# seung-lab/igneous

Measured on NVIDIA H100. Metric: Mvoxels/s on 2048x2048x1024 uint32 seg per GPU (downsample+CCL+mesh) @1/2/4/8 H100; % HBM roofline, higher is better.
Workload: dtype u32

## Files before the change

igneous_b200/csrc/common.cuh:

```cuda
#pragma once
#include <cuda_runtime.h>
#include <stdint.h>
#include <stdio.h>
#include <string>
#include <vector>

#include "../../include/igneous_b200.h"

#if defined(__CUDA_ARCH__) && (__CUDA_ARCH__ != 900)
#error "libigneous_b200 targets sm_90a (Hopper H100) only"
#endif

namespace ign {

void set_error(const char* fmt, ...);

#define IGN_CUDA(call)                                                          \
  do {                                                                          \
    cudaError_t _e = (call);                                                    \
    if (_e != cudaSuccess) {                                                    \
      ign::set_error("%s:%d: %s -> %s", __FILE__, __LINE__, #call,              \
                     cudaGetErrorString(_e));                                   \
      return IGN_ERR_CUDA;                                                      \
    }                                                                           \
  } while (0)

#define IGN_TRY(call)                 \
  do {                                \
    int _s = (call);                  \
    if (_s != IGN_OK) return _s;      \
  } while (0)

#define IGN_REQUIRE(cond, status, ...)   \
  do {                                   \
    if (!(cond)) {                       \
      ign::set_error(__VA_ARGS__);       \
      return (status);                   \
    }                                    \
  } while (0)

static inline int dtype_size(int dt) {
  switch (dt) {
    case IGN_U8: return 1;
    case IGN_U16: return 2;
    case IGN_U32: return 4;
    case IGN_U64: return 8;
    case IGN_F32: return 4;
    default: return 0;
  }
}

template <typename F>
int dispatch_label(int dtype, const char* who, F&& f) {
  switch (dtype) {
    case IGN_U8: return f(uint8_t{});
    case IGN_U16: return f(uint16_t{});
    case IGN_U32: return f(uint32_t{});
    case IGN_U64: return f(uint64_t{});
  }
  set_error("%s: unsupported label dtype %d", who, dtype);
  return IGN_ERR_UNSUPPORTED;
}

}

constexpr int IGN_TIMER_SLOTS = 64;

struct ign_ctx {
  int device;
  int sm_count;
  cudaStream_t stream;
  cudaStream_t copy_stream;
  struct ScratchBlock { char* base; size_t bytes, used; };
  std::vector<ScratchBlock> scratch;
  size_t scratch_lin;
  size_t scratch_high;
  int scratch_frames;
  char* pinned;
  size_t pinned_bytes;
  cudaEvent_t timers[IGN_TIMER_SLOTS][2];
  uint64_t launches;
  int prof_on;
  struct ProfRec { int cls; cudaEvent_t a, b; };
  ProfRec* prof;
  int prof_n, prof_cap;
  char* mesh_pool;
  size_t mesh_pool_bytes;
  int mesh_pool_busy;
  char* win;
  char* win_dev;
  size_t win_fetch_used, win_push_used;
  struct FetchRec { void* dst; size_t off, bytes; };
  FetchRec fetch[32];
  int fetch_n;
};

enum { IGN_PROF_CCL_LOCAL = 0, IGN_PROF_CCL_MERGE = 1, IGN_PROF_CCL_LABEL = 2, IGN_PROF_POOL = 3,
       IGN_PROF_MC = 4, IGN_PROF_SIMP = 5, IGN_PROF_CLASSES = 8 };

namespace ign {

int activate(ign_ctx* ctx);
class ScratchFrame {
 public:
  explicit ScratchFrame(ign_ctx* ctx);
  ~ScratchFrame();
  ScratchFrame(const ScratchFrame&) = delete;
  ScratchFrame& operator=(const ScratchFrame&) = delete;
  int take(void** p, size_t bytes);
  template <typename T>
  int take(T** p, size_t count) { return take((void**)p, count * sizeof(T)); }
  void rewind();
  bool innermost() const;

 private:
  ign_ctx* ctx_;
  std::vector<size_t> mark_;
  size_t mark_lin_;
  int depth_;
};

static inline size_t align_up(size_t v, size_t a) { return (v + a - 1) / a * a; }

struct HostBuf {
  const void* from;
  void* to;
  size_t bytes;
};

template <typename F>
int staged(ign_ctx* ctx, std::vector<HostBuf>& bufs, F&& call) {
  IGN_TRY(activate(ctx));
  ScratchFrame f(ctx);
  std::vector<void*> d(bufs.size(), nullptr);
  for (size_t i = 0; i < bufs.size(); i++) {
    if (!bufs[i].from && !bufs[i].to) continue;
    IGN_TRY(f.take(&d[i], bufs[i].bytes));
    if (bufs[i].from)
      IGN_CUDA(cudaMemcpyAsync(d[i], bufs[i].from, bufs[i].bytes, cudaMemcpyHostToDevice, ctx->stream));
  }
  IGN_TRY(call(d.data()));
  for (size_t i = 0; i < bufs.size(); i++)
    if (bufs[i].to) IGN_CUDA(cudaMemcpyAsync(bufs[i].to, d[i], bufs[i].bytes, cudaMemcpyDeviceToHost, ctx->stream));
  IGN_CUDA(cudaStreamSynchronize(ctx->stream));
  return IGN_OK;
}
template <typename F>
int staged(ign_ctx* ctx, std::vector<HostBuf>&& bufs, F&& call) {
  return staged(ctx, bufs, call);
}

int small_d2h(ign_ctx* ctx, void* host_dst, const void* dev_src, size_t bytes);
int d2h_by_kernel(ign_ctx* ctx, void* host_dst, const void* dev_src, size_t bytes);
int small_h2d(ign_ctx* ctx, void* dev_dst, const void* host_src, size_t bytes);
int small_sync(ign_ctx* ctx);

#define IGN_LAUNCH(ctx, kernel, grid, block, smem, ...)                          \
  do {                                                                           \
    kernel<<<(grid), (block), (smem), (ctx)->stream>>>(__VA_ARGS__);             \
    (ctx)->launches++;                                                           \
    IGN_CUDA(cudaGetLastError());                                                \
  } while (0)

int prof_begin(ign_ctx* ctx, int cls);
void prof_end(ign_ctx* ctx, int slot);
#define IGN_LAUNCH_PROF(ctx, cls, kernel, grid, block, smem, ...)                 \
  do {                                                                           \
    const int _slot = ign::prof_begin((ctx), (cls));                             \
    kernel<<<(grid), (block), (smem), (ctx)->stream>>>(__VA_ARGS__);             \
    (ctx)->launches++;                                                           \
    ign::prof_end((ctx), _slot);                                                 \
    IGN_CUDA(cudaGetLastError());                                                \
  } while (0)

static inline unsigned blocks_for(uint64_t n, unsigned threads) {
  return (unsigned)((n + threads - 1) / threads);
}

}

#ifdef __CUDACC__
namespace ign {

__device__ __forceinline__ uint4 ld_stream(const void* p) {
  uint4 r;
  asm volatile("ld.global.nc.L1::no_allocate.v4.u32 {%0,%1,%2,%3}, [%4];"
               : "=r"(r.x), "=r"(r.y), "=r"(r.z), "=r"(r.w)
               : "l"(p));
  return r;
}
__device__ __forceinline__ void st_stream(void* p, uint4 v) {
  asm volatile("st.global.L1::no_allocate.v4.u32 [%0], {%1,%2,%3,%4};" ::"l"(p), "r"(v.x),
               "r"(v.y), "r"(v.z), "r"(v.w)
               : "memory");
}
__device__ __forceinline__ void st_stream(void* p, uint2 v) {
  asm volatile("st.global.L1::no_allocate.v2.u32 [%0], {%1,%2};" ::"l"(p), "r"(v.x), "r"(v.y)
               : "memory");
}

__device__ __forceinline__ uint64_t mix64(uint64_t z) {
  z += 0x9E3779B97F4A7C15ull;
  z = (z ^ (z >> 30)) * 0xBF58476D1CE4E5B9ull;
  z = (z ^ (z >> 27)) * 0x94D049BB133111EBull;
  return z ^ (z >> 31);
}

}
#endif
```

igneous_b200/csrc/ctx.cu:

```cuda
#include <stdarg.h>
#include <string.h>

#include "common.cuh"

namespace ign {

static thread_local std::string g_err;

void set_error(const char* fmt, ...) {
  char buf[1024];
  va_list ap;
  va_start(ap, fmt);
  vsnprintf(buf, sizeof(buf), fmt, ap);
  va_end(ap);
  g_err = buf;
}

int activate(ign_ctx* ctx) {
  IGN_REQUIRE(ctx != nullptr, IGN_ERR_INVALID, "null ign_ctx");
  IGN_CUDA(cudaSetDevice(ctx->device));
  return IGN_OK;
}

ScratchFrame::ScratchFrame(ign_ctx* ctx) : ctx_(ctx), mark_lin_(ctx->scratch_lin), depth_(++ctx->scratch_frames) {
  for (const auto& b : ctx->scratch) mark_.push_back(b.used);
}

ScratchFrame::~ScratchFrame() {
  rewind();
  if (--ctx_->scratch_frames > 0 || ctx_->scratch.size() < 2) return;
  if (cudaStreamSynchronize(ctx_->stream) != cudaSuccess) {
    cudaGetLastError();
    return;
  }
  for (const auto& b : ctx_->scratch) cudaFree(b.base);
  ctx_->scratch.clear();
  const size_t bytes = align_up(ctx_->scratch_high, 1 << 20);
  char* base = nullptr;
  if (cudaMalloc((void**)&base, bytes) == cudaSuccess) ctx_->scratch.push_back({base, bytes, 0});
  else cudaGetLastError();
}

void ScratchFrame::rewind() {
  for (size_t b = 0; b < ctx_->scratch.size(); b++) ctx_->scratch[b].used = b < mark_.size() ? mark_[b] : 0;
  ctx_->scratch_lin = mark_lin_;
}

bool ScratchFrame::innermost() const { return ctx_->scratch_frames == depth_; }

int ScratchFrame::take(void** p, size_t bytes) {
  *p = nullptr;
  std::vector<ign_ctx::ScratchBlock>& blocks = ctx_->scratch;
  size_t b = 0, off = 0;
  for (; b < blocks.size(); b++) {
    off = align_up(blocks[b].used, 256);
    if (off + bytes <= blocks[b].bytes) break;
  }
  if (b == blocks.size()) {
    const size_t want = align_up(bytes ? bytes : 1, 1 << 20);
    char* base = nullptr;
    cudaError_t e = cudaMalloc((void**)&base, want);
    if (e != cudaSuccess) {
      cudaGetLastError();
      set_error("scratch arena: cudaMalloc(%zu) failed: %s", want, cudaGetErrorString(e));
      return IGN_ERR_NOMEM;
    }
    blocks.push_back({base, want, 0});
    off = 0;
  }
  blocks[b].used = off + bytes;
  ctx_->scratch_lin = align_up(ctx_->scratch_lin, 256) + bytes;
  if (ctx_->scratch_lin > ctx_->scratch_high) ctx_->scratch_high = ctx_->scratch_lin;
  *p = blocks[b].base + off;
  return IGN_OK;
}

template <typename T>
__global__ void __launch_bounds__(256)
    k_copy_box(const T* __restrict__ src, uint64_t sx, uint64_t sy, uint64_t x0, uint64_t y0,
               uint64_t z0, uint64_t bx, uint64_t by, uint64_t total, T* __restrict__ dst) {
  const uint64_t i = blockIdx.x * (uint64_t)blockDim.x + threadIdx.x;
  if (i >= total) return;
  const uint64_t x = i % bx, r = i / bx, y = r % by, z = r / by;
  dst[i] = src[((z0 + z) * sy + (y0 + y)) * sx + (x0 + x)];
}

enum : size_t { WIN_FETCH_BYTES = 256 << 10, WIN_PUSH_BYTES = 768 << 10 };

__global__ void __launch_bounds__(256) k_copy_small(void* __restrict__ dst, const void* __restrict__ src,
                                                    uint32_t n_words, uint32_t tail_bytes) {
  const uint32_t i = blockIdx.x * blockDim.x + threadIdx.x;
  if (i < n_words) ((uint32_t*)dst)[i] = ((const uint32_t*)src)[i];
  if (i < tail_bytes) ((uint8_t*)dst)[4ull * n_words + i] = ((const uint8_t*)src)[4ull * n_words + i];
}

static int copy_small_launch(ign_ctx* ctx, void* dst, const void* src, size_t bytes);

__global__ void __launch_bounds__(256) k_copy_to_host(uint4* __restrict__ dst, const uint4* __restrict__ src, uint64_t n16) {
  for (uint64_t i = blockIdx.x * (uint64_t)blockDim.x + threadIdx.x; i < n16; i += (uint64_t)gridDim.x * blockDim.x)
    dst[i] = src[i];
}

int d2h_by_kernel(ign_ctx* ctx, void* host_dst, const void* dev_src, size_t bytes) {
  cudaPointerAttributes at;
  const bool pinned = cudaPointerGetAttributes(&at, host_dst) == cudaSuccess && at.type == cudaMemoryTypeHost &&
                      at.devicePointer != nullptr;
  cudaGetLastError();
  if (!pinned || ((uintptr_t)at.devicePointer % 16) != 0 || ((uintptr_t)dev_src % 16) != 0) {
    IGN_CUDA(cudaMemcpyAsync(host_dst, dev_src, bytes, cudaMemcpyDeviceToHost, ctx->stream));
    return IGN_OK;
  }
  const uint64_t n16 = bytes / 16;
  if (n16) {
    const unsigned grid = (unsigned)(blocks_for(n16, 256) < (uint64_t)ctx->sm_count * 2 ? blocks_for(n16, 256) : (uint64_t)ctx->sm_count * 2);
    IGN_LAUNCH(ctx, k_copy_to_host, grid, 256, 0, (uint4*)at.devicePointer, (const uint4*)dev_src, n16);
  }
  if (bytes % 16)
    IGN_TRY(copy_small_launch(ctx, (char*)at.devicePointer + 16 * n16, (const char*)dev_src + 16 * n16, bytes % 16));
  return IGN_OK;
}

static int copy_small_launch(ign_ctx* ctx, void* dst, const void* src, size_t bytes) {
  const bool words = ((uintptr_t)dst % 4 == 0) && ((uintptr_t)src % 4 == 0);
  const uint32_t nw = words ? (uint32_t)(bytes / 4) : 0;
  const uint32_t tail = (uint32_t)(bytes - 4ull * nw);
  const uint32_t work = nw > tail ? nw : tail;
  IGN_LAUNCH(ctx, k_copy_small, blocks_for(work, 256), 256, 0, dst, src, nw, tail);
  return IGN_OK;
}

int small_d2h(ign_ctx* ctx, void* host_dst, const void* dev_src, size_t bytes) {
  if (bytes == 0) return IGN_OK;
  const size_t off = align_up(ctx->win_fetch_used, 16);
  if (!ctx->win || ctx->fetch_n == 32 || off + bytes > WIN_FETCH_BYTES) {
    IGN_CUDA(cudaMemcpyAsync(host_dst, dev_src, bytes, cudaMemcpyDeviceToHost, ctx->stream));
    return IGN_OK;
  }
  IGN_TRY(copy_small_launch(ctx, ctx->win_dev + off, dev_src, bytes));
  ctx->fetch[ctx->fetch_n++] = {host_dst, off, bytes};
  ctx->win_fetch_used = off + bytes;
  return IGN_OK;
}

int small_sync(ign_ctx* ctx) {
  cudaError_t e = cudaStreamSynchronize(ctx->stream);
  if (e == cudaSuccess)
    for (int i = 0; i < ctx->fetch_n; i++)
      memcpy(ctx->fetch[i].dst, ctx->win + ctx->fetch[i].off, ctx->fetch[i].bytes);
  ctx->fetch_n = 0;
  ctx->win_fetch_used = 0;
  ctx->win_push_used = 0;
  IGN_CUDA(e);
  return IGN_OK;
}

int small_h2d(ign_ctx* ctx, void* dev_dst, const void* host_src, size_t bytes) {
  if (bytes == 0) return IGN_OK;
  if (!ctx->win || bytes > WIN_PUSH_BYTES) {
    IGN_CUDA(cudaMemcpyAsync(dev_dst, host_src, bytes, cudaMemcpyHostToDevice, ctx->stream));
    return IGN_OK;
  }
  size_t off = align_up(ctx->win_push_used, 16);
  if (off + bytes > WIN_PUSH_BYTES) {
    IGN_CUDA(cudaStreamSynchronize(ctx->stream));
    off = 0;
  }
  char* stage = ctx->win + WIN_FETCH_BYTES + off;
  memcpy(stage, host_src, bytes);
  ctx->win_push_used = off + bytes;
  return copy_small_launch(ctx, dev_dst, ctx->win_dev + WIN_FETCH_BYTES + off, bytes);
}

int prof_begin(ign_ctx* ctx, int cls) {
  if (!ctx->prof_on) return -1;
  if (ctx->prof_n == ctx->prof_cap) {
    const int ncap = ctx->prof_cap ? ctx->prof_cap * 2 : 256;
    ign_ctx::ProfRec* np = (ign_ctx::ProfRec*)realloc(ctx->prof, sizeof(ign_ctx::ProfRec) * ncap);
    if (!np) return -1;
    for (int i = ctx->prof_cap; i < ncap; i++) {
      cudaEventCreate(&np[i].a);
      cudaEventCreate(&np[i].b);
    }
    ctx->prof = np;
    ctx->prof_cap = ncap;
  }
  const int slot = ctx->prof_n++;
  ctx->prof[slot].cls = cls;
  cudaEventRecord(ctx->prof[slot].a, ctx->stream);
  return slot;
}

void prof_end(ign_ctx* ctx, int slot) {
  if (slot >= 0) cudaEventRecord(ctx->prof[slot].b, ctx->stream);
}

}

using namespace ign;

extern "C" {

int ign_version(void) { return 100; }

const char* ign_last_error(void) { return g_err.c_str(); }

int ign_device_count(int* n) {
  IGN_REQUIRE(n, IGN_ERR_INVALID, "null out pointer");
  cudaError_t e = cudaGetDeviceCount(n);
  if (e != cudaSuccess) {
    *n = 0;
    set_error("cudaGetDeviceCount: %s", cudaGetErrorString(e));
    cudaGetLastError();
    return IGN_ERR_CUDA;
  }
  return IGN_OK;
}

int ign_init(int device, ign_ctx** out) {
  IGN_REQUIRE(out, IGN_ERR_INVALID, "null out pointer");
  *out = nullptr;
  int n = 0;
  IGN_TRY(ign_device_count(&n));
  IGN_REQUIRE(n > 0, IGN_ERR_CUDA, "no CUDA device visible (this library has no CPU fallback)");
  IGN_REQUIRE(device >= 0 && device < n, IGN_ERR_INVALID, "device %d out of range [0,%d)", device, n);
  IGN_CUDA(cudaSetDevice(device));
  cudaDeviceProp prop;
  IGN_CUDA(cudaGetDeviceProperties(&prop, device));
  IGN_REQUIRE(prop.major == 9 && prop.minor == 0, IGN_ERR_UNSUPPORTED,
              "device %d is sm_%d%d; libigneous_b200 is built for sm_90a (H100) only", device,
              prop.major, prop.minor);
  ign_ctx* ctx = new ign_ctx();
  ctx->device = device;
  ctx->sm_count = prop.multiProcessorCount;
  ctx->launches = 0;
  ctx->prof_on = 0;
  ctx->prof = nullptr;
  ctx->prof_n = ctx->prof_cap = 0;
  ctx->mesh_pool = nullptr;
  ctx->mesh_pool_bytes = 0;
  ctx->mesh_pool_busy = 0;
  IGN_CUDA(cudaStreamCreateWithFlags(&ctx->stream, cudaStreamNonBlocking));
  IGN_CUDA(cudaStreamCreateWithFlags(&ctx->copy_stream, cudaStreamNonBlocking));
  ctx->pinned_bytes = 1 << 20;
  IGN_CUDA(cudaHostAlloc((void**)&ctx->pinned, ctx->pinned_bytes, cudaHostAllocDefault));
  for (int i = 0; i < IGN_TIMER_SLOTS; i++) {
    IGN_CUDA(cudaEventCreate(&ctx->timers[i][0]));
    IGN_CUDA(cudaEventCreate(&ctx->timers[i][1]));
  }
  ctx->win = ctx->win_dev = nullptr;
  ctx->win_fetch_used = ctx->win_push_used = 0;
  ctx->fetch_n = 0;
  if (cudaHostAlloc((void**)&ctx->win, WIN_FETCH_BYTES + WIN_PUSH_BYTES,
                    cudaHostAllocMapped | cudaHostAllocPortable) != cudaSuccess ||
      cudaHostGetDevicePointer((void**)&ctx->win_dev, ctx->win, 0) != cudaSuccess) {
    cudaGetLastError();
    if (ctx->win) cudaFreeHost(ctx->win);
    ctx->win = ctx->win_dev = nullptr;
  }
  *out = ctx;
  return IGN_OK;
}

int ign_destroy(ign_ctx* ctx) {
  if (!ctx) return IGN_OK;
  cudaSetDevice(ctx->device);
  cudaStreamSynchronize(ctx->stream);
  for (const auto& b : ctx->scratch) cudaFree(b.base);
  if (ctx->pinned) cudaFreeHost(ctx->pinned);
  if (ctx->win) cudaFreeHost(ctx->win);
  if (ctx->mesh_pool) cudaFree(ctx->mesh_pool);
  for (int i = 0; i < IGN_TIMER_SLOTS; i++) {
    cudaEventDestroy(ctx->timers[i][0]);
    cudaEventDestroy(ctx->timers[i][1]);
  }
  cudaStreamDestroy(ctx->stream);
  cudaStreamDestroy(ctx->copy_stream);
  delete ctx;
  return IGN_OK;
}

int ign_sync(ign_ctx* ctx) {
  IGN_TRY(activate(ctx));
  IGN_CUDA(cudaStreamSynchronize(ctx->stream));
  return IGN_OK;
}

int ign_launch_count(ign_ctx* ctx, uint64_t* n) {
  IGN_REQUIRE(ctx && n, IGN_ERR_INVALID, "null argument");
  *n = ctx->launches;
  return IGN_OK;
}

int ign_stream(ign_ctx* ctx, void** stream) {
  IGN_REQUIRE(ctx && stream, IGN_ERR_INVALID, "null argument");
  *stream = (void*)ctx->stream;
  return IGN_OK;
}

int ign_dev_alloc(ign_ctx* ctx, uint64_t bytes, void** dptr) {
  IGN_TRY(activate(ctx));
  IGN_REQUIRE(dptr, IGN_ERR_INVALID, "null out pointer");
  *dptr = nullptr;
  cudaError_t e = cudaMalloc(dptr, bytes ? bytes : 1);
  if (e != cudaSuccess) {
    cudaGetLastError();
    set_error("cudaMalloc(%llu) failed: %s", (unsigned long long)bytes, cudaGetErrorString(e));
    return IGN_ERR_NOMEM;
  }
  return IGN_OK;
}

int ign_dev_free(ign_ctx* ctx, void* dptr) {
  IGN_TRY(activate(ctx));
  IGN_CUDA(cudaStreamSynchronize(ctx->stream));
  IGN_CUDA(cudaFree(dptr));
  return IGN_OK;
}

int ign_host_alloc(ign_ctx* ctx, uint64_t bytes, void** hptr) {
  IGN_TRY(activate(ctx));
  IGN_REQUIRE(hptr, IGN_ERR_INVALID, "null out pointer");
  cudaError_t e = cudaHostAlloc(hptr, bytes ? bytes : 1, cudaHostAllocDefault);
  if (e != cudaSuccess) {
    cudaGetLastError();
    set_error("cudaHostAlloc(%llu) failed: %s", (unsigned long long)bytes, cudaGetErrorString(e));
    return IGN_ERR_NOMEM;
  }
  return IGN_OK;
}

int ign_host_free(ign_ctx* ctx, void* hptr) {
  IGN_TRY(activate(ctx));
  IGN_CUDA(cudaFreeHost(hptr));
  return IGN_OK;
}

static const uint64_t BULK_PIECE = 64ull << 20;

static int bulk_copy(ign_ctx* ctx, void* dst, const void* src, uint64_t bytes, cudaMemcpyKind kind) {
  for (uint64_t at = 0; at < bytes; at += BULK_PIECE) {
    const uint64_t nb = bytes - at < BULK_PIECE ? bytes - at : BULK_PIECE;
    IGN_CUDA(cudaMemcpyAsync((char*)dst + at, (const char*)src + at, nb, kind, ctx->stream));
  }
  return IGN_OK;
}

int ign_h2d(ign_ctx* ctx, void* dst, const void* src, uint64_t bytes) {
  IGN_TRY(activate(ctx));
  return bulk_copy(ctx, dst, src, bytes, cudaMemcpyHostToDevice);
}

int ign_d2h(ign_ctx* ctx, void* dst, const void* src, uint64_t bytes) {
  IGN_TRY(activate(ctx));
  return bulk_copy(ctx, dst, src, bytes, cudaMemcpyDeviceToHost);
}

int ign_d2d(ign_ctx* ctx, void* dst, const void* src, uint64_t bytes) {
  IGN_TRY(activate(ctx));
  IGN_CUDA(cudaMemcpyAsync(dst, src, bytes, cudaMemcpyDeviceToDevice, ctx->stream));
  return IGN_OK;
}

int ign_memset(ign_ctx* ctx, void* dst, int byte, uint64_t bytes) {
  IGN_TRY(activate(ctx));
  IGN_CUDA(cudaMemsetAsync(dst, byte, bytes, ctx->stream));
  return IGN_OK;
}

int ign_prof_enable(ign_ctx* ctx, int on) {
  IGN_REQUIRE(ctx, IGN_ERR_INVALID, "null ctx");
  ctx->prof_on = on ? 1 : 0;
  ctx->prof_n = 0;
  return IGN_OK;
}

int ign_prof_read(ign_ctx* ctx, int cls, float* total_ms, uint64_t* launches) {
  IGN_TRY(activate(ctx));
  IGN_REQUIRE(total_ms && launches, IGN_ERR_INVALID, "null argument");
  IGN_CUDA(cudaStreamSynchronize(ctx->stream));
  float sum = 0;
  uint64_t cnt = 0;
  for (int i = 0; i < ctx->prof_n; i++) {
    if (ctx->prof[i].cls != cls) continue;
    float ms = 0;
    IGN_CUDA(cudaEventElapsedTime(&ms, ctx->prof[i].a, ctx->prof[i].b));
    sum += ms;
    cnt++;
  }
  *total_ms = sum;
  *launches = cnt;
  return IGN_OK;
}

int ign_copy_box_dev(ign_ctx* ctx, const void* src, int dtype, uint64_t sx, uint64_t sy, uint64_t sz,
                     uint64_t x0, uint64_t y0, uint64_t z0, uint64_t bx, uint64_t by, uint64_t bz,
                     void* dst) {
  IGN_TRY(activate(ctx));
  const size_t es = dtype_size(dtype);
  IGN_REQUIRE(src && dst && es > 0, IGN_ERR_INVALID, "bad copy_box argument");
  IGN_REQUIRE(x0 + bx <= sx && y0 + by <= sy && z0 + bz <= sz, IGN_ERR_INVALID, "box outside the volume");
  const uint64_t total = bx * by * bz;
  if (total == 0) return IGN_OK;
  const unsigned g = blocks_for(total, 256);
  switch (es) {
    case 1: IGN_LAUNCH(ctx, (k_copy_box<uint8_t>), g, 256, 0, (const uint8_t*)src, sx, sy, x0, y0, z0, bx, by, total, (uint8_t*)dst); break;
    case 2: IGN_LAUNCH(ctx, (k_copy_box<uint16_t>), g, 256, 0, (const uint16_t*)src, sx, sy, x0, y0, z0, bx, by, total, (uint16_t*)dst); break;
    case 4: IGN_LAUNCH(ctx, (k_copy_box<uint32_t>), g, 256, 0, (const uint32_t*)src, sx, sy, x0, y0, z0, bx, by, total, (uint32_t*)dst); break;
    default: IGN_LAUNCH(ctx, (k_copy_box<uint64_t>), g, 256, 0, (const uint64_t*)src, sx, sy, x0, y0, z0, bx, by, total, (uint64_t*)dst); break;
  }
  return IGN_OK;
}

int ign_stream_wait_mark(ign_ctx* waiter, ign_ctx* producer, int slot) {
  IGN_REQUIRE(waiter && producer && slot >= 0 && slot < IGN_TIMER_SLOTS, IGN_ERR_INVALID, "bad stream_wait argument");
  IGN_TRY(activate(waiter));
  IGN_CUDA(cudaStreamWaitEvent(waiter->stream, producer->timers[slot][0], 0));
  return IGN_OK;
}

int ign_stream_priority(ign_ctx* ctx, int high) {
  IGN_TRY(activate(ctx));
  int least = 0, greatest = 0;
  IGN_CUDA(cudaDeviceGetStreamPriorityRange(&least, &greatest));
  IGN_CUDA(cudaStreamSynchronize(ctx->stream));
  cudaStream_t fresh;
  IGN_CUDA(cudaStreamCreateWithPriority(&fresh, cudaStreamNonBlocking, high ? greatest : least));
  cudaStreamDestroy(ctx->stream);
  ctx->stream = fresh;
  return IGN_OK;
}

int ign_timer_start(ign_ctx* ctx, int slot) {
  IGN_TRY(activate(ctx));
  IGN_REQUIRE(slot >= 0 && slot < IGN_TIMER_SLOTS, IGN_ERR_INVALID, "timer slot %d out of range", slot);
  IGN_CUDA(cudaEventRecord(ctx->timers[slot][0], ctx->stream));
  return IGN_OK;
}

int ign_timer_stop(ign_ctx* ctx, int slot) {
  IGN_TRY(activate(ctx));
  IGN_REQUIRE(slot >= 0 && slot < IGN_TIMER_SLOTS, IGN_ERR_INVALID, "timer slot %d out of range", slot);
  IGN_CUDA(cudaEventRecord(ctx->timers[slot][1], ctx->stream));
  return IGN_OK;
}

int ign_timer_ms(ign_ctx* ctx, int slot, float* ms) {
  IGN_TRY(activate(ctx));
  IGN_REQUIRE(slot >= 0 && slot < IGN_TIMER_SLOTS && ms, IGN_ERR_INVALID, "bad timer argument");
  IGN_CUDA(cudaEventSynchronize(ctx->timers[slot][1]));
  IGN_CUDA(cudaEventElapsedTime(ms, ctx->timers[slot][0], ctx->timers[slot][1]));
  return IGN_OK;
}

}
```

igneous_b200/csrc/mesh.cu:

```cuda
#include <cub/device/device_radix_sort.cuh>
#include <cub/device/device_scan.cuh>

#include <atomic>
#include <climits>
#include <vector>

#include "common.cuh"
#include "mc_table.h"

namespace ign {

constexpr unsigned MFULL = 0xFFFFFFFFu;
constexpr int TRI_T_BITS = 3, TRI_CUBE_BITS = 30;
constexpr int V_COORD_BITS = 11;
constexpr int V_LABEL_SHIFT = 3 * V_COORD_BITS;
constexpr int TRI_LABEL_SHIFT = TRI_T_BITS + TRI_CUBE_BITS;

__constant__ int8_t c_edge_mid[12][3] = {{1, 0, 0}, {2, 1, 0}, {1, 2, 0}, {0, 1, 0},
                                         {1, 0, 2}, {2, 1, 2}, {1, 2, 2}, {0, 1, 2},
                                         {0, 0, 1}, {2, 0, 1}, {2, 2, 1}, {0, 2, 1}};

struct McTables {
  int8_t tri[256][16];
  uint8_t ntri[256];
};
__constant__ McTables c_mc;

__device__ __forceinline__ void cube_corners(const uint32_t* __restrict__ lab, uint32_t sx,
                                             uint32_t sxy, uint32_t base, uint32_t (&c)[8]) {
  c[0] = lab[base];
  c[1] = lab[base + 1];
  c[2] = lab[base + 1 + sx];
  c[3] = lab[base + sx];
  c[4] = lab[base + sxy];
  c[5] = lab[base + 1 + sxy];
  c[6] = lab[base + 1 + sx + sxy];
  c[7] = lab[base + sx + sxy];
}

template <bool EMIT>
__global__ void __launch_bounds__(256)
    k_mc(const uint32_t* __restrict__ lab, uint32_t sx, uint32_t sy, uint32_t sz,
         unsigned long long* total, uint64_t* __restrict__ keys, uint8_t* __restrict__ cases,
         uint64_t capacity) {
  __shared__ uint8_t s_ntri[256];
  for (int i = threadIdx.x; i < 256; i += blockDim.x) s_ntri[i] = c_mc.ntri[i];
  __syncthreads();
  const uint32_t cx = sx - 1, cy = sy - 1, cz = sz - 1;
  const uint64_t ncubes = (uint64_t)cx * cy * cz;
  const uint64_t t = blockIdx.x * (uint64_t)blockDim.x + threadIdx.x;
  const uint32_t lane = threadIdx.x & 31;
  uint32_t mine = 0;
  uint32_t c[8];
  uint32_t x = 0, y = 0, z = 0;
  bool active = false;
  if (t < ncubes) {
    x = (uint32_t)(t % cx);
    y = (uint32_t)((t / cx) % cy);
    z = (uint32_t)(t / ((uint64_t)cx * cy));
    cube_corners(lab, sx, sx * sy, (z * sy + y) * sx + x, c);
    const uint32_t o = c[0] | c[1] | c[2] | c[3] | c[4] | c[5] | c[6] | c[7];
    const bool same = (c[0] == c[1]) & (c[0] == c[2]) & (c[0] == c[3]) & (c[0] == c[4]) &
                      (c[0] == c[5]) & (c[0] == c[6]) & (c[0] == c[7]);
    active = (o != 0) && !same;
  }
  uint8_t idxs[8];
  if (active) {
#pragma unroll
    for (int k = 0; k < 8; k++) {
      const uint32_t L = c[k];
      bool first = (L != 0);
#pragma unroll
      for (int j = 0; j < 8; j++)
        if (j < k) first = first && (c[j] != L);
      uint32_t idx = 0;
#pragma unroll
      for (int j = 0; j < 8; j++) idx |= (uint32_t)(c[j] == L) << j;
      idxs[k] = first ? (uint8_t)idx : 0;
      mine += s_ntri[idxs[k]];
    }
  }
  if (!EMIT) {
    uint32_t s = mine;
    for (int d = 16; d > 0; d >>= 1) s += __shfl_down_sync(MFULL, s, d);
    if (lane == 0 && s) atomicAdd(total, (unsigned long long)s);
    return;
  }
  uint32_t incl = mine;
  for (int d = 1; d < 32; d <<= 1) {
    const uint32_t v = __shfl_up_sync(MFULL, incl, d);
    if (lane >= d) incl += v;
  }
  const uint32_t warp_total = __shfl_sync(MFULL, incl, 31);
  if (warp_total == 0) return;
  unsigned long long base = 0;
  if (lane == 31) base = atomicAdd(total, (unsigned long long)warp_total);
  base = __shfl_sync(MFULL, base, 31);
  uint64_t pos = base + (incl - mine);
  if (active) {
    const uint64_t cube = (uint64_t)t;
#pragma unroll
    for (int k = 0; k < 8; k++) {
      const uint32_t n = s_ntri[idxs[k]];
      for (uint32_t tt = 0; tt < n; tt++) {
        if (pos < capacity) {
          keys[pos] = ((uint64_t)c[k] << TRI_LABEL_SHIFT) | (cube << TRI_T_BITS) | tt;
          cases[pos] = idxs[k];
        }
        pos++;
      }
    }
  }
}

__global__ void __launch_bounds__(256)
    k_tri_vertices(const uint64_t* __restrict__ keys, const uint8_t* __restrict__ cases, uint64_t T,
                   uint32_t cx, uint32_t cy, uint64_t* __restrict__ vkeys,
                   uint32_t* __restrict__ corner) {
  const uint64_t t = blockIdx.x * (uint64_t)blockDim.x + threadIdx.x;
  if (t >= T) return;
  const uint64_t key = keys[t];
  const uint64_t label = key >> TRI_LABEL_SHIFT;
  const uint64_t cube = (key >> TRI_T_BITS) & ((1ull << TRI_CUBE_BITS) - 1);
  const uint32_t tt = (uint32_t)(key & ((1u << TRI_T_BITS) - 1));
  const uint32_t x = (uint32_t)(cube % cx), y = (uint32_t)((cube / cx) % cy),
                 z = (uint32_t)(cube / ((uint64_t)cx * cy));
  const int8_t* row = c_mc.tri[cases[t]];
#pragma unroll
  for (int v = 0; v < 3; v++) {
    const int e = row[3 * tt + (2 - v)];
    const uint64_t vx = 2 * x + c_edge_mid[e][0], vy = 2 * y + c_edge_mid[e][1],
                   vz = 2 * z + c_edge_mid[e][2];
    vkeys[3 * t + v] = (label << V_LABEL_SHIFT) | (vz << (2 * V_COORD_BITS)) | (vy << V_COORD_BITS) | vx;
    corner[3 * t + v] = (uint32_t)(3 * t + v);
  }
}

__global__ void __launch_bounds__(256)
    k_label_starts(const uint64_t* __restrict__ keys, uint64_t n, int shift,
                   uint32_t* __restrict__ start ) {
  const uint64_t i = blockIdx.x * (uint64_t)blockDim.x + threadIdx.x;
  if (i >= n) return;
  const uint64_t label = keys[i] >> shift;
  if (i == 0 || (keys[i - 1] >> shift) != label) start[label] = (uint32_t)i;
}

__global__ void __launch_bounds__(256) k_fill_u32(uint32_t* a, uint32_t value, uint32_t n) {
  const uint32_t i = blockIdx.x * blockDim.x + threadIdx.x;
  if (i < n) a[i] = value;
}

__global__ void __launch_bounds__(256)
    k_vertex_heads(const uint64_t* __restrict__ vkeys_sorted, uint64_t n, uint32_t* __restrict__ heads) {
  const uint64_t i = blockIdx.x * (uint64_t)blockDim.x + threadIdx.x;
  if (i < n) heads[i] = (i == 0 || vkeys_sorted[i - 1] != vkeys_sorted[i]) ? 1u : 0u;
}

__global__ void __launch_bounds__(256)
    k_vertex_assign(const uint64_t* __restrict__ vkeys_sorted, const uint32_t* __restrict__ corner_sorted,
                    const uint32_t* __restrict__ heads, const uint32_t* __restrict__ rank, uint64_t n,
                    uint64_t* __restrict__ uniq_vkeys, uint32_t* __restrict__ face_global) {
  const uint64_t i = blockIdx.x * (uint64_t)blockDim.x + threadIdx.x;
  if (i >= n) return;
  const uint32_t id = rank[i] + heads[i] - 1;
  if (heads[i]) uniq_vkeys[id] = vkeys_sorted[i];
  face_global[corner_sorted[i]] = id;
}

__global__ void __launch_bounds__(256)
    k_faces_local(const uint64_t* __restrict__ tri_keys, const uint32_t* __restrict__ vert_off,
                  uint64_t T, uint32_t* __restrict__ faces) {
  const uint64_t i = blockIdx.x * (uint64_t)blockDim.x + threadIdx.x;
  if (i >= 3 * T) return;
  const uint64_t label = tri_keys[i / 3] >> TRI_LABEL_SHIFT;
  faces[i] -= vert_off[label];
}

__global__ void __launch_bounds__(256)
    k_vertex_positions(const uint64_t* __restrict__ uniq_vkeys, uint64_t first, uint64_t count,
                       float rx, float ry, float rz, float shift, float* __restrict__ out) {
  const uint64_t i = blockIdx.x * (uint64_t)blockDim.x + threadIdx.x;
  if (i >= count) return;
  const uint64_t k = uniq_vkeys[first + i];
  const float x = (float)(k & ((1u << V_COORD_BITS) - 1));
  const float y = (float)((k >> V_COORD_BITS) & ((1u << V_COORD_BITS) - 1));
  const float z = (float)((k >> (2 * V_COORD_BITS)) & ((1u << V_COORD_BITS) - 1));
  out[3 * i + 0] = __fmul_rn(__fadd_rn(__fmul_rn(x, 0.5f), shift), rx);
  out[3 * i + 1] = __fmul_rn(__fadd_rn(__fmul_rn(y, 0.5f), shift), ry);
  out[3 * i + 2] = __fmul_rn(__fadd_rn(__fmul_rn(z, 0.5f), shift), rz);
}

}

#include "mesher.h"

namespace ign {
int simp_export_positions(ign_ctx* ctx, const float* pos_f, uint64_t first, uint64_t count,
                          const float shift[3], float* d_out);
}
using namespace ign;

static int mesher_positions(ign_mesher* m, uint64_t first, uint64_t count, const float resolution[3],
                            int voxel_centered, float* d_out) {
  ign_ctx* ctx = m->ctx;
  if (m->simplified) {
    IGN_REQUIRE(resolution[0] == m->res[0] && resolution[1] == m->res[1] && resolution[2] == m->res[2],
                IGN_ERR_INVALID, "resolution differs from the one the mesher was simplified with");
    const float shift[3] = {voxel_centered ? 0.5f * m->res[0] : 0.0f, voxel_centered ? 0.5f * m->res[1] : 0.0f,
                            voxel_centered ? 0.5f * m->res[2] : 0.0f};
    return simp_export_positions(ctx, m->d_pos_f, first, count, shift, d_out);
  }
  IGN_LAUNCH(ctx, k_vertex_positions, blocks_for(count, 256), 256, 0, m->d_uniq_vkeys, first, count,
             resolution[0], resolution[1], resolution[2], voxel_centered ? 0.5f : 0.0f, d_out);
  return IGN_OK;
}

static std::atomic<bool> g_tables_loaded[64];

static int load_tables(ign_ctx* ctx) {
  if (ctx->device < 64 && g_tables_loaded[ctx->device]) return IGN_OK;
  McTables h;
  memcpy(h.tri, mc_tri_table, sizeof(h.tri));
  memcpy(h.ntri, mc_tri_count, sizeof(h.ntri));
  IGN_CUDA(cudaMemcpyToSymbolAsync(c_mc, &h, sizeof(h), 0, cudaMemcpyHostToDevice, ctx->stream));
  IGN_CUDA(cudaStreamSynchronize(ctx->stream));
  if (ctx->device < 64) g_tables_loaded[ctx->device] = true;
  return IGN_OK;
}

static int bits_for(uint64_t v) {
  int b = 1;
  while (b < 64 && (1ull << b) <= v) b++;
  return b;
}

extern "C" {

int ign_mesh_free(ign_mesher* m) {
  if (!m) return IGN_OK;
  cudaSetDevice(m->ctx->device);
  if (m->pooled) {
    m->ctx->mesh_pool_busy = 0;
  } else {
    if (m->d_uniq_vkeys) cudaFree(m->d_uniq_vkeys);
    if (m->d_faces) cudaFree(m->d_faces);
  }
  delete m;
  return IGN_OK;
}

int ign_mesh_begin_dev(ign_ctx* ctx, const void* labels, int dtype, uint64_t sx, uint64_t sy,
                       uint64_t sz, ign_mesher** out) {
  IGN_TRY(activate(ctx));
  IGN_REQUIRE(labels && out, IGN_ERR_INVALID, "null argument");
  *out = nullptr;
  IGN_REQUIRE(sx >= 1 && sy >= 1 && sz >= 1, IGN_ERR_INVALID, "empty volume");
  IGN_REQUIRE(sx <= 1023 && sy <= 1023 && sz <= 1023, IGN_ERR_UNSUPPORTED,
              "mesher: task of %llux%llux%llu exceeds the 1023^3 limit of the packed vertex format",
              (unsigned long long)sx, (unsigned long long)sy, (unsigned long long)sz);
  IGN_TRY(load_tables(ctx));
  const uint64_t n = sx * sy * sz;

  ign_mesher* m = new ign_mesher();
  m->ctx = ctx;
  m->K = m->T = m->U = 0;
  m->d_uniq_vkeys = nullptr;
  m->d_faces = nullptr;
  m->pooled = false;
  m->simplified = false;
  m->d_pos_f = nullptr;
  m->simp_factor = 0;
  m->simp_max_error = 0;
  m->simp_rounds = 0;
  struct Guard {
    ign_mesher* m;
    ~Guard() { ign_mesh_free(m); }
  } guard{m};
  ScratchFrame f(ctx);

  uint32_t* d_lab;
  IGN_TRY(f.take(&d_lab, n));
  uint64_t K = 0;
  {
    ScratchFrame fu(ctx);
    uint64_t* d_uniq;
    IGN_TRY(fu.take(&d_uniq, n));
    IGN_TRY(ign_renumber_dev(ctx, labels, dtype, n, d_lab, d_uniq, n, &K));
    m->K = K;
    m->ids.resize(K);
    if (K) {
      IGN_TRY(small_d2h(ctx, m->ids.data(), d_uniq, K * 8));
      IGN_TRY(small_sync(ctx));
    }
  }
  m->tri_off.assign(K + 2, 0);
  m->vert_off.assign(K + 2, 0);
  if (K == 0 || sx < 2 || sy < 2 || sz < 2) {
    guard.m = nullptr;
    *out = m;
    return IGN_OK;
  }
  IGN_REQUIRE(K < (1ull << 31), IGN_ERR_OVERFLOW, "mesher: too many labels");

  unsigned long long* d_total;
  IGN_TRY(f.take(&d_total, 32));
  const uint64_t ncubes = (sx - 1) * (sy - 1) * (sz - 1);
  const unsigned grid = blocks_for(ncubes, 256);
  unsigned long long T = 0;
  IGN_CUDA(cudaMemsetAsync(d_total, 0, 8, ctx->stream));
  IGN_LAUNCH(ctx, (k_mc<false>), grid, 256, 0, d_lab, (uint32_t)sx, (uint32_t)sy, (uint32_t)sz, d_total,
             (uint64_t*)nullptr, (uint8_t*)nullptr, 0ull);
  IGN_TRY(small_d2h(ctx, &T, d_total, 8));
  IGN_TRY(small_sync(ctx));
  m->T = T;
  if (T == 0) {
    guard.m = nullptr;
    *out = m;
    return IGN_OK;
  }
  IGN_REQUIRE(3 * T <= (unsigned long long)INT_MAX, IGN_ERR_OVERFLOW,
              "mesher: %llu triangles exceed 2^31 - 1 corners; split the volume into tasks", T);

  size_t sort1 = 0, sort2 = 0, scanb = 0;
  cub::DeviceRadixSort::SortPairs(nullptr, sort1, (const uint64_t*)nullptr, (uint64_t*)nullptr,
                                  (const uint8_t*)nullptr, (uint8_t*)nullptr, (int)T);
  cub::DeviceRadixSort::SortPairs(nullptr, sort2, (const uint64_t*)nullptr, (uint64_t*)nullptr,
                                  (const uint32_t*)nullptr, (uint32_t*)nullptr, (int)(3 * T));
  cub::DeviceScan::ExclusiveSum(nullptr, scanb, (const uint32_t*)nullptr, (uint32_t*)nullptr, (int)(3 * T));
  size_t tmp_bytes = sort1 > sort2 ? sort1 : sort2;
  if (scanb > tmp_bytes) tmp_bytes = scanb;
  uint64_t *keys, *keys_s, *vkeys, *vkeys_s;
  uint8_t *cases, *cases_s;
  uint32_t *corner, *corner_s, *heads, *rank, *d_tri_off, *d_vert_off;
  void* tmp;
  IGN_TRY(f.take(&keys, T));
  IGN_TRY(f.take(&keys_s, T));
  IGN_TRY(f.take(&cases, T));
  IGN_TRY(f.take(&cases_s, T));
  IGN_TRY(f.take(&vkeys, 3 * T));
  IGN_TRY(f.take(&vkeys_s, 3 * T));
  IGN_TRY(f.take(&corner, 3 * T));
  IGN_TRY(f.take(&corner_s, 3 * T));
  IGN_TRY(f.take(&heads, 3 * T));
  IGN_TRY(f.take(&rank, 3 * T));
  IGN_TRY(f.take(&d_tri_off, K + 2));
  IGN_TRY(f.take(&d_vert_off, K + 2));
  IGN_TRY(f.take(&tmp, tmp_bytes));

  IGN_CUDA(cudaMemsetAsync(d_total, 0, 8, ctx->stream));
  IGN_LAUNCH(ctx, (k_mc<true>), grid, 256, 0, d_lab, (uint32_t)sx, (uint32_t)sy, (uint32_t)sz, d_total, keys,
             cases, (uint64_t)T);
  const int label_bits = bits_for(K);
  size_t tb = tmp_bytes;
  IGN_CUDA(cub::DeviceRadixSort::SortPairs(tmp, tb, keys, keys_s, cases, cases_s, (int)T, 0,
                                           TRI_LABEL_SHIFT + label_bits, ctx->stream));
  ctx->launches += 4;

  IGN_LAUNCH(ctx, k_tri_vertices, blocks_for(T, 256), 256, 0, keys_s, cases_s, (uint64_t)T, (uint32_t)(sx - 1),
             (uint32_t)(sy - 1), vkeys, corner);
  tb = tmp_bytes;
  IGN_CUDA(cub::DeviceRadixSort::SortPairs(tmp, tb, vkeys, vkeys_s, corner, corner_s, (int)(3 * T), 0,
                                           V_LABEL_SHIFT + label_bits, ctx->stream));
  ctx->launches += 4;
  IGN_LAUNCH(ctx, k_vertex_heads, blocks_for(3 * T, 256), 256, 0, vkeys_s, (uint64_t)(3 * T), heads);
  tb = tmp_bytes;
  IGN_CUDA(cub::DeviceScan::ExclusiveSum(tmp, tb, heads, rank, (int)(3 * T), ctx->stream));
  ctx->launches += 2;
  uint32_t last[2];
  IGN_TRY(small_d2h(ctx, &last[0], rank + (3 * T - 1), 4));
  IGN_TRY(small_d2h(ctx, &last[1], heads + (3 * T - 1), 4));
  IGN_TRY(small_sync(ctx));
  const uint64_t U = (uint64_t)last[0] + last[1];
  m->U = U;
  {
    const size_t fbytes = align_up(3 * T * 4, 256), vbytes = align_up(U * 12, 256);
    if (!ctx->mesh_pool_busy) {
      if (ctx->mesh_pool_bytes < fbytes + vbytes) {
        IGN_CUDA(cudaStreamSynchronize(ctx->stream));
        if (ctx->mesh_pool) cudaFree(ctx->mesh_pool);
        ctx->mesh_pool = nullptr;
        ctx->mesh_pool_bytes = 0;
        const size_t want = (fbytes + vbytes) * 5 / 4;
        IGN_CUDA(cudaMalloc((void**)&ctx->mesh_pool, want));
        ctx->mesh_pool_bytes = want;
      }
      m->d_faces = (uint32_t*)ctx->mesh_pool;
      m->d_uniq_vkeys = (uint64_t*)(ctx->mesh_pool + fbytes);
      m->pooled = true;
      ctx->mesh_pool_busy = 1;
    } else {
      IGN_CUDA(cudaMalloc((void**)&m->d_faces, 3 * T * 4));
      IGN_CUDA(cudaMalloc((void**)&m->d_uniq_vkeys, U * 12));
    }
  }
  IGN_LAUNCH(ctx, k_vertex_assign, blocks_for(3 * T, 256), 256, 0, vkeys_s, corner_s, heads, rank,
             (uint64_t)(3 * T), m->d_uniq_vkeys, m->d_faces);

  IGN_LAUNCH(ctx, k_fill_u32, blocks_for(K + 2, 256), 256, 0, d_tri_off, (uint32_t)T, (uint32_t)(K + 2));
  IGN_LAUNCH(ctx, k_fill_u32, blocks_for(K + 2, 256), 256, 0, d_vert_off, (uint32_t)U, (uint32_t)(K + 2));
  IGN_LAUNCH(ctx, k_label_starts, blocks_for(T, 256), 256, 0, keys_s, (uint64_t)T, TRI_LABEL_SHIFT, d_tri_off);
  IGN_LAUNCH(ctx, k_label_starts, blocks_for(U, 256), 256, 0, m->d_uniq_vkeys, U, V_LABEL_SHIFT, d_vert_off);
  IGN_TRY(small_d2h(ctx, m->tri_off.data(), d_tri_off, (K + 2) * 4));
  IGN_TRY(small_d2h(ctx, m->vert_off.data(), d_vert_off, (K + 2) * 4));
  IGN_TRY(small_sync(ctx));
  for (int64_t l = (int64_t)K; l >= 0; l--) {
    if (m->tri_off[l] > m->tri_off[l + 1]) m->tri_off[l] = m->tri_off[l + 1];
    if (m->vert_off[l] > m->vert_off[l + 1]) m->vert_off[l] = m->vert_off[l + 1];
  }
  IGN_TRY(small_h2d(ctx, d_vert_off, m->vert_off.data(), (K + 2) * 4));
  IGN_LAUNCH(ctx, k_faces_local, blocks_for(3 * T, 256), 256, 0, keys_s, d_vert_off, (uint64_t)T, m->d_faces);
  IGN_CUDA(cudaStreamSynchronize(ctx->stream));
  for (uint64_t l = 1; l <= K; l++)
    if (m->tri_off[l + 1] > m->tri_off[l]) m->present.push_back(m->ids[l - 1]);
  guard.m = nullptr;
  *out = m;
  return IGN_OK;
}

int ign_mesh_begin(ign_ctx* ctx, const void* labels, int dtype, uint64_t sx, uint64_t sy, uint64_t sz,
                   ign_mesher** out) {
  return staged(ctx, {{labels, nullptr, sx * sy * sz * dtype_size(dtype)}},
                [&](void* const* d) { return ign_mesh_begin_dev(ctx, d[0], dtype, sx, sy, sz, out); });
}

int ign_mesh_num_ids(ign_mesher* m, uint64_t* n) {
  IGN_REQUIRE(m && n, IGN_ERR_INVALID, "null argument");
  *n = m->present.size();
  return IGN_OK;
}

int ign_mesh_ids(ign_mesher* m, uint64_t* ids, uint64_t capacity) {
  IGN_REQUIRE(m && ids, IGN_ERR_INVALID, "null argument");
  const uint64_t k = m->present.size() < capacity ? m->present.size() : capacity;
  for (uint64_t i = 0; i < k; i++) ids[i] = m->present[i];
  return IGN_OK;
}

int ign_mesh_totals(ign_mesher* m, uint64_t* nv, uint64_t* nf) {
  IGN_REQUIRE(m && nv && nf, IGN_ERR_INVALID, "null argument");
  *nv = m->U;
  *nf = m->T;
  return IGN_OK;
}

static int64_t dense_of(ign_mesher* m, uint64_t id) {
  for (uint64_t i = 0; i < m->ids.size(); i++)
    if (m->ids[i] == id) return (int64_t)i + 1;
  return -1;
}

int ign_mesh_counts(ign_mesher* m, uint64_t id, uint64_t* nv, uint64_t* nf) {
  IGN_REQUIRE(m && nv && nf, IGN_ERR_INVALID, "null argument");
  const int64_t l = dense_of(m, id);
  IGN_REQUIRE(l > 0, IGN_ERR_KEY, "%llu", (unsigned long long)id);
  *nv = m->vert_off[l + 1] - m->vert_off[l];
  *nf = m->tri_off[l + 1] - m->tri_off[l];
  return IGN_OK;
}

int ign_mesh_get(ign_mesher* m, uint64_t id, const float resolution[3], int reduction_factor,
                 float max_error, int voxel_centered, float* vertices, uint32_t* faces, uint64_t* nv,
                 uint64_t* nf) {
  IGN_REQUIRE(m && resolution && nv && nf, IGN_ERR_INVALID, "null argument");
  ign_ctx* ctx = m->ctx;
  IGN_TRY(activate(ctx));
  if (reduction_factor > 0 && !m->simplified) IGN_TRY(ign_mesh_simplify(m, resolution, reduction_factor, max_error));
  if (m->simplified) {
    IGN_REQUIRE(reduction_factor == m->simp_factor && max_error == m->simp_max_error, IGN_ERR_INVALID,
                "mesher was simplified with reduction_factor=%d max_error=%g; call mesh() again to change",
                m->simp_factor, (double)m->simp_max_error);
  }
  const int64_t l = dense_of(m, id);
  IGN_REQUIRE(l > 0, IGN_ERR_KEY, "%llu", (unsigned long long)id);
  const uint64_t v0 = m->vert_off[l], v1 = m->vert_off[l + 1];
  const uint64_t t0 = m->tri_off[l], t1 = m->tri_off[l + 1];
  *nv = v1 - v0;
  *nf = t1 - t0;
  if (*nv == 0 || vertices == nullptr || faces == nullptr) return IGN_OK;
  ScratchFrame f(ctx);
  float* d_pos;
  IGN_TRY(f.take(&d_pos, (v1 - v0) * 3));
  IGN_TRY(mesher_positions(m, v0, v1 - v0, resolution, voxel_centered, d_pos));
  IGN_CUDA(cudaMemcpyAsync(vertices, d_pos, (v1 - v0) * 12, cudaMemcpyDeviceToHost, ctx->stream));
  IGN_CUDA(cudaMemcpyAsync(faces, m->d_faces + 3 * t0, (t1 - t0) * 12, cudaMemcpyDeviceToHost, ctx->stream));
  IGN_CUDA(cudaStreamSynchronize(ctx->stream));
  return IGN_OK;
}

int ign_mesh_export(ign_mesher* m, const float resolution[3], int voxel_centered, float* vertices,
                    uint32_t* faces, uint64_t* vert_offsets, uint64_t* face_offsets) {
  IGN_REQUIRE(m && resolution && vert_offsets && face_offsets, IGN_ERR_INVALID, "null argument");
  ign_ctx* ctx = m->ctx;
  IGN_TRY(activate(ctx));
  uint64_t j = 0;
  for (uint64_t l = 1; l <= m->K; l++) {
    if (m->tri_off[l + 1] > m->tri_off[l]) {
      vert_offsets[j] = m->vert_off[l];
      face_offsets[j] = m->tri_off[l];
      j++;
    }
  }
  vert_offsets[j] = m->U;
  face_offsets[j] = m->T;
  if (m->U == 0 || vertices == nullptr || faces == nullptr) return IGN_OK;
  ScratchFrame f(ctx);
  float* d_pos;
  IGN_TRY(f.take(&d_pos, m->U * 3));
  IGN_TRY(mesher_positions(m, 0, m->U, resolution, voxel_centered, d_pos));
  IGN_TRY(d2h_by_kernel(ctx, vertices, d_pos, m->U * 12));
  IGN_TRY(d2h_by_kernel(ctx, faces, m->d_faces, m->T * 12));
  IGN_CUDA(cudaStreamSynchronize(ctx->stream));
  return IGN_OK;
}

}
```

igneous_b200/csrc/simplify.cu:

```cuda
#include <cub/device/device_radix_sort.cuh>
#include <cub/device/device_scan.cuh>

#include <stdlib.h>

#include <algorithm>
#include <type_traits>

#include "mesher.h"

namespace ign {

constexpr uint64_t S_KEYMAX = 0xFFFFFFFFFFFFFFFFull;
constexpr int S_MAXV = 32;
constexpr int S_VCAP = 64;
constexpr int VB = 11;

struct Simp {
  uint64_t U, T;
  double* pos;
  double* Q;
  uint32_t* face;
  uint32_t* flabel;
  uint8_t* falive;
  uint8_t* valive;
  uint8_t* vbound;
  uint32_t* vf;
  uint32_t* vn;
  const uint32_t* tri_off;
};

__device__ __forceinline__ uint32_t s_mix(uint32_t x) {
  x ^= x >> 16; x *= 0x7feb352dU; x ^= x >> 15; x *= 0x846ca68bU; x ^= x >> 16;
  return x;
}
__device__ __forceinline__ uint32_t s_unmix(uint32_t x) {
  x ^= x >> 16; x *= 0x43021123U; x ^= x >> 15 ^ x >> 30; x *= 0x1d69e2a5U; x ^= x >> 16;
  return x;
}
__device__ __forceinline__ uint32_t s_mix16(uint32_t x) {
  x &= 0xFFFFu;
  x = (x * 0x2F35u) & 0xFFFFu; x ^= x >> 7;
  x = (x * 0x4A6Bu) & 0xFFFFu; x ^= x >> 9;
  x = (x * 0x9E37u) & 0xFFFFu; x ^= x >> 8;
  return x;
}
__device__ __forceinline__ uint32_t s_unmix16(uint32_t x) {
  x &= 0xFFFFu;
  x ^= x >> 8; x = (x * 0x7787u) & 0xFFFFu;
  x ^= x >> 9; x = (x * 0x1243u) & 0xFFFFu;
  x ^= x >> 7; x ^= x >> 14; x = (x * 0xEB1Du) & 0xFFFFu;
  return x;
}
__device__ __forceinline__ unsigned long long s_key(double cost, uint32_t h, uint32_t salt) {
  const float c = __double2float_rn(cost);
  return ((unsigned long long)__float_as_uint(c) << 32) | s_mix(h ^ salt);
}

__device__ __forceinline__ double s_qeval(const double* q, const double* p) {
  const double x = p[0], y = p[1], z = p[2];
  return q[0] * x * x + 2.0 * q[1] * x * y + 2.0 * q[2] * x * z + 2.0 * q[3] * x + q[4] * y * y +
         2.0 * q[5] * y * z + 2.0 * q[6] * y + q[7] * z * z + 2.0 * q[8] * z + q[9];
}

__device__ int s_twins(const Simp& s, uint32_t f, uint32_t u, uint32_t v, uint32_t* twin) {
  int cnt = 0;
  const uint32_t* lu = s.vf + (uint64_t)u * S_VCAP;
  const uint32_t cu = s.vn[u];
  for (uint32_t j = 0; j < cu; j++) {
    const uint32_t h = lu[j];
    const uint32_t g = h / 3;
    if (g == f || !s.falive[g]) continue;
    const uint32_t* fv = s.face + 3 * (uint64_t)g;
    if (fv[0] == v || fv[1] == v || fv[2] == v) {
      if (cnt == 0) *twin = h;
      cnt++;
    }
  }
  return cnt;
}

struct SEval {
  bool valid;
  double cost;
  uint32_t keep, remove;
  double p[3];
};

__device__ __forceinline__ void s_cost_q(const double* q, const double* pu, const double* pv, double max_err2,
                                         uint32_t u, uint32_t v, bool bu, bool bv, SEval* e) {
  e->valid = false;
  if (bu && bv) return;
  double best[3], cost;
  if (bu) {
    e->keep = u;
    e->remove = v;
    best[0] = pu[0]; best[1] = pu[1]; best[2] = pu[2];
    cost = s_qeval(q, best);
  } else if (bv) {
    e->keep = v;
    e->remove = u;
    best[0] = pv[0]; best[1] = pv[1]; best[2] = pv[2];
    cost = s_qeval(q, best);
  } else {
    e->keep = u < v ? u : v;
    e->remove = u < v ? v : u;
    const bool uk = u < v;
    const double kk[3] = {uk ? pu[0] : pv[0], uk ? pu[1] : pv[1], uk ? pu[2] : pv[2]};
    const double rr[3] = {uk ? pv[0] : pu[0], uk ? pv[1] : pu[1], uk ? pv[2] : pu[2]};
    const double mid[3] = {(kk[0] + rr[0]) * 0.5, (kk[1] + rr[1]) * 0.5, (kk[2] + rr[2]) * 0.5};
    const double ck = s_qeval(q, kk), cr = s_qeval(q, rr), cm = s_qeval(q, mid);
    cost = ck;
    best[0] = kk[0]; best[1] = kk[1]; best[2] = kk[2];
    if (cr < cost) { cost = cr; best[0] = rr[0]; best[1] = rr[1]; best[2] = rr[2]; }
    if (cm < cost) { cost = cm; best[0] = mid[0]; best[1] = mid[1]; best[2] = mid[2]; }
  }
  if (cost < 0.0) cost = 0.0;
  if (!(cost <= max_err2)) return;
  e->valid = true;
  e->cost = cost;
  e->p[0] = best[0]; e->p[1] = best[1]; e->p[2] = best[2];
}

__device__ __forceinline__ void s_cost(const double* Q, const double* pos, double max_err2, uint32_t u, uint32_t v,
                                       uint64_t gu, uint64_t gv, bool bu, bool bv, SEval* e) {
  e->valid = false;
  if (bu && bv) return;
  const double* Qu = Q + 10 * gu;
  const double* Qv = Q + 10 * gv;
  double q[10];
#pragma unroll
  for (int i = 0; i < 10; i++) q[i] = Qu[i] + Qv[i];
  s_cost_q(q, pos + 3 * gu, pos + 3 * gv, max_err2, u, v, bu, bv, e);
}

__global__ void __launch_bounds__(256)
    k_simp_init_verts(const uint64_t* __restrict__ vkeys, uint64_t U, double rx, double ry, double rz,
                      double* __restrict__ pos, uint8_t* __restrict__ valive,
                      uint8_t* __restrict__ vbound, uint32_t* __restrict__ vn) {
  const uint64_t i = blockIdx.x * (uint64_t)blockDim.x + threadIdx.x;
  if (i >= U) return;
  const uint64_t k = vkeys[i];
  const double x = (double)(k & ((1u << VB) - 1));
  const double y = (double)((k >> VB) & ((1u << VB) - 1));
  const double z = (double)((k >> (2 * VB)) & ((1u << VB) - 1));
  pos[3 * i + 0] = x * 0.5 * rx;
  pos[3 * i + 1] = y * 0.5 * ry;
  pos[3 * i + 2] = z * 0.5 * rz;
  valive[i] = 1;
  vbound[i] = 0;
  vn[i] = 0;
}

__global__ void __launch_bounds__(256)
    k_simp_init_faces(const uint32_t* __restrict__ faces_local, const uint32_t* __restrict__ tri_off,
                      const uint32_t* __restrict__ vert_off, uint32_t K, uint64_t T,
                      uint32_t* __restrict__ face, uint32_t* __restrict__ flabel,
                      uint8_t* __restrict__ falive, uint32_t* __restrict__ node_vertex,
                      uint32_t* __restrict__ node_id) {
  const uint64_t f = blockIdx.x * (uint64_t)blockDim.x + threadIdx.x;
  if (f >= T) return;
  uint32_t lo = 1, hi = K;
  while (lo < hi) {
    const uint32_t mid = (lo + hi + 1) >> 1;
    if (tri_off[mid] <= f) lo = mid;
    else hi = mid - 1;
  }
  flabel[f] = lo;
  falive[f] = 1;
  for (int k = 0; k < 3; k++) {
    const uint32_t g = faces_local[3 * f + k] + vert_off[lo];
    face[3 * f + k] = g;
    node_vertex[3 * f + k] = g;
    node_id[3 * f + k] = (uint32_t)(3 * f + k);
  }
}

__global__ void __launch_bounds__(256)
    k_simp_link(const uint32_t* __restrict__ sv, const uint32_t* __restrict__ sh, uint64_t n,
                uint32_t* __restrict__ vf, uint32_t* __restrict__ vn, uint32_t* overflow) {
  const uint64_t i = blockIdx.x * (uint64_t)blockDim.x + threadIdx.x;
  if (i >= n) return;
  const uint32_t v = sv[i];
  if (i > 0 && sv[i - 1] == v) return;
  uint32_t c = 0;
  for (uint64_t j = i; j < n && sv[j] == v; j++) {
    if (c < S_VCAP) vf[(uint64_t)v * S_VCAP + c] = sh[j];
    c++;
  }
  if (c > S_VCAP) {
    *overflow = 1;
    c = S_VCAP;
  }
  vn[v] = c;
}

__global__ void __launch_bounds__(128) k_simp_quadrics(Simp s) {
  const uint64_t v = blockIdx.x * (uint64_t)blockDim.x + threadIdx.x;
  if (v >= s.U) return;
  double q[10];
  for (int i = 0; i < 10; i++) q[i] = 0.0;
  for (uint32_t j = 0; j < s.vn[v]; j++) {
    const uint32_t h = s.vf[(uint64_t)v * S_VCAP + j];
    const uint32_t* fv = s.face + 3 * (uint64_t)(h / 3);
    const double* a = s.pos + 3 * (uint64_t)fv[0];
    const double* b = s.pos + 3 * (uint64_t)fv[1];
    const double* c = s.pos + 3 * (uint64_t)fv[2];
    const double ux = b[0] - a[0], uy = b[1] - a[1], uz = b[2] - a[2];
    const double vx = c[0] - a[0], vy = c[1] - a[1], vz = c[2] - a[2];
    double nx = uy * vz - uz * vy, ny = uz * vx - ux * vz, nz = ux * vy - uy * vx;
    const double len = sqrt(nx * nx + ny * ny + nz * nz);
    if (!(len > 0.0)) continue;
    nx = nx / len; ny = ny / len; nz = nz / len;
    const double d = -(nx * a[0] + ny * a[1] + nz * a[2]);
    q[0] += nx * nx; q[1] += nx * ny; q[2] += nx * nz; q[3] += nx * d;
    q[4] += ny * ny; q[5] += ny * nz; q[6] += ny * d;
    q[7] += nz * nz; q[8] += nz * d; q[9] += d * d;
  }
  for (int i = 0; i < 10; i++) s.Q[10 * v + i] = q[i];
}

__global__ void __launch_bounds__(256) k_simp_boundary(Simp s) {
  const uint64_t h = blockIdx.x * (uint64_t)blockDim.x + threadIdx.x;
  if (h >= 3 * s.T) return;
  const uint32_t f = (uint32_t)(h / 3), c = (uint32_t)(h % 3);
  const uint32_t u = s.face[3 * (uint64_t)f + c], v = s.face[3 * (uint64_t)f + (c + 1) % 3];
  uint32_t tw;
  if (s_twins(s, f, u, v, &tw) != 1) {
    s.vbound[u] = 1;
    s.vbound[v] = 1;
  }
}

__global__ void __launch_bounds__(256)
    k_simp_ecost(Simp s, double max_err2, float* __restrict__ ecost, uint8_t* __restrict__ fstate,
                 uint32_t* counts) {
  const uint64_t f = blockIdx.x * (uint64_t)blockDim.x + threadIdx.x;
  uint32_t n = 0;
  if (f < s.T) {
    const uint32_t* fv = s.face + 3 * f;
    uint32_t st = 0;
#pragma unroll
    for (int c = 0; c < 3; c++) {
      const uint32_t u = fv[c], v = fv[(c + 1) % 3];
      if (!(u < v)) continue;
      SEval ev;
      s_cost(s.Q, s.pos, max_err2, u, v, u, v, s.vbound[u] != 0, s.vbound[v] != 0, &ev);
      uint32_t es = 3;
      if (ev.valid) {
        ecost[3 * f + c] = __double2float_rn(ev.cost);
        es = 2;
      }
      st |= es << (2 * c);
      n++;
    }
    fstate[f] = (uint8_t)st;
  }
  const int tot = __syncthreads_count(n & 1u) + 2 * __syncthreads_count(n >> 1);
  if (threadIdx.x == 0 && tot) atomicAdd(counts, (uint32_t)tot);
}

constexpr uint32_t VF_ALIVE = 1, VF_BOUND = 2, VF_DONE = 16, VF_END = 32, VF_RDIRTY = 64;
constexpr int SL_THREADS = 1024;
constexpr int SL_WCAP = 128;
constexpr uint32_t WF_BAD = 1;
constexpr int SL_LIST_PER = 16;

constexpr int SL_NCLASS = 3;
constexpr int SL_CLASS_THREADS[SL_NCLASS] = {1024, 512, 256};

struct SlWin {
  double best[3];
  uint32_t u, v, h, cnt[2], keep, flags;
  uint32_t order;
};
constexpr size_t SL_WIN_BYTES = sizeof(SlWin) + 2 * S_MAXV * 2;

struct SlLayout {
  size_t o_ring, o_key, o_f0, o_fl, o_fs, o_vf, o_vl, o_fm, o_vm, need;
};
__host__ __device__ inline SlLayout sl_layout(uint32_t T, uint32_t U, bool resumed = false,
                                              uint32_t wcap = SL_WCAP) {
  SlLayout y;
  y.o_ring = (size_t)wcap * sizeof(SlWin);
  y.o_key = y.o_ring + (size_t)wcap * 2 * S_MAXV * 2;
  y.o_f0 = y.o_key + 4 * (size_t)U;
  y.o_fl = y.o_f0 + 6 * (size_t)T;
  y.o_fs = y.o_fl + 2 * (size_t)T;
  y.o_vf = (y.o_fs + T + 3) & ~(size_t)3;
  y.o_vl = (y.o_vf + U + 3) & ~(size_t)3;
  y.o_fm = (y.o_vl + U + 3) & ~(size_t)3;
  y.o_vm = y.o_fm + 2 * (size_t)T;
  y.need = resumed ? y.o_vm + 2 * (size_t)U + 4 : y.o_vl + U + 4;
  return y;
}
__host__ __device__ inline bool sl_fits_smem(uint32_t T, uint32_t U, uint32_t threads, size_t smem_bytes,
                                             bool resumed = false) {
  const uint32_t cap = (uint32_t)SL_LIST_PER * threads;
  return 3ull * T <= 65536ull && T <= cap && U <= cap && sl_layout(T, U, resumed).need <= smem_bytes;
}
__host__ __device__ inline uint32_t sl_wcap(uint32_t T, uint32_t U, uint32_t threads, size_t smem_bytes,
                                            bool resumed, uint32_t limit) {
  const size_t w = SL_WCAP + (smem_bytes - sl_layout(T, U, resumed).need) / SL_WIN_BYTES;
  const size_t m = threads < limit ? threads : limit;
  return (uint32_t)(w < m ? w : m);
}

struct SlArgs {
  double* pos;
  double* Q;
  uint32_t* face;
  uint8_t* falive;
  uint8_t* valive;
  const uint8_t* vbound;
  float* ecost;
  unsigned long long* key1;
  uint8_t* fstate;
  uint8_t* vflag;
  uint8_t* vlose;
  uint32_t *flist, *flist2;
  uint32_t *vlist, *vlist2;
  const uint32_t* tri_off;
  const uint32_t* vert_off;
  const uint32_t* target;
  const uint32_t* order;
  uint32_t K;
  uint32_t base;
  uint32_t cls;
  uint32_t* counters;
  double max_err2;
  int max_rounds;
  uint32_t smem_bytes;
  uint32_t* mq_next;
  uint32_t smem_next;
  const uint32_t* mq;
  uint16_t* finv;
  int persist;
  uint32_t* lrec;
  uint32_t* trace;
  uint32_t wcap_max;
  uint32_t group_min;
};

constexpr int SL_HIST = 1664, SL_HP = 16, SL_HW = 64, SL_HR = S_MAXV + 2, SL_HCLS = SL_HP + SL_HW + SL_HR;

constexpr int SL_MREC = 8;
constexpr int SL_LREC = 7;
constexpr int SL_NPH = 9;
constexpr int SL_TFLIP = 1620;

struct SlShared {
  uint32_t work, alive, progress, ncol, nwin, stop, slow, counter, npass;
  uint32_t ring8, ring16;
  uint32_t nnarrow, nwide;
  uint32_t rec, valive;
  unsigned long long visits, wins;
  long long t_label;
  uint32_t nrecost;
  uint32_t ngroup[3];
  unsigned long long ph[SL_NPH];
  long long t_prev;
};

template <bool SM>
struct SlLab {
  typedef typename std::conditional<SM, uint16_t, uint32_t>::type idx_t;
  uint32_t T, U, tbase, vbase, target, label;
  idx_t *fc0, *fc1, *fc2;
  idx_t *fmap, *vmap;
  uint32_t* gface;
  uint8_t* fstate;
  uint8_t* vflag;
  uint8_t* vlose;
  typedef typename std::conditional<SM, uint32_t, unsigned long long>::type key_t;
  key_t* key1;
  bool fmt16;
  uint32_t wcap;
  idx_t* ring;
  idx_t *flist, *flist2, *vlist, *vlist2;
};

template <bool SM>
__device__ __forceinline__ uint32_t sl_fget(const SlLab<SM>& L, uint32_t f, int c) {
  if (SM) return c == 0 ? L.fc0[f] : (c == 1 ? L.fc1[f] : L.fc2[f]);
  return L.gface[3 * (uint64_t)f + c] - L.vbase;
}
template <bool SM>
__device__ __forceinline__ void sl_fset(const SlLab<SM>& L, uint32_t f, int c, uint32_t x) {
  typedef typename SlLab<SM>::idx_t idx_t;
  if (SM) {
    if (c == 0) L.fc0[f] = (idx_t)x;
    else if (c == 1) L.fc1[f] = (idx_t)x;
    else L.fc2[f] = (idx_t)x;
  } else {
    L.gface[3 * (uint64_t)f + c] = x + L.vbase;
  }
}
template <bool SM, bool R>
__device__ __forceinline__ uint64_t sl_vg(const SlLab<SM>& L, uint32_t v) {
  return L.vbase + (uint64_t)(R ? (uint32_t)L.vmap[v] : v);
}
template <bool SM, bool R>
__device__ __forceinline__ uint32_t sl_fo(const SlLab<SM>& L, uint32_t f) {
  return R ? (uint32_t)L.fmap[f] : f;
}
template <bool SM>
__device__ __forceinline__ void sl_vor(uint8_t* vflag, uint32_t v, uint32_t bits) {
  const uintptr_t a = (uintptr_t)(vflag + v);
  if ((*(volatile uint8_t*)a & bits) == bits) return;
  const uint32_t word = bits << (8 * (a & 3));
  if (SM) {
    asm volatile("red.shared.or.b32 [%0], %1;" ::"r"((uint32_t)__cvta_generic_to_shared((void*)(a & ~(uintptr_t)3))), "r"(word) : "memory");
  } else {
    atomicOr((uint32_t*)(a & ~(uintptr_t)3), word);
  }
}
template <bool SM>
__device__ __forceinline__ void sl_vclear(uint8_t* vflag, uint32_t v, uint32_t bits) {
  const uintptr_t a = (uintptr_t)(vflag + v);
  const uint32_t word = ~(bits << (8 * (a & 3)));
  if (SM) {
    asm volatile("red.shared.and.b32 [%0], %1;" ::"r"((uint32_t)__cvta_generic_to_shared((void*)(a & ~(uintptr_t)3))), "r"(word) : "memory");
  } else {
    atomicAnd((uint32_t*)(a & ~(uintptr_t)3), word);
  }
}
__device__ __forceinline__ void sl_post(unsigned long long* key1, uint32_t u, uint32_t v, unsigned long long key) {
  if (key < *(volatile unsigned long long*)&key1[u]) atomicMin(&key1[u], key);
  if (key < *(volatile unsigned long long*)&key1[v]) atomicMin(&key1[v], key);
}
__device__ __forceinline__ void sl_post(uint32_t* key1, uint32_t u, uint32_t v, uint32_t key) {
  if (key < *(volatile uint32_t*)&key1[u])
    asm volatile("red.shared.min.u32 [%0], %1;" ::"r"((uint32_t)__cvta_generic_to_shared(key1 + u)), "r"(key) : "memory");
  if (key < *(volatile uint32_t*)&key1[v])
    asm volatile("red.shared.min.u32 [%0], %1;" ::"r"((uint32_t)__cvta_generic_to_shared(key1 + v)), "r"(key) : "memory");
}
template <bool SM>
__device__ __forceinline__ typename SlLab<SM>::key_t sl_key(const SlLab<SM>& L, float cost, uint32_t hl, uint32_t salt) {
  typedef typename SlLab<SM>::key_t key_t;
  const uint32_t bits = __float_as_uint(cost);
  if (SM || L.fmt16) return (key_t)((((bits >> 15) & 0xFFFFu) << 16) | s_mix16((hl ^ salt) & 0xFFFFu));
  return (key_t)(((unsigned long long)bits << 32) | s_mix(hl ^ salt));
}
template <bool SM>
__device__ __forceinline__ uint32_t sl_key_edge(const SlLab<SM>& L, typename SlLab<SM>::key_t key, uint32_t salt) {
  if (SM || L.fmt16) return s_unmix16((uint32_t)key & 0xFFFFu) ^ (salt & 0xFFFFu);
  return s_unmix((uint32_t)((unsigned long long)key & 0xFFFFFFFFull)) ^ salt;
}

template <bool SM, bool R>
__device__ __forceinline__ void sl_cost(const SlArgs& A, const SlLab<SM>& L, uint32_t u, uint32_t v, SEval* e) {
  s_cost(A.Q, A.pos, A.max_err2, u, v, sl_vg<SM, R>(L, u), sl_vg<SM, R>(L, v), (L.vflag[u] & VF_BOUND) != 0,
         (L.vflag[v] & VF_BOUND) != 0, e);
}

template <bool SM>
__device__ __forceinline__ uint32_t sl_kcorner(const SlLab<SM>& L, uint32_t f, uint32_t k) {
  return sl_fget<SM>(L, f, 0) == k ? 0u : (sl_fget<SM>(L, f, 1) == k ? 1u : 2u);
}
template <bool SM, bool R, int W>
__device__ __forceinline__ uint32_t sl_recost_k(const SlArgs& A, const SlLab<SM>& L, bool has, uint32_t f,
                                                uint32_t c, uint32_t k, double qs, double qs2, const double* pk) {
  uint32_t u = k, v = k;
  if (has) { u = sl_fget<SM>(L, f, (int)c); v = sl_fget<SM>(L, f, (int)((c + 1) % 3)); }
  const bool ku = (u == k);
  const uint64_t go = sl_vg<SM, R>(L, ku ? v : u);
  double q[10], po[3] = {0.0, 0.0, 0.0};
#pragma unroll
  for (int i = 0; i < 10; i++) q[i] = has ? A.Q[10 * go + i] : 0.0;
  if (has) { po[0] = A.pos[3 * go]; po[1] = A.pos[3 * go + 1]; po[2] = A.pos[3 * go + 2]; }
#pragma unroll
  for (int i = 0; i < 10; i++)
    q[i] += __shfl_sync(0xFFFFFFFFu, (W == 8 && i >= 8) ? qs2 : qs, (W == 8 && i >= 8) ? i - 8 : i, W);
  if (!has) return 0;
  double pu[3], pv[3];
#pragma unroll
  for (int i = 0; i < 3; i++) {
    const double b = pk[i];
    pu[i] = ku ? b : po[i];
    pv[i] = ku ? po[i] : b;
  }
  SEval ev;
  s_cost_q(q, pu, pv, A.max_err2, u, v, (L.vflag[u] & VF_BOUND) != 0, (L.vflag[v] & VF_BOUND) != 0, &ev);
  if (!ev.valid) return 3;
  A.ecost[3 * (uint64_t)(L.tbase + sl_fo<SM, R>(L, f)) + c] = __double2float_rn(ev.cost);
  return 2;
}

template <bool SM, bool R>
__device__ __forceinline__ bool sl_flips(const SlArgs& A, const SlLab<SM>& L, const uint32_t* a, uint32_t w,
                                         const double* best) {
  double P[3][3], N[3][3];
#pragma unroll
  for (int k = 0; k < 3; k++) {
    const double* p = A.pos + 3 * sl_vg<SM, R>(L, a[k]);
    P[k][0] = p[0]; P[k][1] = p[1]; P[k][2] = p[2];
  }
#pragma unroll
  for (int k = 0; k < 3; k++) {
    const bool mv = (a[k] == w);
    N[k][0] = mv ? best[0] : P[k][0];
    N[k][1] = mv ? best[1] : P[k][1];
    N[k][2] = mv ? best[2] : P[k][2];
  }
  const double ax = P[1][0] - P[0][0], ay = P[1][1] - P[0][1], az = P[1][2] - P[0][2];
  const double bx = P[2][0] - P[0][0], by = P[2][1] - P[0][1], bz = P[2][2] - P[0][2];
  const double n0x = ay * bz - az * by, n0y = az * bx - ax * bz, n0z = ax * by - ay * bx;
  const double cx = N[1][0] - N[0][0], cy = N[1][1] - N[0][1], cz = N[1][2] - N[0][2];
  const double dx = N[2][0] - N[0][0], dy = N[2][1] - N[0][1], dz = N[2][2] - N[0][2];
  const double n1x = cy * dz - cz * dy, n1y = cz * dx - cx * dz, n1z = cx * dy - cy * dx;
  const double dot = n0x * n1x + n0y * n1y + n0z * n1z;
  return !(dot > 0.0);
}

__device__ __forceinline__ void sl_others(const uint32_t* a, uint32_t w, uint32_t* o1, uint32_t* o2) {
  if (a[0] == w) { *o1 = a[1]; *o2 = a[2]; }
  else if (a[1] == w) { *o1 = a[2]; *o2 = a[0]; }
  else { *o1 = a[0]; *o2 = a[1]; }
}

__device__ __forceinline__ uint32_t sl_distinct(uint32_t x1, uint32_t x2, uint32_t n, uint32_t lane, bool* f1,
                                                bool* f2) {
  const uint32_t FULL = 0xFFFFFFFFu;
  const bool have = lane < n;
  const uint32_t m1 = __match_any_sync(FULL, x1);
  const uint32_t m2 = __match_any_sync(FULL, x2);
  *f1 = have && ((int)lane == __ffs(m1) - 1);
  bool in1 = false;
  for (uint32_t j = 0; j < n; j++) in1 |= (__shfl_sync(FULL, x1, j) == x2);
  *f2 = have && ((int)lane == __ffs(m2) - 1) && !in1;
  return __popc(__ballot_sync(FULL, *f1)) + __popc(__ballot_sync(FULL, *f2));
}

template <bool SM, typename IDX, typename PRED>
__device__ __forceinline__ uint32_t sl_compact(IDX*& list, IDX*& list2, uint32_t n, uint32_t* counter, PRED alive) {
  const uint32_t FULL = 0xFFFFFFFFu;
  const uint32_t tid = threadIdx.x, lane = tid & 31u;
  if (tid == 0) *counter = 0;
  __syncthreads();
  if (SM) {
    IDX keep[SL_LIST_PER];
    uint32_t m = 0;
#pragma unroll
    for (int k = 0; k < SL_LIST_PER; k++) {
      const uint32_t i = tid + k * blockDim.x;
      keep[k] = 0;
      if (i < n) {
        const IDX e = list[i];
        keep[k] = e;
        if (alive((uint32_t)e)) m |= 1u << k;
      }
    }
    __syncthreads();
    const uint32_t cnt = __popc(m);
    uint32_t inc = cnt;
#pragma unroll
    for (int d = 1; d < 32; d <<= 1) {
      const uint32_t o = __shfl_up_sync(FULL, inc, d);
      if ((int)lane >= d) inc += o;
    }
    uint32_t base = 0;
    if (lane == 31 && inc) base = atomicAdd(counter, inc);
    base = __shfl_sync(FULL, base, 31) + inc - cnt;
#pragma unroll
    for (int k = 0; k < SL_LIST_PER; k++)
      if ((m >> k) & 1u) list[base++] = keep[k];
  } else {
    for (uint32_t i0 = (tid & ~31u); i0 < n; i0 += blockDim.x) {
      const uint32_t i = i0 + lane;
      IDX e = 0;
      bool al = false;
      if (i < n) {
        e = list[i];
        al = alive((uint32_t)e);
      }
      const uint32_t bal = __ballot_sync(FULL, al);
      if (!bal) continue;
      uint32_t base = 0;
      const int leader = __ffs(bal) - 1;
      if ((int)lane == leader) base = atomicAdd(counter, (uint32_t)__popc(bal));
      base = __shfl_sync(FULL, base, leader);
      if (al) list2[base + __popc(bal & ((1u << lane) - 1u))] = e;
    }
    IDX* t = list;
    list = list2;
    list2 = t;
  }
  __syncthreads();
  const uint32_t kept = *counter;
  __syncthreads();
  return kept;
}

#define SL_MARK(id)                                   \
  do {                                                \
    if (A.trace != nullptr && tid == 0) {             \
      const long long _t = clock64();                 \
      sh.ph[id] += (unsigned long long)(_t - sh.t_prev); \
      sh.t_prev = _t;                                 \
    }                                                 \
  } while (0)

extern __shared__ __align__(16) unsigned char sl_smem[];

__device__ __forceinline__ SlWin* sl_win() { return (SlWin*)sl_smem; }

__device__ __forceinline__ uint32_t sl_width(uint32_t nfu, uint32_t nfv, uint32_t wmin) {
  const uint32_t n = nfu > nfv ? nfu : nfv;
  const uint32_t w = n <= 8u ? 8u : (n <= 16u ? 16u : 32u);
  return w > wmin ? w : wmin;
}

template <bool SM, bool R, int W>
__device__ __forceinline__ void sl_group_pass(const SlArgs& A, const SlLab<SM>& L, SlShared& sh, uint32_t first,
                                              uint32_t last, uint32_t w0, uint32_t* nev) {
  static_assert(W == 8 || W == 16 || W == 32, "group width");
  const uint32_t FULL = 0xFFFFFFFFu;
  const uint32_t tid = threadIdx.x, lane = tid & 31u, warp = tid >> 5, NW = blockDim.x >> 5;
  constexpr uint32_t G = 32 / W;
  const uint32_t gl = lane & (W - 1), goff = lane & ~(uint32_t)(W - 1);
  const uint32_t wmask = W == 32 ? FULL : (1u << W) - 1u;
  const uint32_t gmask = wmask << goff;
  const uint32_t gidx = lane / W;
  SlWin* const win = sl_win();
  for (uint32_t base = first + ((warp + NW - w0) % NW) * G; base < last; base += NW * G) {
    bool act = base + gidx < last;
    uint32_t slot = 0, nfu = 0, nfv = 0;
    if (act) {
      slot = win[base + gidx].order;
      nfu = win[slot].cnt[0]; nfv = win[slot].cnt[1];
    }
    act = act && sl_width(nfu, nfv, A.group_min) == (uint32_t)W;
    const uint32_t b_act = __ballot_sync(FULL, act && gl == 0);
    if (!b_act) continue;
    if (lane == 0) atomicAdd(&sh.ngroup[W == 8 ? 0 : (W == 16 ? 1 : 2)], (uint32_t)__popc(b_act));
    if (W == 32 && act && gl == 0 && (nfu > (uint32_t)S_MAXV || nfv > (uint32_t)S_MAXV)) atomicAdd(&A.counters[25], 1u);
    uint32_t fu = 0, fv = 0, u = 0, v = 0, k = 0;
    bool ok = false;
    if (act) {
      if (gl < nfu) fu = L.ring[(2 * slot) * S_MAXV + gl];
      if (gl < nfv) fv = L.ring[(2 * slot + 1) * S_MAXV + gl];
      u = win[slot].u; v = win[slot].v; k = win[slot].keep;
      ok = !(win[slot].flags & WF_BAD) && nfu <= (uint32_t)S_MAXV && nfv <= (uint32_t)S_MAXV;
    }
    uint32_t au[3] = {0, 0, 0}, av[3] = {0, 0, 0};
    if (ok && gl < nfu) { au[0] = sl_fget<SM>(L, fu, 0); au[1] = sl_fget<SM>(L, fu, 1); au[2] = sl_fget<SM>(L, fu, 2); }
    if (ok && gl < nfv) { av[0] = sl_fget<SM>(L, fv, 0); av[1] = sl_fget<SM>(L, fv, 1); av[2] = sl_fget<SM>(L, fv, 2); }
    uint32_t flip = 0;
    if (ok && gl < nfu && au[0] != v && au[1] != v && au[2] != v && sl_flips<SM, R>(A, L, au, u, win[slot].best)) flip = 1u;
    if (ok && gl < nfv && av[0] != u && av[1] != u && av[2] != u && sl_flips<SM, R>(A, L, av, v, win[slot].best)) flip |= 2u;
    if (__ballot_sync(FULL, flip != 0) & gmask) ok = false;
    if (A.trace != nullptr) {
      const uint32_t b_u = __ballot_sync(FULL, flip & 1u) & gmask, b_v = __ballot_sync(FULL, flip & 2u) & gmask;
      if (act && gl == 0 && (b_u || b_v)) atomicAdd(&A.trace[SL_TFLIP + (b_u && b_v ? 2 : (b_u ? 0 : 1))], 1u);
    }
    const uint32_t rm = (k == u) ? v : u;
    const uint64_t gk = sl_vg<SM, R>(L, k), gr = sl_vg<SM, R>(L, rm);
    double* Qk = A.Q + 10 * gk;
    const double* Qr = A.Q + 10 * gr;
    double qk = 0.0, qr = 0.0, qk2 = 0.0, qr2 = 0.0;
    if (ok && gl < 10) { qk = Qk[gl]; qr = Qr[gl]; }
    if (W == 8 && ok && gl < 2) { qk2 = Qk[gl + 8]; qr2 = Qr[gl + 8]; }
    const bool hu = ok && gl < nfu, hv = ok && gl < nfv;
    uint32_t x1 = 0xF0000000u + lane, x2 = 0xF1000000u + lane, y1 = 0xF2000000u + lane, y2 = 0xF3000000u + lane;
    if (hu) sl_others(au, u, &x1, &x2);
    if (hv) sl_others(av, v, &y1, &y2);
    const bool rm_is_u = (rm == u);
    const uint32_t crm = rm_is_u ? (au[0] == u ? 0u : (au[1] == u ? 1u : 2u)) : (av[0] == v ? 0u : (av[1] == v ? 1u : 2u));
    const uint32_t nu = ok ? nfu : 0u, nv = ok ? nfv : 0u;
    uint32_t nmax = nu > nv ? nu : nv;
#pragma unroll
    for (uint32_t d = W; d < 32u; d <<= 1) {
      const uint32_t o = __shfl_xor_sync(FULL, nmax, d);
      nmax = o > nmax ? o : nmax;
    }
    const uint32_t mu1 = __match_any_sync(FULL, x1) & gmask, mu2 = __match_any_sync(FULL, x2) & gmask;
    const uint32_t mv1 = __match_any_sync(FULL, y1) & gmask, mv2 = __match_any_sync(FULL, y2) & gmask;
    bool inu = false, inv = false, c1 = false, c2 = false;
    for (uint32_t j = 0; j < nmax; j++) {
      const uint32_t sx1 = __shfl_sync(FULL, x1, j, W), sy1 = __shfl_sync(FULL, y1, j, W), sy2 = __shfl_sync(FULL, y2, j, W);
      if (j < nu) inu |= (sx1 == x2);
      if (j < nv) {
        inv |= (sy1 == y2);
        c1 |= (x1 == sy1) | (x1 == sy2);
        c2 |= (x2 == sy1) | (x2 == sy2);
      }
    }
    const bool f1 = hu && ((int)lane == __ffs(mu1) - 1);
    const bool f2 = hu && ((int)lane == __ffs(mu2) - 1) && !inu;
    const bool g1 = hv && ((int)lane == __ffs(mv1) - 1);
    const bool g2 = hv && ((int)lane == __ffs(mv2) - 1) && !inv;
    const uint32_t b_f1 = __ballot_sync(FULL, f1), b_f2 = __ballot_sync(FULL, f2);
    const uint32_t b_g1 = __ballot_sync(FULL, g1), b_g2 = __ballot_sync(FULL, g2);
    const uint32_t b_c1 = __ballot_sync(FULL, f1 && c1), b_c2 = __ballot_sync(FULL, f2 && c2);
    const uint32_t b_sh = __ballot_sync(FULL, hu && (x1 == v || x2 == v));
    const uint32_t nnu = __popc(b_f1 & gmask) + __popc(b_f2 & gmask), nnv = __popc(b_g1 & gmask) + __popc(b_g2 & gmask);
    const uint32_t common = __popc(b_c1 & gmask) + __popc(b_c2 & gmask), shared = __popc(b_sh & gmask);
    const bool go = ok && nnu <= (uint32_t)S_MAXV && nnv <= (uint32_t)S_MAXV && shared == 2 && common == 2;
    if (act && !go && gl == 0) {
      const uint32_t hl = win[slot].h, f = hl / 3, c = hl - 3 * f;
      const uint32_t st = L.fstate[f];
      L.fstate[f] = (uint8_t)((st & ~(3u << (2 * c))) | (1u << (2 * c)));
      sl_vclear<SM>(L.vflag, u, VF_END);
      sl_vclear<SM>(L.vflag, v, VF_END);
      atomicOr(&sh.progress, 1u);
    }
    const bool hr = go && (rm_is_u ? hu : hv);
    const uint32_t rf = rm_is_u ? fu : fv;
    const bool dies = hr && (rm_is_u ? (x1 == k || x2 == k) : (y1 == k || y2 == k));
    if (hr) {
      if (dies) L.fstate[rf] = (uint8_t)(L.fstate[rf] & 0x7Fu);
      else sl_fset<SM>(L, rf, (int)crm, k);
    }
    const uint32_t dead = __popc(__ballot_sync(FULL, dies) & gmask);
    const double qs = qk + qr, qs2 = qk2 + qr2;
    if (go) {
      if (hu && x1 != v && x2 != v) { sl_vor<SM>(L.vflag, x1, VF_RDIRTY); sl_vor<SM>(L.vflag, x2, VF_RDIRTY); }
      if (hv && y1 != u && y2 != u) { sl_vor<SM>(L.vflag, y1, VF_RDIRTY); sl_vor<SM>(L.vflag, y2, VF_RDIRTY); }
      if (gl < 10) Qk[gl] = qs;
      if (gl >= 10 && gl < 13) A.pos[3 * gk + (gl - 10)] = win[slot].best[gl - 10];
      if (W == 8) {
        if (gl < 2) Qk[gl + 8] = qs2;
        else if (gl < 5) A.pos[3 * gk + (gl - 2)] = win[slot].best[gl - 2];
      }
      if (gl == 0) {
        sl_vclear<SM>(L.vflag, k, VF_END);
        sl_vclear<SM>(L.vflag, rm, 0xFFu);
        atomicSub(&sh.alive, dead);
        atomicAdd(&sh.ncol, 1u);
        atomicOr(&sh.progress, 1u);
      }
    }
    __syncwarp();
    uint32_t m = 0, ck = 0, st0 = 0, st1 = 0;
    if (go && gl < nfu) {
      st0 = L.fstate[fu];
      if (st0 & 0x80u) {
        const uint32_t c = sl_kcorner<SM>(L, fu, k);
        ck = c;
        m |= (k < sl_fget<SM>(L, fu, (int)((c + 1) % 3)) ? 1u : 0u) | (sl_fget<SM>(L, fu, (int)((c + 2) % 3)) < k ? 2u : 0u);
      }
    }
    if (go && gl < nfv) {
      st1 = L.fstate[fv];
      if (st1 & 0x80u) {
        const uint32_t c = sl_kcorner<SM>(L, fv, k);
        ck |= c << 2;
        m |= (k < sl_fget<SM>(L, fv, (int)((c + 1) % 3)) ? 4u : 0u) | (sl_fget<SM>(L, fv, (int)((c + 2) % 3)) < k ? 8u : 0u);
      }
    }
    const uint32_t cnt = __popc(m);
    uint32_t inc = cnt;
#pragma unroll
    for (uint32_t d = 1; d < W; d <<= 1) {
      const uint32_t o = __shfl_up_sync(FULL, inc, d, W);
      if (gl >= d) inc += o;
    }
    const uint32_t P = inc - cnt, N = __shfl_sync(FULL, inc, W - 1, W);
    uint32_t rounds = (N + W - 1) / W;
#pragma unroll
    for (uint32_t d = W; d < 32u; d <<= 1) {
      const uint32_t o = __shfl_xor_sync(FULL, rounds, d);
      rounds = o > rounds ? o : rounds;
    }
    uint32_t res = 0;
    for (uint32_t r = 0; r < rounds; r++) {
      const uint32_t idx = r * W + gl;
      uint32_t own = 0;
      for (uint32_t j = 1; j < W; j++)
        if (__shfl_sync(FULL, P, j, W) <= idx) own = j;
      const uint32_t mo = __shfl_sync(FULL, m, own, W), po = __shfl_sync(FULL, P, own, W);
      const uint32_t fuo = __shfl_sync(FULL, fu, own, W), fvo = __shfl_sync(FULL, fv, own, W);
      const uint32_t cko = __shfl_sync(FULL, ck, own, W);
      const bool has = idx < N;
      uint32_t f = 0, c = 0;
      if (has) {
        uint32_t b = mo;
        for (uint32_t q = idx - po; q; q--) b &= b - 1;
        const uint32_t bit = (uint32_t)__ffs(b) - 1, side = bit >> 1;
        c = (((cko >> (2 * side)) & 3u) + 2u * (bit & 1u)) % 3u;
        f = side ? fvo : fuo;
        (*nev)++;
      }
      res |= sl_recost_k<SM, R, W>(A, L, has, f, c, k, qs, qs2, win[slot].best) << (2 * r);
    }
    uint32_t q = P;
#pragma unroll
    for (uint32_t bit = 0; bit < 4; bit++) {
      const uint32_t val = __shfl_sync(FULL, res, q % W, W);
      if ((m >> bit) & 1u) {
        const uint32_t side = bit >> 1, es = (val >> (2 * (q / W))) & 3u;
        const uint32_t c = (((ck >> (2 * side)) & 3u) + 2u * (bit & 1u)) % 3u;
        if (side) st1 = (st1 & ~(3u << (2 * c))) | (es << (2 * c));
        else st0 = (st0 & ~(3u << (2 * c))) | (es << (2 * c));
        q++;
      }
    }
    if (m & 3u) L.fstate[fu] = (uint8_t)st0;
    if (m & 12u) L.fstate[fv] = (uint8_t)st1;
  }
}

template <bool R>
__device__ void sl_migrate(const SlArgs& A, const SlLab<true>& L, SlShared& sh, const uint16_t* flist, uint32_t nF,
                           int r) {
  const uint32_t FULL = 0xFFFFFFFFu;
  const uint32_t tid = threadIdx.x, NT = blockDim.x, lane = tid & 31u, warp = tid >> 5, NW = NT >> 5;
  uint32_t* const wsum = (uint32_t*)sl_win();
  const uint32_t per = (L.U + NT - 1) / NT, v0 = min(tid * per, L.U), v1 = min(v0 + per, L.U);
  uint32_t cnt = 0;
  for (uint32_t v = v0; v < v1; v++) cnt += L.vflag[v] & VF_ALIVE;
  uint32_t inc = cnt;
#pragma unroll
  for (int d = 1; d < 32; d <<= 1) {
    const uint32_t o = __shfl_up_sync(FULL, inc, d);
    if ((int)lane >= d) inc += o;
  }
  if (lane == 31) wsum[warp] = inc;
  __syncthreads();
  if (warp == 0) {
    const uint32_t t = lane < NW ? wsum[lane] : 0u;
    uint32_t x = t;
#pragma unroll
    for (int d = 1; d < 32; d <<= 1) {
      const uint32_t o = __shfl_up_sync(FULL, x, d);
      if ((int)lane >= d) x += o;
    }
    if (lane < NW) wsum[lane] = x - t;
  }
  __syncthreads();
  uint32_t j = wsum[warp] + inc - cnt;
  for (uint32_t v = v0; v < v1; v++) {
    const uint32_t fl = L.vflag[v];
    if (!(fl & VF_ALIVE)) continue;
    A.vlist[L.vbase + j] = (uint32_t)(R ? L.vmap[v] : v) | (fl << 16);
    L.key1[v] = j++;
  }
  __syncthreads();
  for (uint32_t i = tid; i < nF; i += NT) {
    const uint32_t f = flist[i], fo = sl_fo<true, R>(L, f);
    A.flist[L.tbase + i] = L.key1[L.fc0[f]] | (L.key1[L.fc1[f]] << 16);
    A.flist2[L.tbase + i] = L.key1[L.fc2[f]] | (fo << 16);
    A.fstate[L.tbase + i] = L.fstate[f];
    A.finv[L.tbase + fo] = (uint16_t)i;
  }
  if (tid == 0) {
    uint32_t* h = A.mq_next + SL_MREC * (size_t)atomicAdd(&A.counters[16 + A.cls + 1], 1u);
    h[0] = L.label;
    h[1] = sh.rec;
    h[2] = (uint32_t)r + 1;
    h[3] = sh.slow;
    h[4] = nF;
    h[5] = sh.valive;
  }
}

template <bool SM, bool R>
__device__ void sl_run(const SlArgs& A, const SlLab<SM>& L, SlShared& sh, const uint32_t* hdr) {
  if (threadIdx.x == 0) sh.nrecost = sh.ngroup[0] = sh.ngroup[1] = sh.ngroup[2] = 0;
  if (A.trace != nullptr && threadIdx.x == 0) {
    for (int q = 0; q < SL_NPH; q++) sh.ph[q] = 0;
    sh.t_prev = clock64();
    sh.t_label = sh.t_prev;
    sh.visits = 0;
    sh.wins = 0;
  }
  typedef typename SlLab<SM>::idx_t idx_t;
  typedef typename SlLab<SM>::key_t key_t;
  const uint32_t FULL = 0xFFFFFFFFu;
  const uint32_t tid = threadIdx.x, NT = blockDim.x, lane = tid & 31u, warp = tid >> 5, NW = NT >> 5;
  const uint32_t T = L.T, U = L.U;
  idx_t *flist = L.flist, *flist2 = L.flist2, *vlist = L.vlist, *vlist2 = L.vlist2;
  int r = 0;
  if (R) {
    for (uint32_t f = tid; f < T; f += NT) {
      const uint32_t w0 = A.flist[L.tbase + f], w1 = A.flist2[L.tbase + f];
      sl_fset<SM>(L, f, 0, w0 & 0xFFFFu);
      sl_fset<SM>(L, f, 1, w0 >> 16);
      sl_fset<SM>(L, f, 2, w1 & 0xFFFFu);
      L.fmap[f] = (idx_t)(w1 >> 16);
      L.fstate[f] = A.fstate[L.tbase + f];
      flist[f] = (idx_t)f;
    }
    for (uint32_t v = tid; v < U; v += NT) {
      const uint32_t w = A.vlist[L.vbase + v];
      L.vmap[v] = (idx_t)(w & 0xFFFFu);
      L.vflag[v] = (uint8_t)(w >> 16);
    }
    r = (int)hdr[2];
    if (tid == 0) {
      sh.rec = hdr[1];
      sh.slow = hdr[3];
      sh.alive = hdr[4];
    }
  } else {
    for (uint32_t f = tid; f < T; f += NT) {
      if (SM) {
        const uint32_t* g = A.face + 3 * (uint64_t)(L.tbase + f);
        sl_fset<SM>(L, f, 0, g[0] - L.vbase);
        sl_fset<SM>(L, f, 1, g[1] - L.vbase);
        sl_fset<SM>(L, f, 2, g[2] - L.vbase);
      }
      L.fstate[f] = (uint8_t)(0x80u | A.fstate[L.tbase + f]);
      flist[f] = (idx_t)f;
    }
    for (uint32_t v = tid; v < U; v += NT) {
      L.vflag[v] = (uint8_t)(VF_ALIVE | (A.vbound[L.vbase + v] ? VF_BOUND : 0u));
      if (!SM) vlist[v] = (idx_t)v;
    }
    if (tid == 0) {
      sh.rec = A.base + sh.work;
      sh.alive = T;
      sh.slow = 0;
    }
  }
  if (tid == 0) {
    sh.valive = U;
    sh.stop = 0;
  }
  __syncthreads();
  uint32_t nF = T, nV = U;
  bool migrated = false;

  for (; r < A.max_rounds; r++) {
    if (sh.alive <= L.target) break;
    const uint32_t salt = (uint32_t)r * 0x9E3779B9u;
    for (uint32_t i = tid; i < nV; i += NT) {
      const uint32_t v = SM ? i : (uint32_t)vlist[i];
      L.key1[v] = (key_t)S_KEYMAX;
      L.vlose[v] = 0;
      const uint8_t b = L.vflag[v];
      if (b & VF_DONE) L.vflag[v] = (uint8_t)(b & ~VF_DONE);
    }
    if (tid == 0) {
      sh.progress = 0;
      sh.ncol = 0;
      sh.npass = 0;
    }
    __syncthreads();
    SL_MARK(0);
    {
      const float* ecb = A.ecost + 3 * (uint64_t)L.tbase;
      uint32_t f_n = 0, fo_n = 0;
      float ec_n[3] = {0.f, 0.f, 0.f};
      if (warp * 32 + lane < nF) {
        f_n = flist[warp * 32 + lane];
        fo_n = sl_fo<SM, R>(L, f_n);
        ec_n[0] = ecb[3 * (uint64_t)fo_n]; ec_n[1] = ecb[3 * (uint64_t)fo_n + 1]; ec_n[2] = ecb[3 * (uint64_t)fo_n + 2];
      }
      for (uint32_t base = warp * 32; base < nF; base += NT) {
        const uint32_t i = base + lane;
        const uint32_t f = f_n, fo = fo_n;
        const float ec[3] = {ec_n[0], ec_n[1], ec_n[2]};
        if (i + NT < nF) {
          f_n = flist[i + NT];
          fo_n = sl_fo<SM, R>(L, f_n);
          ec_n[0] = ecb[3 * (uint64_t)fo_n]; ec_n[1] = ecb[3 * (uint64_t)fo_n + 1]; ec_n[2] = ecb[3 * (uint64_t)fo_n + 2];
        }
        uint32_t st = 0, a[3] = {0, 0, 0}, fl[3] = {0, 0, 0};
        if (i < nF) st = L.fstate[f];
        bool act = (st & 0x80u) != 0;
        if (act) {
          a[0] = sl_fget<SM>(L, f, 0); a[1] = sl_fget<SM>(L, f, 1); a[2] = sl_fget<SM>(L, f, 2);
          fl[0] = L.vflag[a[0]]; fl[1] = L.vflag[a[1]]; fl[2] = L.vflag[a[2]];
        }
        if (act) {
          uint32_t nst = st;
#pragma unroll
          for (int c = 0; c < 3; c++) {
            const uint32_t u = a[c], v = a[(c + 1) % 3];
            const uint32_t fe = fl[c] | fl[(c + 1) % 3];
            if (!(u < v)) continue;
            uint32_t es = (st >> (2 * c)) & 3u;
            if (es == 1 && (fe & VF_RDIRTY)) es = 2;
            if (es == 2) sl_post(L.key1, u, v, sl_key<SM>(L, ec[c], 3u * fo + (uint32_t)c, salt));
            else if (es == 0) atomicAdd(&A.counters[28], 1u);
            nst = (nst & ~(3u << (2 * c))) | (es << (2 * c));
          }
          if (nst != st) L.fstate[f] = (uint8_t)nst;
        }
      }
    }
    __syncthreads();
    SL_MARK(1);
    for (uint32_t i = tid; i < nV; i += NT) {
      const uint32_t v = SM ? i : (uint32_t)vlist[i];
      if (L.vflag[v] & VF_RDIRTY) sl_vclear<SM>(L.vflag, v, VF_RDIRTY);
    }
    for (uint32_t i = tid; i < nF; i += 2 * NT) {
      const uint32_t i2 = i + NT;
      const bool two = i2 < nF;
      const uint32_t fa = flist[i], fb = two ? (uint32_t)flist[i2] : fa;
      const bool la = (L.fstate[fa] & 0x80u) != 0, lb = two && (L.fstate[fb] & 0x80u) != 0;
      uint32_t a0 = 0, a1 = 0, a2 = 0, b0 = 0, b1 = 0, b2 = 0;
      if (la) { a0 = sl_fget<SM>(L, fa, 0); a1 = sl_fget<SM>(L, fa, 1); a2 = sl_fget<SM>(L, fa, 2); }
      if (lb) { b0 = sl_fget<SM>(L, fb, 0); b1 = sl_fget<SM>(L, fb, 1); b2 = sl_fget<SM>(L, fb, 2); }
      key_t ka0 = 0, ka1 = 0, ka2 = 0, kb0 = 0, kb1 = 0, kb2 = 0;
      if (la) { ka0 = L.key1[a0]; ka1 = L.key1[a1]; ka2 = L.key1[a2]; }
      if (lb) { kb0 = L.key1[b0]; kb1 = L.key1[b1]; kb2 = L.key1[b2]; }
      if (la) {
        key_t m = ka0 < ka1 ? ka0 : ka1;
        m = ka2 < m ? ka2 : m;
        if (ka0 > m) L.vlose[a0] = 1;
        if (ka1 > m) L.vlose[a1] = 1;
        if (ka2 > m) L.vlose[a2] = 1;
      }
      if (lb) {
        key_t m = kb0 < kb1 ? kb0 : kb1;
        m = kb2 < m ? kb2 : m;
        if (kb0 > m) L.vlose[b0] = 1;
        if (kb1 > m) L.vlose[b1] = 1;
        if (kb2 > m) L.vlose[b2] = 1;
      }
    }
    __syncthreads();
    SL_MARK(2);
    SlWin* const win = sl_win();
    for (;;) {
      if (tid == 0) { sh.nwin = 0; sh.ring8 = 0; sh.ring16 = 0; sh.nnarrow = 0; sh.nwide = 0; sh.npass++; }
      __syncthreads();
      for (uint32_t i = tid; i < nV; i += NT) {
        const uint32_t a = SM ? i : (uint32_t)vlist[i];
        const uint32_t fl = L.vflag[a];
        if (!(fl & VF_ALIVE) || (fl & VF_DONE) || L.vlose[a]) continue;
        const key_t key = L.key1[a];
        if (key == (key_t)S_KEYMAX) continue;
        const uint32_t hl = sl_key_edge<SM>(L, key, salt);
        const uint32_t fo = hl / 3, c = hl - 3 * fo;
        const uint32_t f = R ? (uint32_t)A.finv[L.tbase + fo] : fo;
        if (sl_fget<SM>(L, f, (int)c) != a) continue;
        const uint32_t v = sl_fget<SM>(L, f, (int)((c + 1) % 3));
        if (L.key1[v] != key || (L.vflag[v] & VF_DONE) || L.vlose[v]) continue;
        const uint32_t slot = atomicAdd(&sh.nwin, 1u);
        if (slot < L.wcap) {
          win[slot].u = a;
          win[slot].v = v;
          win[slot].h = 3 * f + c;
          win[slot].cnt[0] = 0;
          win[slot].cnt[1] = 0;
          win[slot].flags = 0;
          sl_vor<SM>(L.vflag, a, VF_DONE | VF_END);
          sl_vor<SM>(L.vflag, v, VF_DONE | VF_END);
        }
      }
      __syncthreads();
      SL_MARK(3);
      const uint32_t total = sh.nwin;
      const uint32_t nb = total < L.wcap ? total : L.wcap;
      if (A.trace != nullptr && tid == 0 && sh.npass == 1) {
        const uint32_t b = total / 16 < (uint32_t)SL_HW - 1 ? total / 16 : (uint32_t)SL_HW - 1;
        atomicAdd(&A.trace[SL_HIST + SL_HCLS * A.cls + SL_HP + b], 1u);
      }
      if (nb == 0) break;
      if (A.trace != nullptr && tid == 0) sh.wins += nb;
      for (uint32_t i = tid; i < nb; i += NT) {
        L.key1[win[i].u] = (key_t)(2u * i);
        L.key1[win[i].v] = (key_t)(2u * i + 1u);
      }
      __syncthreads();
      SL_MARK(4);
      {
        const uint32_t nbt = (nb + 31u) & ~31u;
        const bool split = NT - nbt >= NT / 2;
        if (tid < nb) {
          const uint32_t i = tid;
          SEval e;
          sl_cost<SM, R>(A, L, win[i].u, win[i].v, &e);
          win[i].keep = e.valid ? e.keep : win[i].u;
          win[i].flags = e.valid ? 0u : WF_BAD;
          if (e.valid) {
            win[i].best[0] = e.p[0]; win[i].best[1] = e.p[1]; win[i].best[2] = e.p[2];
          }
        }
        if (!split || tid >= nbt) {
          const uint32_t first = split ? tid - nbt : tid, step = split ? NT - nbt : NT;
          for (uint32_t i = first; i < nF; i += 2 * step) {
            const uint32_t i2 = i + step;
            const bool two = i2 < nF;
            const uint32_t fa = flist[i], fb = two ? (uint32_t)flist[i2] : fa;
            const bool la = (L.fstate[fa] & 0x80u) != 0, lb = two && (L.fstate[fb] & 0x80u) != 0;
            uint32_t x[6] = {0, 0, 0, 0, 0, 0}, fl[6] = {0, 0, 0, 0, 0, 0};
            if (la) { x[0] = sl_fget<SM>(L, fa, 0); x[1] = sl_fget<SM>(L, fa, 1); x[2] = sl_fget<SM>(L, fa, 2); }
            if (lb) { x[3] = sl_fget<SM>(L, fb, 0); x[4] = sl_fget<SM>(L, fb, 1); x[5] = sl_fget<SM>(L, fb, 2); }
            if (la) { fl[0] = L.vflag[x[0]]; fl[1] = L.vflag[x[1]]; fl[2] = L.vflag[x[2]]; }
            if (lb) { fl[3] = L.vflag[x[3]]; fl[4] = L.vflag[x[4]]; fl[5] = L.vflag[x[5]]; }
#pragma unroll
            for (int c = 0; c < 6; c++) {
              if (!(fl[c] & VF_END)) continue;
              const uint32_t sl = (uint32_t)L.key1[x[c]];
              const uint32_t p = atomicAdd(&win[sl >> 1].cnt[sl & 1u], 1u);
              if (p < (uint32_t)S_MAXV) L.ring[sl * S_MAXV + p] = (idx_t)(c < 3 ? fa : fb);
              if (p == 8u) sh.ring8 = 1;
              if (p == 16u) sh.ring16 = 1;
            }
          }
        }
      }
      __syncthreads();
      SL_MARK(5);
      SL_MARK(6);
      if (A.trace != nullptr) {
        for (uint32_t i = tid; i < 2 * nb; i += NT) {
          const uint32_t n = win[i >> 1].cnt[i & 1u];
          atomicAdd(&A.trace[SL_HIST + SL_HCLS * A.cls + SL_HP + SL_HW + (n <= (uint32_t)S_MAXV ? n : S_MAXV + 1)], 1u);
        }
      }
      for (uint32_t i0 = warp * 32; i0 < nb; i0 += NT) {
        const uint32_t i = i0 + lane;
        const bool have = i < nb;
        const bool narrow = have && sl_width(win[i].cnt[0], win[i].cnt[1], A.group_min) == 8u;
        const uint32_t bn = __ballot_sync(FULL, narrow), bw = __ballot_sync(FULL, have && !narrow);
        uint32_t pn = 0, pw = 0;
        if (lane == 0) {
          if (bn) pn = atomicAdd(&sh.nnarrow, (uint32_t)__popc(bn));
          if (bw) pw = atomicAdd(&sh.nwide, (uint32_t)__popc(bw));
        }
        pn = __shfl_sync(FULL, pn, 0);
        pw = __shfl_sync(FULL, pw, 0);
        const uint32_t below = (1u << lane) - 1u;
        if (narrow) win[pn + __popc(bn & below)].order = i;
        else if (have) win[nb - 1 - (pw + __popc(bw & below))].order = i;
      }
      __syncthreads();
      {
        uint32_t nev = 0;
        const uint32_t wmin = A.group_min, n8 = sh.nnarrow;
        uint32_t w0 = 0;
        if (n8) {
          sl_group_pass<SM, R, 8>(A, L, sh, 0, n8, w0, &nev);
          w0 = (w0 + (n8 + 3u) / 4u) % NW;
        }
        if (wmin == 16u || (wmin == 8u && sh.ring8)) {
          sl_group_pass<SM, R, 16>(A, L, sh, n8, nb, w0, &nev);
          w0 = (w0 + (nb - n8 + 1u) / 2u) % NW;
        }
        if (wmin == 32u || sh.ring16) sl_group_pass<SM, R, 32>(A, L, sh, n8, nb, w0, &nev);
        if (nev) atomicAdd(&sh.nrecost, nev);
      }
      __syncthreads();
      SL_MARK(7);
      if (total <= L.wcap) break;
    }
    if (tid == 0) {
      const uint32_t passes = sh.npass;
      if (passes > 1) atomicAdd(&A.counters[24], 1u);
      if (A.trace != nullptr) atomicAdd(&A.trace[SL_HIST + SL_HCLS * A.cls + (passes < (uint32_t)SL_HP ? passes : SL_HP) - 1], 1u);
    }
    if (tid == 0 && A.trace != nullptr && sh.rec == 0 && r < 400) {
      A.trace[4 * r + 0] = sh.progress;
      A.trace[4 * r + 1] = sh.ncol;
      A.trace[4 * r + 2] = sh.alive;
      A.trace[4 * r + 3] = nF;
    }
    if (A.trace != nullptr && tid == 0) sh.visits += nF;
    if (tid == 0) {
      sh.valive -= sh.ncol;
      uint32_t stop = 0;
      if (!sh.progress) {
        stop = 1;
      } else {
        if ((uint64_t)sh.ncol * 1000 < (uint64_t)sh.alive) sh.slow++;
        else sh.slow = 0;
        if (sh.slow >= 4) stop = 1;
      }
      sh.stop = stop;
    }
    __syncthreads();
    SL_MARK(8);
    if (sh.stop) {
      r++;
      break;
    }
    if (r & 1) {
      nF = sl_compact<SM>(flist, flist2, nF, &sh.counter, [&](uint32_t f) { return (L.fstate[f] & 0x80u) != 0; });
      if (!SM) nV = sl_compact<SM>(vlist, vlist2, nV, &sh.counter, [&](uint32_t v) { return (L.vflag[v] & VF_ALIVE) != 0; });
      if (SM && A.mq_next != nullptr && sl_fits_smem(nF, sh.valive, NT / 2, A.smem_next, true)) {
        if constexpr (SM) sl_migrate<R>(A, L, sh, flist, nF, r);
        migrated = true;
        r++;
        break;
      }
    }
  }
  for (uint32_t f = tid; f < T; f += NT) {
    const bool al = L.fstate[f] & 0x80u;
    const uint32_t fo = sl_fo<SM, R>(L, f);
    if (migrated && al) continue;
    A.falive[L.tbase + fo] = al ? 1 : 0;
    if (SM && al) {
      uint32_t* g = A.face + 3 * (uint64_t)(L.tbase + fo);
      g[0] = (uint32_t)sl_vg<SM, R>(L, sl_fget<SM>(L, f, 0));
      g[1] = (uint32_t)sl_vg<SM, R>(L, sl_fget<SM>(L, f, 1));
      g[2] = (uint32_t)sl_vg<SM, R>(L, sl_fget<SM>(L, f, 2));
    }
  }
  for (uint32_t v = tid; v < U; v += NT) {
    const bool al = L.vflag[v] & VF_ALIVE;
    if (!(migrated && al)) A.valive[sl_vg<SM, R>(L, v)] = al ? 1 : 0;
  }
  if (tid == 0 && A.trace != nullptr) {
    for (int q = 0; q < SL_NPH; q++) atomicAdd((unsigned long long*)(A.trace + 1600) + q, sh.ph[q]);
    uint32_t* rec = A.lrec + SL_LREC * (size_t)sh.rec;
    const unsigned long long vis = rec[3] + sh.visits;
    const uint32_t kc = (uint32_t)((clock64() - sh.t_label) >> 10);
    if (!R) rec[0] = T;
    rec[1] = (uint32_t)r;
    rec[2] += kc;
    rec[6] += kc / (SL_THREADS / NT);
    rec[3] = (uint32_t)(vis > 0xFFFFFFFFull ? 0xFFFFFFFFull : vis);
    rec[4] += (uint32_t)sh.wins;
    if (!R) rec[5] = (SM ? 1u : ((const void*)L.key1 == (const void*)(A.key1 + L.vbase) ? 3u : 2u)) | (A.cls << 2);
  }
  if (tid == 0) {
    if (sh.nrecost) atomicAdd(&A.counters[27], sh.nrecost);
    for (int w = 0; w < 3; w++)
      if (sh.ngroup[w]) atomicAdd(&A.counters[29 + w], sh.ngroup[w]);
    if (!migrated) atomicMax(&A.counters[1], (uint32_t)r);
    if (!R) {
      atomicAdd(&A.counters[SM ? 2 : 3], 1u);
      atomicAdd(&A.counters[8 + A.cls], 1u);
    }
  }
}

__global__ void __launch_bounds__(SL_THREADS, 1) k_simp_labels(SlArgs A) {
  __shared__ SlShared sh;
  do {
    __syncthreads();
    if (threadIdx.x == 0) sh.work = atomicAdd(&A.counters[4 + A.cls], 1u);
    __syncthreads();
    const uint32_t wi = sh.work;
    if (wi >= A.K) break;
    const uint32_t l = A.order[wi];
    const uint32_t tbase = A.tri_off[l], T = A.tri_off[l + 1] - tbase;
    const uint32_t vbase = A.vert_off[l], U = A.vert_off[l + 1] - vbase;
    const uint32_t target = A.target[l];
    if (T == 0 || T <= target) continue;
    const bool fmt16 = 3ull * T <= 65536ull;
    if (sl_fits_smem(T, U, blockDim.x, A.smem_bytes)) {
      const uint32_t wcap = sl_wcap(T, U, blockDim.x, A.smem_bytes, false, A.wcap_max);
      const SlLayout y = sl_layout(T, U, false, wcap);
      SlLab<true> L;
      L.T = T; L.U = U; L.tbase = tbase; L.vbase = vbase; L.target = target;
      L.wcap = wcap;
      L.ring = (uint16_t*)(sl_smem + y.o_ring);
      L.key1 = (uint32_t*)(sl_smem + y.o_key);
      L.fmt16 = true;
      L.fc0 = (uint16_t*)(sl_smem + y.o_f0);
      L.fc1 = L.fc0 + T;
      L.fc2 = L.fc1 + T;
      L.flist = (uint16_t*)(sl_smem + y.o_fl);
      L.vlist = nullptr;
      L.flist2 = L.vlist2 = nullptr;
      L.gface = nullptr;
      L.fstate = sl_smem + y.o_fs;
      L.vflag = sl_smem + y.o_vf;
      L.vlose = sl_smem + y.o_vl;
      L.label = l;
      L.fmap = L.vmap = nullptr;
      sl_run<true, false>(A, L, sh, nullptr);
    } else {
      const SlLayout y = sl_layout(T, U);
      const size_t o_keyg = y.o_ring + (size_t)SL_WCAP * 2 * S_MAXV * 4;
      SlLab<false> L;
      L.T = T; L.U = U; L.tbase = tbase; L.vbase = vbase; L.target = target;
      L.label = l;
      L.fmap = L.vmap = nullptr;
      L.wcap = SL_WCAP < A.wcap_max ? SL_WCAP : A.wcap_max;
      L.ring = (uint32_t*)(sl_smem + y.o_ring);
      L.fc0 = L.fc1 = L.fc2 = nullptr;
      L.flist = A.flist + tbase; L.flist2 = A.flist2 + tbase;
      L.vlist = A.vlist + vbase; L.vlist2 = A.vlist2 + vbase;
      L.gface = A.face + 3 * (uint64_t)tbase;
      L.fmt16 = fmt16;
      const size_t h_fs = o_keyg + 8 * (size_t)U;
      const size_t h_vf = (h_fs + T + 3) & ~(size_t)3;
      const size_t h_vl = (h_vf + U + 3) & ~(size_t)3;
      if (h_vl + U + 4 <= A.smem_bytes) {
        L.key1 = (unsigned long long*)(sl_smem + o_keyg);
        L.fstate = sl_smem + h_fs;
        L.vflag = sl_smem + h_vf;
        L.vlose = sl_smem + h_vl;
      } else {
        L.key1 = A.key1 + vbase;
        L.fstate = A.fstate + tbase;
        L.vflag = A.vflag + vbase;
        L.vlose = A.vlose + vbase;
      }
      sl_run<false, false>(A, L, sh, nullptr);
    }
  } while (A.persist);
}

__global__ void __launch_bounds__(SL_THREADS / 2, 2) k_simp_resume(SlArgs A) {
  __shared__ SlShared sh;
  do {
    __syncthreads();
    if (threadIdx.x == 0) {
      sh.work = atomicAdd(&A.counters[20 + A.cls], 1u);
      sh.counter = A.counters[16 + A.cls];
    }
    __syncthreads();
    const uint32_t wi = sh.work;
    if (wi >= sh.counter) break;
    const uint32_t* hdr = A.mq + SL_MREC * (size_t)wi;
    const uint32_t l = hdr[0];
    const uint32_t T = hdr[4], U = hdr[5];
    const uint32_t wcap = sl_wcap(T, U, blockDim.x, A.smem_bytes, true, A.wcap_max);
    const SlLayout y = sl_layout(T, U, true, wcap);
    SlLab<true> L;
    L.T = T; L.U = U; L.tbase = A.tri_off[l]; L.vbase = A.vert_off[l]; L.target = A.target[l];
    L.label = l;
    L.wcap = wcap;
    L.ring = (uint16_t*)(sl_smem + y.o_ring);
    L.key1 = (uint32_t*)(sl_smem + y.o_key);
    L.fmt16 = true;
    L.fc0 = (uint16_t*)(sl_smem + y.o_f0);
    L.fc1 = L.fc0 + T;
    L.fc2 = L.fc1 + T;
    L.flist = (uint16_t*)(sl_smem + y.o_fl);
    L.vlist = nullptr;
    L.flist2 = L.vlist2 = nullptr;
    L.gface = nullptr;
    L.fstate = sl_smem + y.o_fs;
    L.vflag = sl_smem + y.o_vf;
    L.vlose = sl_smem + y.o_vl;
    L.fmap = (uint16_t*)(sl_smem + y.o_fm);
    L.vmap = (uint16_t*)(sl_smem + y.o_vm);
    sl_run<true, true>(A, L, sh, hdr);
  } while (A.persist);
}

__global__ void __launch_bounds__(256)
    k_simp_flags_u32(const uint8_t* __restrict__ a, uint64_t n, uint32_t* __restrict__ out) {
  const uint64_t i = blockIdx.x * (uint64_t)blockDim.x + threadIdx.x;
  if (i < n) out[i] = a[i];
}

__global__ void __launch_bounds__(256)
    k_simp_new_offsets(const uint32_t* __restrict__ old_off, const uint32_t* __restrict__ scan,
                       uint32_t K2, uint64_t n, uint32_t total, uint32_t* __restrict__ new_off) {
  const uint32_t l = blockIdx.x * blockDim.x + threadIdx.x;
  if (l < K2) new_off[l] = (old_off[l] < n) ? scan[old_off[l]] : total;
}

__global__ void __launch_bounds__(256)
    k_simp_compact_verts(Simp s, const uint32_t* __restrict__ vscan, float* __restrict__ pos_f) {
  const uint64_t v = blockIdx.x * (uint64_t)blockDim.x + threadIdx.x;
  if (v >= s.U || !s.valive[v]) return;
  const uint32_t n = vscan[v];
  pos_f[3 * (uint64_t)n + 0] = __double2float_rn(s.pos[3 * v + 0]);
  pos_f[3 * (uint64_t)n + 1] = __double2float_rn(s.pos[3 * v + 1]);
  pos_f[3 * (uint64_t)n + 2] = __double2float_rn(s.pos[3 * v + 2]);
}

__global__ void __launch_bounds__(256)
    k_simp_compact_faces(Simp s, const uint32_t* __restrict__ vscan, const uint32_t* __restrict__ fscan,
                         const uint32_t* __restrict__ new_vert_off, uint32_t* __restrict__ faces_out) {
  const uint64_t f = blockIdx.x * (uint64_t)blockDim.x + threadIdx.x;
  if (f >= s.T || !s.falive[f]) return;
  const uint32_t n = fscan[f];
  const uint32_t base = new_vert_off[s.flabel[f]];
  for (int k = 0; k < 3; k++) faces_out[3 * (uint64_t)n + k] = vscan[s.face[3 * f + k]] - base;
}

__global__ void __launch_bounds__(256)
    k_simp_export(const float* __restrict__ pos_f, uint64_t first, uint64_t count, float sx, float sy,
                  float sz, float* __restrict__ out) {
  const uint64_t i = blockIdx.x * (uint64_t)blockDim.x + threadIdx.x;
  if (i >= count) return;
  out[3 * i + 0] = __fadd_rn(pos_f[3 * (first + i) + 0], sx);
  out[3 * i + 1] = __fadd_rn(pos_f[3 * (first + i) + 1], sy);
  out[3 * i + 2] = __fadd_rn(pos_f[3 * (first + i) + 2], sz);
}

int simp_export_positions(ign_ctx* ctx, const float* pos_f, uint64_t first, uint64_t count,
                          const float shift[3], float* d_out) {
  if (count == 0) return IGN_OK;
  IGN_LAUNCH(ctx, k_simp_export, blocks_for(count, 256), 256, 0, pos_f, first, count, shift[0], shift[1],
             shift[2], d_out);
  return IGN_OK;
}

}

using namespace ign;

extern "C" int ign_mesh_simplify(ign_mesher* m, const float resolution[3], int reduction_factor,
                                 float max_error) {
  IGN_REQUIRE(m && resolution, IGN_ERR_INVALID, "null argument");
  ign_ctx* ctx = m->ctx;
  IGN_TRY(activate(ctx));
  IGN_REQUIRE(!m->simplified, IGN_ERR_INVALID, "mesher is already simplified; call mesh() again");
  IGN_REQUIRE(reduction_factor >= 1, IGN_ERR_INVALID, "reduction_factor must be >= 1");
  m->res[0] = resolution[0];
  m->res[1] = resolution[1];
  m->res[2] = resolution[2];
  m->simp_factor = reduction_factor;
  m->simp_max_error = max_error;
  m->simp_rounds = 0;
  m->simp_labels_smem = m->simp_labels_gmem = 0;
  for (int c = 0; c < SL_NCLASS; c++) m->simp_labels_class[c] = m->simp_migrations[c] = 0;
  m->simp_passes[0] = m->simp_passes[1] = 0;
  m->simp_costs[0] = m->simp_costs[1] = m->simp_costs[2] = 0;
  m->simp_groups[0] = m->simp_groups[1] = m->simp_groups[2] = 0;
  const uint64_t U = m->U, T = m->T, K = m->K;
  if (T == 0 || U == 0) {
    m->simplified = true;
    m->d_pos_f = nullptr;
    return IGN_OK;
  }
  size_t sortb = 0, scanb = 0;
  cub::DeviceRadixSort::SortPairs(nullptr, sortb, (const uint32_t*)nullptr, (uint32_t*)nullptr,
                                  (const uint32_t*)nullptr, (uint32_t*)nullptr, (int)(3 * T));
  cub::DeviceScan::ExclusiveSum(nullptr, scanb, (const uint32_t*)nullptr, (uint32_t*)nullptr,
                                (int)(3 * T));
  const size_t tmpb = (sortb > scanb ? sortb : scanb) + 256;
  ScratchFrame f(ctx);
  Simp s;
  s.U = U;
  s.T = T;
  uint32_t *node_v, *node_h, *vscan, *vflag32, *d_target, *d_tri_off, *d_vert_off, *d_new_tri_off, *d_new_vert_off;
  uint32_t *d_order, *flags, *gl_f[2], *gl_v[2], *sorted_v, *sorted_h, *d_mq;
  uint16_t* finv;
  uint8_t *fstate, *vflag, *vlose;
  unsigned long long* key1;
  float* ecost;
  void* tmp;
  IGN_TRY(f.take(&s.pos, U * 3));
  IGN_TRY(f.take(&s.Q, U * 10));
  IGN_TRY(f.take(&s.face, 3 * T));
  IGN_TRY(f.take(&s.vf, U * S_VCAP));
  IGN_TRY(f.take(&node_v, 3 * T));
  IGN_TRY(f.take(&node_h, 3 * T));
  IGN_TRY(f.take(&s.flabel, T));
  IGN_TRY(f.take(&s.falive, T));
  IGN_TRY(f.take(&fstate, T));
  IGN_TRY(f.take(&s.valive, U));
  IGN_TRY(f.take(&s.vbound, U));
  IGN_TRY(f.take(&vflag, U));
  IGN_TRY(f.take(&vlose, U));
  IGN_TRY(f.take(&s.vn, U));
  IGN_TRY(f.take(&vscan, U));
  IGN_TRY(f.take(&vflag32, U));
  IGN_TRY(f.take(&key1, U));
  IGN_TRY(f.take(&d_target, K + 2));
  IGN_TRY(f.take(&d_tri_off, K + 2));
  IGN_TRY(f.take(&d_vert_off, K + 2));
  IGN_TRY(f.take(&d_new_tri_off, K + 2));
  IGN_TRY(f.take(&d_new_vert_off, K + 2));
  IGN_TRY(f.take(&d_order, K + 2));
  IGN_TRY(f.take(&flags, 64));
  IGN_TRY(f.take(&ecost, 3 * T));
  IGN_TRY(f.take(&gl_f[0], T));
  IGN_TRY(f.take(&gl_f[1], T));
  IGN_TRY(f.take(&gl_v[0], U));
  IGN_TRY(f.take(&gl_v[1], U));
  IGN_TRY(f.take(&d_mq, (size_t)SL_MREC * K * (SL_NCLASS - 1)));
  IGN_TRY(f.take(&finv, T));
  IGN_TRY(f.take(&tmp, tmpb));
  IGN_TRY(f.take(&sorted_v, 3 * T));
  IGN_TRY(f.take(&sorted_h, 3 * T));
  s.tri_off = d_tri_off;

  std::vector<uint32_t> target(K + 2, 0);
  for (uint64_t l = 1; l <= K; l++)
    target[l] = (m->tri_off[l + 1] - m->tri_off[l]) / (uint32_t)reduction_factor;
  const size_t sl_static = ((sizeof(SlShared) + 255) / 256) * 256 + 1024;
  size_t sl_dyn[SL_NCLASS];
  for (int c = 0; c < SL_NCLASS; c++) sl_dyn[c] = (232448 / (size_t)(1024 / SL_CLASS_THREADS[c]) - sl_static) & ~(size_t)255;
  std::vector<uint32_t> lcls(K + 2, 0);
  uint32_t ccount[SL_NCLASS] = {0, 0, 0};
  for (uint64_t l = 1; l <= K; l++) {
    const uint32_t tl = m->tri_off[l + 1] - m->tri_off[l], ul = m->vert_off[l + 1] - m->vert_off[l];
    int c = SL_NCLASS - 1;
    while (c > 0 && !sl_fits_smem(tl, ul, SL_CLASS_THREADS[c], sl_dyn[c])) c--;
    lcls[l] = (uint32_t)c;
    ccount[c]++;
  }
  std::vector<uint32_t> order(K);
  for (uint64_t l = 0; l < K; l++) order[l] = (uint32_t)(l + 1);
  std::sort(order.begin(), order.end(), [&](uint32_t a, uint32_t b) {
    const uint32_t ta = m->tri_off[a + 1] - m->tri_off[a], tb = m->tri_off[b + 1] - m->tri_off[b];
    if (lcls[a] != lcls[b]) return lcls[a] < lcls[b];
    return ta != tb ? ta > tb : a < b;
  });
  IGN_TRY(small_h2d(ctx, d_target, target.data(), (K + 2) * 4));
  IGN_TRY(small_h2d(ctx, d_tri_off, m->tri_off.data(), (K + 2) * 4));
  IGN_TRY(small_h2d(ctx, d_vert_off, m->vert_off.data(), (K + 2) * 4));
  IGN_TRY(small_h2d(ctx, d_order, order.data(), K * 4));
  IGN_LAUNCH(ctx, k_simp_init_verts, blocks_for(U, 256), 256, 0, m->d_uniq_vkeys, U, (double)resolution[0],
             (double)resolution[1], (double)resolution[2], s.pos, s.valive, s.vbound, s.vn);
  IGN_LAUNCH(ctx, k_simp_init_faces, blocks_for(T, 256), 256, 0, m->d_faces, d_tri_off, d_vert_off, (uint32_t)K, T,
             s.face, s.flabel, s.falive, node_v, node_h);
  {
    int bits = 1;
    while (bits < 32 && (1ull << bits) < U) bits++;
    size_t tb = tmpb;
    IGN_CUDA(cub::DeviceRadixSort::SortPairs(tmp, tb, node_v, sorted_v, node_h, sorted_h, (int)(3 * T), 0, bits,
                                             ctx->stream));
    ctx->launches += 3;
  }
  IGN_CUDA(cudaMemsetAsync(flags, 0, 32 * 4, ctx->stream));
  IGN_LAUNCH(ctx, k_simp_link, blocks_for(3 * T, 256), 256, 0, sorted_v, sorted_h, (uint64_t)(3 * T), s.vf, s.vn,
             flags + 12);
  IGN_LAUNCH(ctx, k_simp_quadrics, blocks_for(U, 128), 128, 0, s);
  IGN_LAUNCH(ctx, k_simp_boundary, blocks_for(3 * T, 256), 256, 0, s);
  const double max_err2 = (double)max_error * (double)max_error;
  IGN_LAUNCH(ctx, k_simp_ecost, blocks_for(T, 256), 256, 0, s, max_err2, ecost, fstate, flags + 26);

  IGN_CUDA(cudaFuncSetAttribute(k_simp_labels, cudaFuncAttributeMaxDynamicSharedMemorySize, (int)sl_dyn[0]));
  IGN_CUDA(cudaFuncSetAttribute(k_simp_resume, cudaFuncAttributeMaxDynamicSharedMemorySize, (int)sl_dyn[1]));
  SlArgs A;
  A.pos = s.pos; A.Q = s.Q; A.face = s.face; A.falive = s.falive; A.valive = s.valive; A.vbound = s.vbound;
  A.ecost = ecost; A.key1 = key1; A.fstate = fstate; A.vflag = vflag; A.vlose = vlose; A.finv = finv;
  A.flist = gl_f[0]; A.flist2 = gl_f[1]; A.vlist = gl_v[0]; A.vlist2 = gl_v[1];
  A.tri_off = d_tri_off; A.vert_off = d_vert_off; A.target = d_target;
  A.counters = flags;
  A.max_err2 = max_err2;
  A.max_rounds = 400;
  A.trace = nullptr;
  A.lrec = nullptr;
  if (getenv("IGN_SIMP_TRACE") != nullptr) {
    IGN_TRY(f.take(&A.trace, SL_HIST + SL_NCLASS * SL_HCLS));
    IGN_TRY(f.take(&A.lrec, (size_t)K * SL_LREC + 16));
    IGN_CUDA(cudaMemsetAsync(A.trace, 0, (SL_HIST + SL_NCLASS * SL_HCLS) * 4, ctx->stream));
    IGN_CUDA(cudaMemsetAsync(A.lrec, 0, ((size_t)K * SL_LREC + 16) * 4, ctx->stream));
  }
  const char* force_gmem = getenv("IGN_SIMP_GMEM");
  const bool gmem_only = force_gmem && force_gmem[0] == '1';
  const char* wcap_env = getenv("IGN_SIMP_WCAP");
  A.wcap_max = wcap_env && atoi(wcap_env) > 0 ? (uint32_t)atoi(wcap_env) : 0xFFFFFFFFu;
  const char* group_env = getenv("IGN_SIMP_GROUP");
  const int group = group_env ? atoi(group_env) : 0;
  A.group_min = group == 16 || group == 32 ? (uint32_t)group : 8u;
  {
    const int slot = prof_begin(ctx, IGN_PROF_SIMP);
    const char* pe = getenv("IGN_SIMP_PERSIST");
    A.persist = (pe && pe[0] == '1') ? 1 : 0;
    uint32_t resume[SL_NCLASS] = {0, 0, 0};
    if (!gmem_only)
      for (int c = 1; c < SL_NCLASS; c++) resume[c] = resume[c - 1] + ccount[c - 1];
    int prio = 0;
    IGN_CUDA(cudaStreamGetPriority(ctx->stream, &prio));
    cudaStream_t cs[SL_NCLASS] = {ctx->stream, nullptr, nullptr};
    cudaEvent_t ev[SL_NCLASS] = {nullptr, nullptr, nullptr};
    cudaError_t err = cudaEventCreateWithFlags(&ev[0], cudaEventDisableTiming);
    if (err == cudaSuccess) err = cudaEventRecord(ev[0], ctx->stream);
    for (int c = 1; c < SL_NCLASS && err == cudaSuccess; c++) {
      if (ccount[c] == 0 && resume[c] == 0) continue;
      err = cudaStreamCreateWithPriority(&cs[c], cudaStreamNonBlocking, prio);
      if (err == cudaSuccess) err = cudaStreamWaitEvent(cs[c], ev[0], 0);
      if (err == cudaSuccess) err = cudaEventCreateWithFlags(&ev[c], cudaEventDisableTiming);
    }
    cudaEvent_t ev_full = nullptr;
    if (err == cudaSuccess && resume[1]) err = cudaEventCreateWithFlags(&ev_full, cudaEventDisableTiming);
    uint32_t base = 0;
    for (int c = 0; c < SL_NCLASS && err == cudaSuccess; c++) {
      const uint32_t n = ccount[c], nt = (uint32_t)SL_CLASS_THREADS[c];
      A.cls = (uint32_t)c;
      A.smem_bytes = gmem_only ? 0u : (uint32_t)sl_dyn[c];
      A.smem_next = c + 1 < SL_NCLASS ? (uint32_t)sl_dyn[c + 1] : 0u;
      A.mq_next = (c + 1 < SL_NCLASS && resume[c + 1]) ? d_mq + (size_t)SL_MREC * K * c : nullptr;
      A.mq = nullptr;
      const uint64_t slots = (uint64_t)ctx->sm_count * (1024 / nt);
      if (n) {
        A.order = d_order + base; A.K = n; A.base = base;
        const unsigned grid = A.persist ? (unsigned)(n < slots ? n : slots) : n;
        k_simp_labels<<<grid, nt, sl_dyn[c], cs[c]>>>(A);
        ctx->launches++;
        err = cudaGetLastError();
        base += n;
      }
      if (c == 0 && ev_full && err == cudaSuccess) err = cudaEventRecord(ev_full, cs[0]);
    }
    for (int c = 1; c < SL_NCLASS && err == cudaSuccess; c++) {
      if (resume[c]) {
        const uint32_t nt = (uint32_t)SL_CLASS_THREADS[c];
        err = cudaStreamWaitEvent(cs[c], c == 1 ? ev_full : ev[c - 1], 0);
        if (err != cudaSuccess) break;
        A.cls = (uint32_t)c;
        A.smem_bytes = (uint32_t)sl_dyn[c];
        A.smem_next = c + 1 < SL_NCLASS ? (uint32_t)sl_dyn[c + 1] : 0u;
        A.mq_next = (c + 1 < SL_NCLASS) ? d_mq + (size_t)SL_MREC * K * c : nullptr;
        A.mq = d_mq + (size_t)SL_MREC * K * (c - 1);
        const uint64_t slots = (uint64_t)ctx->sm_count * (1024 / nt);
        const unsigned grid = A.persist ? (unsigned)(resume[c] < slots ? resume[c] : slots) : resume[c];
        k_simp_resume<<<grid, nt, sl_dyn[c], cs[c]>>>(A);
        ctx->launches++;
        err = cudaGetLastError();
      }
      if (ev[c] && err == cudaSuccess) err = cudaEventRecord(ev[c], cs[c]);
    }
    for (int c = 1; c < SL_NCLASS && err == cudaSuccess; c++)
      if (ev[c]) err = cudaStreamWaitEvent(ctx->stream, ev[c], 0);
    if (ev_full) cudaEventDestroy(ev_full);
    for (int c = 0; c < SL_NCLASS; c++) {
      if (ev[c]) cudaEventDestroy(ev[c]);
      if (c > 0 && cs[c]) cudaStreamDestroy(cs[c]);
    }
    prof_end(ctx, slot);
    IGN_CUDA(err);
  }

  uint32_t* fscan = node_v;
  uint32_t* fflag = node_h;
  size_t tb = tmpb;
  IGN_LAUNCH(ctx, k_simp_flags_u32, blocks_for(U, 256), 256, 0, s.valive, U, vflag32);
  IGN_CUDA(cub::DeviceScan::ExclusiveSum(tmp, tb, vflag32, vscan, (int)U, ctx->stream));
  IGN_LAUNCH(ctx, k_simp_flags_u32, blocks_for(T, 256), 256, 0, s.falive, T, fflag);
  tb = tmpb;
  IGN_CUDA(cub::DeviceScan::ExclusiveSum(tmp, tb, fflag, fscan, (int)T, ctx->stream));
  ctx->launches += 4;
  uint32_t last[4], hflags[32];
  IGN_TRY(small_d2h(ctx, &last[0], vscan + (U - 1), 4));
  IGN_TRY(small_d2h(ctx, &last[1], vflag32 + (U - 1), 4));
  IGN_TRY(small_d2h(ctx, &last[2], fscan + (T - 1), 4));
  IGN_TRY(small_d2h(ctx, &last[3], fflag + (T - 1), 4));
  IGN_TRY(small_d2h(ctx, hflags, flags, sizeof(hflags)));
  IGN_TRY(small_sync(ctx));
  if (hflags[12] != 0) {
    set_error("simplify: a vertex has more than %d incident faces", S_VCAP);
    return IGN_ERR_UNSUPPORTED;
  }
  if (A.trace) {
    std::vector<uint32_t> tr(SL_HIST);
    IGN_CUDA(cudaMemcpy(tr.data(), A.trace, SL_HIST * 4, cudaMemcpyDeviceToHost));
    unsigned long long phs[SL_NPH];
    IGN_CUDA(cudaMemcpy(phs, A.trace + 1600, sizeof(phs), cudaMemcpyDeviceToHost));
    static const char* names[SL_NPH] = {"P1", "P2 keys", "P3 lose", "P4 select", "setup", "E1 rings", "E2a cost", "E2 validate+collapse+recost", "stop+compact"};
    unsigned long long tot = 0;
    for (int q = 0; q < SL_NPH; q++) tot += phs[q];
    for (int q = 0; q < SL_NPH; q++)
      fprintf(stderr, "phase %-27s %6.2f %%  %10.3f Mcycles\n", names[q], 100.0 * phs[q] / (tot ? tot : 1), phs[q] / 1e6);
    fprintf(stderr, "cost evaluations: %u initial (k_simp_ecost), %u after collapses (E2), %u half-edges without a cost in P2\n",
            hflags[26], hflags[27], hflags[28]);
    fprintf(stderr, "winners by E2 group width: %u of 8 lanes, %u of 16, %u of 32\n", hflags[29], hflags[30], hflags[31]);
    fprintf(stderr, "winners rejected by E2 flip tests: %u on the u side only, %u on the v side only, %u on both\n",
            tr[SL_TFLIP], tr[SL_TFLIP + 1], tr[SL_TFLIP + 2]);
    {
      std::vector<uint32_t> rec(SL_LREC * (size_t)K);
      IGN_CUDA(cudaMemcpy(rec.data(), A.lrec, rec.size() * 4, cudaMemcpyDeviceToHost));
      static const uint32_t edges[] = {0, 500, 1000, 2000, 3000, 4000, 6000, 8000, 10000, 12000, 16000, 32000, 64000, 0xFFFFFFFFu};
      const int nedges = (int)(sizeof(edges) / sizeof(edges[0]));
      for (int c = 0; c < SL_NCLASS; c++) {
        int per_sm = 0;
        IGN_CUDA(cudaOccupancyMaxActiveBlocksPerMultiprocessor(&per_sm, k_simp_labels, SL_CLASS_THREADS[c], sl_dyn[c]));
        fprintf(stderr, "size class %d: %4d threads, %6zu B dynamic shared memory, %d CTAs per SM, %u labels\n", c,
                SL_CLASS_THREADS[c], sl_dyn[c], per_sm, ccount[c]);
      }
      fprintf(stderr, "%7s %12s %7s %8s %10s %10s %10s %9s %9s  class(sm/hy/gl)\n", "threads", "faces<", "labels", "rounds", "Mcycles", "SM Mcyc", "Mvisits", "kwins", "cyc/round");
      double sr = 0, sv = 0, sc = 0, srr = 0, svv = 0, srv = 0, src = 0, svc = 0;
      uint64_t sm_total[SL_NCLASS] = {0, 0, 0};
      for (int szc = 0; szc < SL_NCLASS; szc++) {
        for (int b = 0; b + 1 < nedges; b++) {
          uint64_t n = 0, rounds = 0, kc = 0, ksm = 0, vis = 0, wins = 0, cls[4] = {0, 0, 0, 0};
          for (uint64_t i = 0; i < K; i++) {
            const uint32_t* q = &rec[SL_LREC * i];
            if (q[1] == 0 || (int)(q[5] >> 2) != szc || q[0] < edges[b] || q[0] >= edges[b + 1]) continue;
            n++; rounds += q[1]; kc += q[2]; ksm += q[6]; vis += q[3]; wins += q[4]; cls[q[5] & 3]++;
            const double R = q[1], V = q[3], C = q[2] * 1024.0;
            sr += R; sv += V; sc += C; srr += R * R; svv += V * V; srv += R * V; src += R * C; svc += V * C;
          }
          sm_total[szc] += ksm;
          if (n) fprintf(stderr, "%7d %12u %7llu %8.1f %10.2f %10.2f %10.3f %9.1f %9.0f  %llu/%llu/%llu\n", SL_CLASS_THREADS[szc], edges[b + 1],
                         (unsigned long long)n, (double)rounds / n, kc * 1024.0 / 1e6, ksm * 1024.0 / 1e6, vis / 1e6, wins / 1e3,
                         rounds ? kc * 1024.0 / rounds : 0.0, (unsigned long long)cls[1], (unsigned long long)cls[2],
                         (unsigned long long)cls[3]);
        }
      }
      fprintf(stderr, "SM Mcycles by starting class: %.0f + %.0f + %.0f = %.0f; labels resumed in the 512- / 256-thread class: %u / %u\n",
              sm_total[0] * 1024.0 / 1e6, sm_total[1] * 1024.0 / 1e6, sm_total[2] * 1024.0 / 1e6,
              (sm_total[0] + sm_total[1] + sm_total[2]) * 1024.0 / 1e6, hflags[17], hflags[18]);
      std::vector<uint32_t> hist(SL_NCLASS * SL_HCLS);
      IGN_CUDA(cudaMemcpy(hist.data(), A.trace + SL_HIST, hist.size() * 4, cudaMemcpyDeviceToHost));
      for (int c = 0; c < SL_NCLASS; c++) {
        const uint32_t* h = &hist[SL_HCLS * c];
        fprintf(stderr, "class %d passes/round (1..%d+):", SL_CLASS_THREADS[c], SL_HP);
        for (int b = 0; b < SL_HP; b++) fprintf(stderr, " %u", h[b]);
        fprintf(stderr, "\nclass %d winners/round (bins of 16, last %d+):", SL_CLASS_THREADS[c], 16 * (SL_HW - 1));
        for (int b = 0; b < SL_HW; b++) fprintf(stderr, " %u", h[SL_HP + b]);
        fprintf(stderr, "\nclass %d ring length per winner side (0..%d, more):", SL_CLASS_THREADS[c], S_MAXV);
        for (int b = 0; b < SL_HR; b++) fprintf(stderr, " %u", h[SL_HP + SL_HW + b]);
        fprintf(stderr, "\n");
      }
      const double det = srr * svv - srv * srv;
      if (det != 0) fprintf(stderr, "fit: cycles ~= %.0f * rounds + %.2f * face visits   (totals: %.0f rounds, %.3g visits, %.3g cycles)\n",
                            (src * svv - svc * srv) / det, (svc * srr - src * srv) / det, sr, sv, sc);
    }
    for (int r = 0; r < 400 && getenv("IGN_SIMP_TRACE_ROUNDS") && (tr[4 * r + 2] || tr[4 * r + 3]); r++)
      fprintf(stderr, "gpu round %d progress %u collapses %u alive %u list %u\n", r, tr[4 * r], tr[4 * r + 1], tr[4 * r + 2], tr[4 * r + 3]);
  }
  m->simp_rounds = (int)hflags[1];
  m->simp_labels_smem = hflags[2];
  m->simp_labels_gmem = hflags[3];
  for (int c = 0; c < SL_NCLASS; c++) m->simp_labels_class[c] = hflags[8 + c];
  for (int c = 0; c < SL_NCLASS; c++) m->simp_migrations[c] = hflags[16 + c];
  m->simp_passes[0] = hflags[24];
  m->simp_passes[1] = hflags[25];
  for (int i = 0; i < 3; i++) m->simp_costs[i] = hflags[26 + i];
  for (int i = 0; i < 3; i++) m->simp_groups[i] = hflags[29 + i];
  const uint32_t U2 = last[0] + last[1], T2 = last[2] + last[3];
  IGN_LAUNCH(ctx, k_simp_new_offsets, blocks_for(K + 2, 256), 256, 0, d_vert_off, vscan, (uint32_t)(K + 2), U, U2,
                   d_new_vert_off);
  IGN_LAUNCH(ctx, k_simp_new_offsets, blocks_for(K + 2, 256), 256, 0, d_tri_off, fscan, (uint32_t)(K + 2), T, T2,
                   d_new_tri_off);
  float* pos_f = (float*)m->d_uniq_vkeys;
  IGN_LAUNCH(ctx, k_simp_compact_verts, blocks_for(U, 256), 256, 0, s, vscan, pos_f);
  IGN_LAUNCH(ctx, k_simp_compact_faces, blocks_for(T, 256), 256, 0, s, vscan, fscan, d_new_vert_off, m->d_faces);
  IGN_TRY(small_d2h(ctx, m->tri_off.data(), d_new_tri_off, (K + 2) * 4));
  IGN_TRY(small_d2h(ctx, m->vert_off.data(), d_new_vert_off, (K + 2) * 4));
  IGN_TRY(small_sync(ctx));
  m->U = U2;
  m->T = T2;
  m->d_pos_f = pos_f;
  m->simplified = true;
  m->present.clear();
  for (uint64_t l = 1; l <= K; l++)
    if (m->tri_off[l + 1] > m->tri_off[l]) m->present.push_back(m->ids[l - 1]);
  return IGN_OK;
}

extern "C" int ign_mesh_simplify_stats(ign_mesher* m, uint32_t stats[6]) {
  IGN_REQUIRE(m && stats, IGN_ERR_INVALID, "null argument");
  IGN_REQUIRE(m->simplified, IGN_ERR_INVALID, "mesher is not simplified");
  stats[0] = (uint32_t)m->simp_rounds;
  stats[1] = m->simp_labels_smem;
  stats[2] = m->simp_labels_gmem;
  for (int c = 0; c < SL_NCLASS; c++) stats[3 + c] = m->simp_labels_class[c];
  return IGN_OK;
}

extern "C" int ign_mesh_simplify_migrations(ign_mesher* m, uint32_t resumed[3]) {
  IGN_REQUIRE(m && resumed, IGN_ERR_INVALID, "null argument");
  IGN_REQUIRE(m->simplified, IGN_ERR_INVALID, "mesher is not simplified");
  for (int c = 0; c < SL_NCLASS; c++) resumed[c] = m->simp_migrations[c];
  return IGN_OK;
}

extern "C" int ign_mesh_simplify_passes(ign_mesher* m, uint32_t counts[2]) {
  IGN_REQUIRE(m && counts, IGN_ERR_INVALID, "null argument");
  IGN_REQUIRE(m->simplified, IGN_ERR_INVALID, "mesher is not simplified");
  counts[0] = m->simp_passes[0];
  counts[1] = m->simp_passes[1];
  return IGN_OK;
}

extern "C" int ign_mesh_simplify_costs(ign_mesher* m, uint32_t counts[3]) {
  IGN_REQUIRE(m && counts, IGN_ERR_INVALID, "null argument");
  IGN_REQUIRE(m->simplified, IGN_ERR_INVALID, "mesher is not simplified");
  for (int i = 0; i < 3; i++) counts[i] = m->simp_costs[i];
  return IGN_OK;
}

extern "C" int ign_mesh_simplify_groups(ign_mesher* m, uint32_t counts[3]) {
  IGN_REQUIRE(m && counts, IGN_ERR_INVALID, "null argument");
  IGN_REQUIRE(m->simplified, IGN_ERR_INVALID, "mesher is not simplified");
  for (int i = 0; i < 3; i++) counts[i] = m->simp_groups[i];
  return IGN_OK;
}
```

Before: 6285.

## Restructure mesh welding with block-scan MC, narrow vertex keys, atomic vertex-face linking

Marching cubes now computes per-block triangle counts and writes at precomputed block offsets, replacing the global atomic counter. It emits separate label and packed cube/case records, so welding can sort narrower, templated vertex keys carrying only coordinate bits, with label checks done when finding heads and a later per-label reorder. In simplify, the radix sort used to build vertex-to-face adjacency is replaced by atomic slot claims followed by a per-vertex insertion sort, which removes the sort scratch buffers. Phase tracing and profiling spans gated by an environment variable are added, at the cost of extra passes and more complex indirection.

```diff
diff --git a/igneous_b200/csrc/common.cuh b/igneous_b200/csrc/common.cuh
--- a/igneous_b200/csrc/common.cuh
+++ b/igneous_b200/csrc/common.cuh
@@ -173,6 +173,36 @@
     IGN_CUDA(cudaGetLastError());                                                \
   } while (0)
 
+struct ProfSpan {
+  ProfSpan(ign_ctx* ctx, int cls) : ctx_(ctx), slot_(prof_begin(ctx, cls)) {}
+  ~ProfSpan() { end(); }
+  ProfSpan(const ProfSpan&) = delete;
+  ProfSpan& operator=(const ProfSpan&) = delete;
+  void end() {
+    prof_end(ctx_, slot_);
+    slot_ = -1;
+  }
+
+ private:
+  ign_ctx* ctx_;
+  int slot_;
+};
+
+class PhaseTrace {
+ public:
+  PhaseTrace(ign_ctx* ctx, const char* call);
+  ~PhaseTrace();
+  PhaseTrace(const PhaseTrace&) = delete;
+  PhaseTrace& operator=(const PhaseTrace&) = delete;
+  void mark(const char* phase);
+
+ private:
+  ign_ctx* ctx_;
+  const char* call_;
+  std::vector<cudaEvent_t> ev_;
+  std::vector<const char*> names_;
+};
+
 static inline unsigned blocks_for(uint64_t n, unsigned threads) {
   return (unsigned)((n + threads - 1) / threads);
 }
diff --git a/igneous_b200/csrc/ctx.cu b/igneous_b200/csrc/ctx.cu
--- a/igneous_b200/csrc/ctx.cu
+++ b/igneous_b200/csrc/ctx.cu
@@ -1,4 +1,5 @@
 #include <stdarg.h>
+#include <stdlib.h>
 #include <string.h>
 
 #include "common.cuh"
@@ -192,6 +193,46 @@
 
 void prof_end(ign_ctx* ctx, int slot) {
   if (slot >= 0) cudaEventRecord(ctx->prof[slot].b, ctx->stream);
+}
+
+PhaseTrace::PhaseTrace(ign_ctx* ctx, const char* call) : ctx_(ctx), call_(call) {
+  const char* e = getenv("IGN_MESH_TRACE");
+  if (!e || e[0] != '1') return;
+  cudaEvent_t ev;
+  if (cudaEventCreate(&ev) != cudaSuccess) return;
+  cudaEventRecord(ev, ctx_->stream);
+  ev_.push_back(ev);
+}
+
+void PhaseTrace::mark(const char* phase) {
+  if (ev_.empty()) return;
+  cudaEvent_t ev;
+  if (cudaEventCreate(&ev) != cudaSuccess) return;
+  cudaEventRecord(ev, ctx_->stream);
+  ev_.push_back(ev);
+  names_.push_back(phase);
+}
+
+PhaseTrace::~PhaseTrace() {
+  if (ev_.empty()) return;
+  char head[96];
+  snprintf(head, sizeof(head), "ign_mesh_trace %s ctx=%p", call_, (void*)ctx_);
+  std::string line = head;
+  if (cudaEventSynchronize(ev_.back()) == cudaSuccess) {
+    for (size_t i = 0; i < names_.size(); i++) {
+      float ms = 0;
+      if (cudaEventElapsedTime(&ms, ev_[i], ev_[i + 1]) != cudaSuccess) ms = -1;
+      char buf[96];
+      snprintf(buf, sizeof(buf), " %s=%.4f", names_[i], ms);
+      line += buf;
+    }
+    char buf[64];
+    snprintf(buf, sizeof(buf), " scratch_high_mb=%.1f", ctx_->scratch_high / 1048576.0);
+    line += buf;
+  }
+  cudaGetLastError();
+  fprintf(stderr, "%s\n", line.c_str());
+  for (cudaEvent_t ev : ev_) cudaEventDestroy(ev);
 }
 
 }
diff --git a/igneous_b200/csrc/mesh.cu b/igneous_b200/csrc/mesh.cu
--- a/igneous_b200/csrc/mesh.cu
+++ b/igneous_b200/csrc/mesh.cu
@@ -11,10 +11,10 @@
 namespace ign {
 
 constexpr unsigned MFULL = 0xFFFFFFFFu;
-constexpr int TRI_T_BITS = 3, TRI_CUBE_BITS = 30;
+constexpr int TRI_CASE_BITS = 8, TRI_T_BITS = 3;
+constexpr int TRI_CUBE_SHIFT = TRI_CASE_BITS + TRI_T_BITS;
 constexpr int V_COORD_BITS = 11;
 constexpr int V_LABEL_SHIFT = 3 * V_COORD_BITS;
-constexpr int TRI_LABEL_SHIFT = TRI_T_BITS + TRI_CUBE_BITS;
 
 __constant__ int8_t c_edge_mid[12][3] = {{1, 0, 0}, {2, 1, 0}, {1, 2, 0}, {0, 1, 0},
                                          {1, 0, 2}, {2, 1, 2}, {1, 2, 2}, {0, 1, 2},
@@ -41,9 +41,10 @@
 template <bool EMIT>
 __global__ void __launch_bounds__(256)
     k_mc(const uint32_t* __restrict__ lab, uint32_t sx, uint32_t sy, uint32_t sz,
-         unsigned long long* total, uint64_t* __restrict__ keys, uint8_t* __restrict__ cases,
-         uint64_t capacity) {
+         uint64_t* __restrict__ block_tris, const uint64_t* __restrict__ block_off,
+         uint32_t* __restrict__ tri_lab, uint64_t* __restrict__ tri_rec, uint64_t capacity) {
   __shared__ uint8_t s_ntri[256];
+  __shared__ uint32_t s_warp[8];
   for (int i = threadIdx.x; i < 256; i += blockDim.x) s_ntri[i] = c_mc.ntri[i];
   __syncthreads();
   const uint32_t cx = sx - 1, cy = sy - 1, cz = sz - 1;
@@ -80,23 +81,24 @@
       mine += s_ntri[idxs[k]];
     }
   }
-  if (!EMIT) {
-    uint32_t s = mine;
-    for (int d = 16; d > 0; d >>= 1) s += __shfl_down_sync(MFULL, s, d);
-    if (lane == 0 && s) atomicAdd(total, (unsigned long long)s);
-    return;
-  }
   uint32_t incl = mine;
   for (int d = 1; d < 32; d <<= 1) {
     const uint32_t v = __shfl_up_sync(MFULL, incl, d);
     if (lane >= d) incl += v;
   }
-  const uint32_t warp_total = __shfl_sync(MFULL, incl, 31);
-  if (warp_total == 0) return;
-  unsigned long long base = 0;
-  if (lane == 31) base = atomicAdd(total, (unsigned long long)warp_total);
-  base = __shfl_sync(MFULL, base, 31);
-  uint64_t pos = base + (incl - mine);
+  const uint32_t warp = threadIdx.x >> 5;
+  if (lane == 31) s_warp[warp] = incl;
+  __syncthreads();
+  uint32_t before = 0, block_total = 0;
+  for (uint32_t w = 0; w < 8; w++) {
+    before += w < warp ? s_warp[w] : 0u;
+    block_total += s_warp[w];
+  }
+  if (!EMIT) {
+    if (threadIdx.x == 0) block_tris[blockIdx.x] = block_total;
+    return;
+  }
+  uint64_t pos = block_off[blockIdx.x] + before + (incl - mine);
   if (active) {
     const uint64_t cube = (uint64_t)t;
 #pragma unroll
@@ -104,8 +106,8 @@
       const uint32_t n = s_ntri[idxs[k]];
       for (uint32_t tt = 0; tt < n; tt++) {
         if (pos < capacity) {
-          keys[pos] = ((uint64_t)c[k] << TRI_LABEL_SHIFT) | (cube << TRI_T_BITS) | tt;
-          cases[pos] = idxs[k];
+          tri_lab[pos] = c[k];
+          tri_rec[pos] = (cube << TRI_CUBE_SHIFT) | (tt << TRI_CASE_BITS) | idxs[k];
         }
         pos++;
       }
@@ -113,36 +115,35 @@
   }
 }
 
-__global__ void __launch_bounds__(256)
-    k_tri_vertices(const uint64_t* __restrict__ keys, const uint8_t* __restrict__ cases, uint64_t T,
-                   uint32_t cx, uint32_t cy, uint64_t* __restrict__ vkeys,
-                   uint32_t* __restrict__ corner) {
+template <typename K>
+__global__ void __launch_bounds__(256)
+    k_tri_vertices(const uint64_t* __restrict__ tri_rec, uint64_t T, uint32_t cx, uint32_t cy, int bx, int bxy,
+                   K* __restrict__ vkeys, uint32_t* __restrict__ corner) {
   const uint64_t t = blockIdx.x * (uint64_t)blockDim.x + threadIdx.x;
   if (t >= T) return;
-  const uint64_t key = keys[t];
-  const uint64_t label = key >> TRI_LABEL_SHIFT;
-  const uint64_t cube = (key >> TRI_T_BITS) & ((1ull << TRI_CUBE_BITS) - 1);
-  const uint32_t tt = (uint32_t)(key & ((1u << TRI_T_BITS) - 1));
+  const uint64_t rec = tri_rec[t];
+  const uint64_t cube = rec >> TRI_CUBE_SHIFT;
+  const uint32_t tt = (uint32_t)(rec >> TRI_CASE_BITS) & ((1u << TRI_T_BITS) - 1);
   const uint32_t x = (uint32_t)(cube % cx), y = (uint32_t)((cube / cx) % cy),
                  z = (uint32_t)(cube / ((uint64_t)cx * cy));
-  const int8_t* row = c_mc.tri[cases[t]];
+  const int8_t* row = c_mc.tri[rec & ((1u << TRI_CASE_BITS) - 1)];
 #pragma unroll
   for (int v = 0; v < 3; v++) {
     const int e = row[3 * tt + (2 - v)];
-    const uint64_t vx = 2 * x + c_edge_mid[e][0], vy = 2 * y + c_edge_mid[e][1],
-                   vz = 2 * z + c_edge_mid[e][2];
-    vkeys[3 * t + v] = (label << V_LABEL_SHIFT) | (vz << (2 * V_COORD_BITS)) | (vy << V_COORD_BITS) | vx;
+    const K vx = 2 * x + c_edge_mid[e][0], vy = 2 * y + c_edge_mid[e][1], vz = 2 * z + c_edge_mid[e][2];
+    vkeys[3 * t + v] = (vz << bxy) | (vy << bx) | vx;
     corner[3 * t + v] = (uint32_t)(3 * t + v);
   }
 }
 
-__global__ void __launch_bounds__(256)
-    k_label_starts(const uint64_t* __restrict__ keys, uint64_t n, int shift,
+template <typename K>
+__global__ void __launch_bounds__(256)
+    k_label_starts(const K* __restrict__ keys, uint64_t n, int shift,
                    uint32_t* __restrict__ start ) {
   const uint64_t i = blockIdx.x * (uint64_t)blockDim.x + threadIdx.x;
   if (i >= n) return;
-  const uint64_t label = keys[i] >> shift;
-  if (i == 0 || (keys[i - 1] >> shift) != label) start[label] = (uint32_t)i;
+  const uint64_t label = (uint64_t)keys[i] >> shift;
+  if (i == 0 || ((uint64_t)keys[i - 1] >> shift) != label) start[label] = (uint32_t)i;
 }
 
 __global__ void __launch_bounds__(256) k_fill_u32(uint32_t* a, uint32_t value, uint32_t n) {
@@ -150,30 +151,53 @@
   if (i < n) a[i] = value;
 }
 
-__global__ void __launch_bounds__(256)
-    k_vertex_heads(const uint64_t* __restrict__ vkeys_sorted, uint64_t n, uint32_t* __restrict__ heads) {
+template <typename K>
+__global__ void __launch_bounds__(256)
+    k_vertex_heads(const K* __restrict__ vkeys_sorted, const uint32_t* __restrict__ corner_sorted,
+                   const uint32_t* __restrict__ tri_lab, uint64_t n, uint32_t* __restrict__ heads) {
   const uint64_t i = blockIdx.x * (uint64_t)blockDim.x + threadIdx.x;
-  if (i < n) heads[i] = (i == 0 || vkeys_sorted[i - 1] != vkeys_sorted[i]) ? 1u : 0u;
-}
-
-__global__ void __launch_bounds__(256)
-    k_vertex_assign(const uint64_t* __restrict__ vkeys_sorted, const uint32_t* __restrict__ corner_sorted,
-                    const uint32_t* __restrict__ heads, const uint32_t* __restrict__ rank, uint64_t n,
-                    uint64_t* __restrict__ uniq_vkeys, uint32_t* __restrict__ face_global) {
+  if (i >= n) return;
+  heads[i] = (i == 0 || vkeys_sorted[i - 1] != vkeys_sorted[i] ||
+              tri_lab[corner_sorted[i - 1] / 3] != tri_lab[corner_sorted[i] / 3]) ? 1u : 0u;
+}
+
+template <typename K>
+__global__ void __launch_bounds__(256)
+    k_vertex_assign(const K* __restrict__ vkeys_sorted, const uint32_t* __restrict__ corner_sorted,
+                    const uint32_t* __restrict__ tri_lab, const uint32_t* __restrict__ heads,
+                    const uint32_t* __restrict__ rank, uint64_t n, int bx, int bxy, uint32_t* __restrict__ vlab,
+                    uint64_t* __restrict__ vpos, uint32_t* __restrict__ vidx, uint32_t* __restrict__ face_pos) {
   const uint64_t i = blockIdx.x * (uint64_t)blockDim.x + threadIdx.x;
   if (i >= n) return;
   const uint32_t id = rank[i] + heads[i] - 1;
-  if (heads[i]) uniq_vkeys[id] = vkeys_sorted[i];
-  face_global[corner_sorted[i]] = id;
-}
-
-__global__ void __launch_bounds__(256)
-    k_faces_local(const uint64_t* __restrict__ tri_keys, const uint32_t* __restrict__ vert_off,
-                  uint64_t T, uint32_t* __restrict__ faces) {
+  const uint32_t c = corner_sorted[i];
+  if (heads[i]) {
+    const uint64_t k = vkeys_sorted[i];
+    const uint64_t vx = k & ((1ull << bx) - 1), vy = (k >> bx) & ((1ull << (bxy - bx)) - 1), vz = k >> bxy;
+    vlab[id] = tri_lab[c / 3];
+    vpos[id] = (vz << (2 * V_COORD_BITS)) | (vy << V_COORD_BITS) | vx;
+    vidx[id] = id;
+  }
+  face_pos[c] = id;
+}
+
+__global__ void __launch_bounds__(256)
+    k_vertex_order(const uint32_t* __restrict__ vlab_sorted, const uint32_t* __restrict__ perm,
+                   const uint64_t* __restrict__ vpos, uint64_t U, uint64_t* __restrict__ uniq_vkeys,
+                   uint32_t* __restrict__ final_id) {
+  const uint64_t u = blockIdx.x * (uint64_t)blockDim.x + threadIdx.x;
+  if (u >= U) return;
+  const uint32_t j = perm[u];
+  uniq_vkeys[u] = ((uint64_t)vlab_sorted[u] << V_LABEL_SHIFT) | vpos[j];
+  final_id[j] = (uint32_t)u;
+}
+
+__global__ void __launch_bounds__(256)
+    k_faces_local(const uint32_t* __restrict__ tri_lab, const uint32_t* __restrict__ final_id,
+                  const uint32_t* __restrict__ vert_off, uint64_t T, uint32_t* __restrict__ faces) {
   const uint64_t i = blockIdx.x * (uint64_t)blockDim.x + threadIdx.x;
   if (i >= 3 * T) return;
-  const uint64_t label = tri_keys[i / 3] >> TRI_LABEL_SHIFT;
-  faces[i] -= vert_off[label];
+  faces[i] = final_id[faces[i]] - vert_off[tri_lab[i / 3]];
 }
 
 __global__ void __launch_bounds__(256)
@@ -234,135 +258,37 @@
   return b;
 }
 
-extern "C" {
-
-int ign_mesh_free(ign_mesher* m) {
-  if (!m) return IGN_OK;
-  cudaSetDevice(m->ctx->device);
-  if (m->pooled) {
-    m->ctx->mesh_pool_busy = 0;
-  } else {
-    if (m->d_uniq_vkeys) cudaFree(m->d_uniq_vkeys);
-    if (m->d_faces) cudaFree(m->d_faces);
-  }
-  delete m;
-  return IGN_OK;
-}
-
-int ign_mesh_begin_dev(ign_ctx* ctx, const void* labels, int dtype, uint64_t sx, uint64_t sy,
-                       uint64_t sz, ign_mesher** out) {
-  IGN_TRY(activate(ctx));
-  IGN_REQUIRE(labels && out, IGN_ERR_INVALID, "null argument");
-  *out = nullptr;
-  IGN_REQUIRE(sx >= 1 && sy >= 1 && sz >= 1, IGN_ERR_INVALID, "empty volume");
-  IGN_REQUIRE(sx <= 1023 && sy <= 1023 && sz <= 1023, IGN_ERR_UNSUPPORTED,
-              "mesher: task of %llux%llux%llu exceeds the 1023^3 limit of the packed vertex format",
-              (unsigned long long)sx, (unsigned long long)sy, (unsigned long long)sz);
-  IGN_TRY(load_tables(ctx));
-  const uint64_t n = sx * sy * sz;
-
-  ign_mesher* m = new ign_mesher();
-  m->ctx = ctx;
-  m->K = m->T = m->U = 0;
-  m->d_uniq_vkeys = nullptr;
-  m->d_faces = nullptr;
-  m->pooled = false;
-  m->simplified = false;
-  m->d_pos_f = nullptr;
-  m->simp_factor = 0;
-  m->simp_max_error = 0;
-  m->simp_rounds = 0;
-  struct Guard {
-    ign_mesher* m;
-    ~Guard() { ign_mesh_free(m); }
-  } guard{m};
-  ScratchFrame f(ctx);
-
-  uint32_t* d_lab;
-  IGN_TRY(f.take(&d_lab, n));
-  uint64_t K = 0;
-  {
-    ScratchFrame fu(ctx);
-    uint64_t* d_uniq;
-    IGN_TRY(fu.take(&d_uniq, n));
-    IGN_TRY(ign_renumber_dev(ctx, labels, dtype, n, d_lab, d_uniq, n, &K));
-    m->K = K;
-    m->ids.resize(K);
-    if (K) {
-      IGN_TRY(small_d2h(ctx, m->ids.data(), d_uniq, K * 8));
-      IGN_TRY(small_sync(ctx));
-    }
-  }
-  m->tri_off.assign(K + 2, 0);
-  m->vert_off.assign(K + 2, 0);
-  if (K == 0 || sx < 2 || sy < 2 || sz < 2) {
-    guard.m = nullptr;
-    *out = m;
-    return IGN_OK;
-  }
-  IGN_REQUIRE(K < (1ull << 31), IGN_ERR_OVERFLOW, "mesher: too many labels");
-
-  unsigned long long* d_total;
-  IGN_TRY(f.take(&d_total, 32));
-  const uint64_t ncubes = (sx - 1) * (sy - 1) * (sz - 1);
-  const unsigned grid = blocks_for(ncubes, 256);
-  unsigned long long T = 0;
-  IGN_CUDA(cudaMemsetAsync(d_total, 0, 8, ctx->stream));
-  IGN_LAUNCH(ctx, (k_mc<false>), grid, 256, 0, d_lab, (uint32_t)sx, (uint32_t)sy, (uint32_t)sz, d_total,
-             (uint64_t*)nullptr, (uint8_t*)nullptr, 0ull);
-  IGN_TRY(small_d2h(ctx, &T, d_total, 8));
-  IGN_TRY(small_sync(ctx));
-  m->T = T;
-  if (T == 0) {
-    guard.m = nullptr;
-    *out = m;
-    return IGN_OK;
-  }
-  IGN_REQUIRE(3 * T <= (unsigned long long)INT_MAX, IGN_ERR_OVERFLOW,
-              "mesher: %llu triangles exceed 2^31 - 1 corners; split the volume into tasks", T);
-
+template <typename K>
+static int weld(ign_ctx* ctx, ScratchFrame& f, PhaseTrace& trace, ign_mesher* m, const uint32_t* tlab_s,
+                const uint64_t* rec_s, uint64_t T, uint64_t sx, uint64_t sy, uint64_t sz, int label_bits,
+                uint32_t** final_id) {
+  const int bx = bits_for(2 * (sx - 1)), bxy = bx + bits_for(2 * (sy - 1)), bits = bxy + bits_for(2 * (sz - 1));
   size_t sort1 = 0, sort2 = 0, scanb = 0;
-  cub::DeviceRadixSort::SortPairs(nullptr, sort1, (const uint64_t*)nullptr, (uint64_t*)nullptr,
-                                  (const uint8_t*)nullptr, (uint8_t*)nullptr, (int)T);
-  cub::DeviceRadixSort::SortPairs(nullptr, sort2, (const uint64_t*)nullptr, (uint64_t*)nullptr,
+  cub::DeviceRadixSort::SortPairs(nullptr, sort1, (const K*)nullptr, (K*)nullptr, (const uint32_t*)nullptr,
+                                  (uint32_t*)nullptr, (int)(3 * T));
+  cub::DeviceRadixSort::SortPairs(nullptr, sort2, (const uint32_t*)nullptr, (uint32_t*)nullptr,
                                   (const uint32_t*)nullptr, (uint32_t*)nullptr, (int)(3 * T));
   cub::DeviceScan::ExclusiveSum(nullptr, scanb, (const uint32_t*)nullptr, (uint32_t*)nullptr, (int)(3 * T));
   size_t tmp_bytes = sort1 > sort2 ? sort1 : sort2;
   if (scanb > tmp_bytes) tmp_bytes = scanb;
-  uint64_t *keys, *keys_s, *vkeys, *vkeys_s;
-  uint8_t *cases, *cases_s;
-  uint32_t *corner, *corner_s, *heads, *rank, *d_tri_off, *d_vert_off;
+  K *vkeys, *vkeys_s;
+  uint32_t *corner, *corner_s, *heads, *rank;
   void* tmp;
-  IGN_TRY(f.take(&keys, T));
-  IGN_TRY(f.take(&keys_s, T));
-  IGN_TRY(f.take(&cases, T));
-  IGN_TRY(f.take(&cases_s, T));
   IGN_TRY(f.take(&vkeys, 3 * T));
   IGN_TRY(f.take(&vkeys_s, 3 * T));
   IGN_TRY(f.take(&corner, 3 * T));
   IGN_TRY(f.take(&corner_s, 3 * T));
   IGN_TRY(f.take(&heads, 3 * T));
   IGN_TRY(f.take(&rank, 3 * T));
-  IGN_TRY(f.take(&d_tri_off, K + 2));
-  IGN_TRY(f.take(&d_vert_off, K + 2));
   IGN_TRY(f.take(&tmp, tmp_bytes));
-
-  IGN_CUDA(cudaMemsetAsync(d_total, 0, 8, ctx->stream));
-  IGN_LAUNCH(ctx, (k_mc<true>), grid, 256, 0, d_lab, (uint32_t)sx, (uint32_t)sy, (uint32_t)sz, d_total, keys,
-             cases, (uint64_t)T);
-  const int label_bits = bits_for(K);
+  IGN_LAUNCH(ctx, k_tri_vertices<K>, blocks_for(T, 256), 256, 0, rec_s, T, (uint32_t)(sx - 1), (uint32_t)(sy - 1), bx,
+             bxy, vkeys, corner);
   size_t tb = tmp_bytes;
-  IGN_CUDA(cub::DeviceRadixSort::SortPairs(tmp, tb, keys, keys_s, cases, cases_s, (int)T, 0,
-                                           TRI_LABEL_SHIFT + label_bits, ctx->stream));
+  IGN_CUDA(cub::DeviceRadixSort::SortPairs(tmp, tb, vkeys, vkeys_s, corner, corner_s, (int)(3 * T), 0, bits,
+                                           ctx->stream));
   ctx->launches += 4;
-
-  IGN_LAUNCH(ctx, k_tri_vertices, blocks_for(T, 256), 256, 0, keys_s, cases_s, (uint64_t)T, (uint32_t)(sx - 1),
-             (uint32_t)(sy - 1), vkeys, corner);
-  tb = tmp_bytes;
-  IGN_CUDA(cub::DeviceRadixSort::SortPairs(tmp, tb, vkeys, vkeys_s, corner, corner_s, (int)(3 * T), 0,
-                                           V_LABEL_SHIFT + label_bits, ctx->stream));
-  ctx->launches += 4;
-  IGN_LAUNCH(ctx, k_vertex_heads, blocks_for(3 * T, 256), 256, 0, vkeys_s, (uint64_t)(3 * T), heads);
+  trace.mark("weld_sort");
+  IGN_LAUNCH(ctx, k_vertex_heads<K>, blocks_for(3 * T, 256), 256, 0, vkeys_s, corner_s, tlab_s, 3 * T, heads);
   tb = tmp_bytes;
   IGN_CUDA(cub::DeviceScan::ExclusiveSum(tmp, tb, heads, rank, (int)(3 * T), ctx->stream));
   ctx->launches += 2;
@@ -393,13 +319,158 @@
       IGN_CUDA(cudaMalloc((void**)&m->d_uniq_vkeys, U * 12));
     }
   }
-  IGN_LAUNCH(ctx, k_vertex_assign, blocks_for(3 * T, 256), 256, 0, vkeys_s, corner_s, heads, rank,
-             (uint64_t)(3 * T), m->d_uniq_vkeys, m->d_faces);
+  uint32_t* vlab = corner;
+  uint32_t* vidx = (uint32_t*)vkeys;
+  uint32_t *vlab_s, *perm;
+  uint64_t* vpos;
+  IGN_TRY(f.take(&vlab_s, U));
+  IGN_TRY(f.take(&perm, U));
+  IGN_TRY(f.take(&vpos, U));
+  IGN_TRY(f.take(final_id, U));
+  IGN_LAUNCH(ctx, k_vertex_assign<K>, blocks_for(3 * T, 256), 256, 0, vkeys_s, corner_s, tlab_s, heads, rank, 3 * T,
+             bx, bxy, vlab, vpos, vidx, m->d_faces);
+  tb = tmp_bytes;
+  IGN_CUDA(cub::DeviceRadixSort::SortPairs(tmp, tb, vlab, vlab_s, vidx, perm, (int)U, 0, label_bits, ctx->stream));
+  ctx->launches += 4;
+  IGN_LAUNCH(ctx, k_vertex_order, blocks_for(U, 256), 256, 0, vlab_s, perm, vpos, U, m->d_uniq_vkeys, *final_id);
+  return IGN_OK;
+}
+
+extern "C" {
+
+int ign_mesh_free(ign_mesher* m) {
+  if (!m) return IGN_OK;
+  cudaSetDevice(m->ctx->device);
+  if (m->pooled) {
+    m->ctx->mesh_pool_busy = 0;
+  } else {
+    if (m->d_uniq_vkeys) cudaFree(m->d_uniq_vkeys);
+    if (m->d_faces) cudaFree(m->d_faces);
+  }
+  delete m;
+  return IGN_OK;
+}
+
+int ign_mesh_begin_dev(ign_ctx* ctx, const void* labels, int dtype, uint64_t sx, uint64_t sy,
+                       uint64_t sz, ign_mesher** out) {
+  IGN_TRY(activate(ctx));
+  IGN_REQUIRE(labels && out, IGN_ERR_INVALID, "null argument");
+  *out = nullptr;
+  IGN_REQUIRE(sx >= 1 && sy >= 1 && sz >= 1, IGN_ERR_INVALID, "empty volume");
+  IGN_REQUIRE(sx <= 1023 && sy <= 1023 && sz <= 1023, IGN_ERR_UNSUPPORTED,
+              "mesher: task of %llux%llux%llu exceeds the 1023^3 limit of the packed vertex format",
+              (unsigned long long)sx, (unsigned long long)sy, (unsigned long long)sz);
+  IGN_TRY(load_tables(ctx));
+  const uint64_t n = sx * sy * sz;
+
+  ign_mesher* m = new ign_mesher();
+  m->ctx = ctx;
+  m->K = m->T = m->U = 0;
+  m->d_uniq_vkeys = nullptr;
+  m->d_faces = nullptr;
+  m->pooled = false;
+  m->simplified = false;
+  m->d_pos_f = nullptr;
+  m->simp_factor = 0;
+  m->simp_max_error = 0;
+  m->simp_rounds = 0;
+  struct Guard {
+    ign_mesher* m;
+    ~Guard() { ign_mesh_free(m); }
+  } guard{m};
+  ScratchFrame f(ctx);
+  ProfSpan prof(ctx, IGN_PROF_MC);
+  PhaseTrace trace(ctx, "begin");
+
+  uint32_t* d_lab;
+  IGN_TRY(f.take(&d_lab, n));
+  uint64_t K = 0;
+  {
+    ScratchFrame fu(ctx);
+    uint64_t* d_uniq;
+    IGN_TRY(fu.take(&d_uniq, n));
+    IGN_TRY(ign_renumber_dev(ctx, labels, dtype, n, d_lab, d_uniq, n, &K));
+    m->K = K;
+    m->ids.resize(K);
+    if (K) {
+      IGN_TRY(small_d2h(ctx, m->ids.data(), d_uniq, K * 8));
+      IGN_TRY(small_sync(ctx));
+    }
+  }
+  trace.mark("renumber");
+  m->tri_off.assign(K + 2, 0);
+  m->vert_off.assign(K + 2, 0);
+  if (K == 0 || sx < 2 || sy < 2 || sz < 2) {
+    guard.m = nullptr;
+    *out = m;
+    return IGN_OK;
+  }
+  IGN_REQUIRE(K < (1ull << 31), IGN_ERR_OVERFLOW, "mesher: too many labels");
+
+  const uint64_t ncubes = (sx - 1) * (sy - 1) * (sz - 1);
+  const unsigned grid = blocks_for(ncubes, 256);
+  uint64_t *d_btris, *d_boff;
+  void* btmp;
+  size_t btmp_bytes = 0;
+  cub::DeviceScan::ExclusiveSum(nullptr, btmp_bytes, (const uint64_t*)nullptr, (uint64_t*)nullptr, (int)grid + 1);
+  IGN_TRY(f.take(&d_btris, grid + 1));
+  IGN_TRY(f.take(&d_boff, grid + 1));
+  IGN_TRY(f.take(&btmp, btmp_bytes));
+  IGN_CUDA(cudaMemsetAsync(d_btris + grid, 0, 8, ctx->stream));
+  IGN_LAUNCH(ctx, (k_mc<false>), grid, 256, 0, d_lab, (uint32_t)sx, (uint32_t)sy, (uint32_t)sz, d_btris,
+             (const uint64_t*)nullptr, (uint32_t*)nullptr, (uint64_t*)nullptr, 0ull);
+  IGN_CUDA(cub::DeviceScan::ExclusiveSum(btmp, btmp_bytes, d_btris, d_boff, (int)grid + 1, ctx->stream));
+  ctx->launches += 2;
+  unsigned long long T = 0;
+  IGN_TRY(small_d2h(ctx, &T, d_boff + grid, 8));
+  IGN_TRY(small_sync(ctx));
+  trace.mark("mc_count");
+  m->T = T;
+  if (T == 0) {
+    guard.m = nullptr;
+    *out = m;
+    return IGN_OK;
+  }
+  IGN_REQUIRE(3 * T <= (unsigned long long)INT_MAX, IGN_ERR_OVERFLOW,
+              "mesher: %llu triangles exceed 2^31 - 1 corners; split the volume into tasks", T);
+
+  size_t tmp_bytes = 0;
+  cub::DeviceRadixSort::SortPairs(nullptr, tmp_bytes, (const uint32_t*)nullptr, (uint32_t*)nullptr,
+                                  (const uint64_t*)nullptr, (uint64_t*)nullptr, (int)T);
+  uint64_t *rec, *rec_s;
+  uint32_t *tlab, *tlab_s, *d_tri_off, *d_vert_off, *final_id;
+  IGN_TRY(f.take(&tlab, T));
+  IGN_TRY(f.take(&tlab_s, T));
+  IGN_TRY(f.take(&rec, T));
+  IGN_TRY(f.take(&rec_s, T));
+  IGN_TRY(f.take(&d_tri_off, K + 2));
+  IGN_TRY(f.take(&d_vert_off, K + 2));
+
+  IGN_LAUNCH(ctx, (k_mc<true>), grid, 256, 0, d_lab, (uint32_t)sx, (uint32_t)sy, (uint32_t)sz,
+             (uint64_t*)nullptr, d_boff, tlab, rec, (uint64_t)T);
+  trace.mark("mc_emit");
+  const int label_bits = bits_for(K);
+  {
+    ScratchFrame ft(ctx);
+    void* tmp;
+    IGN_TRY(ft.take(&tmp, tmp_bytes));
+    IGN_CUDA(cub::DeviceRadixSort::SortPairs(tmp, tmp_bytes, tlab, tlab_s, rec, rec_s, (int)T, 0, label_bits,
+                                             ctx->stream));
+    ctx->launches += 4;
+  }
+  trace.mark("tri_sort");
+
+  const bool key32 = bits_for(2 * (sx - 1)) + bits_for(2 * (sy - 1)) + bits_for(2 * (sz - 1)) <= 32;
+  IGN_TRY(key32 ? weld<uint32_t>(ctx, f, trace, m, tlab_s, rec_s, T, sx, sy, sz, label_bits, &final_id)
+                : weld<uint64_t>(ctx, f, trace, m, tlab_s, rec_s, T, sx, sy, sz, label_bits, &final_id));
+  const uint64_t U = m->U;
+  trace.mark("weld_ids");
 
   IGN_LAUNCH(ctx, k_fill_u32, blocks_for(K + 2, 256), 256, 0, d_tri_off, (uint32_t)T, (uint32_t)(K + 2));
   IGN_LAUNCH(ctx, k_fill_u32, blocks_for(K + 2, 256), 256, 0, d_vert_off, (uint32_t)U, (uint32_t)(K + 2));
-  IGN_LAUNCH(ctx, k_label_starts, blocks_for(T, 256), 256, 0, keys_s, (uint64_t)T, TRI_LABEL_SHIFT, d_tri_off);
-  IGN_LAUNCH(ctx, k_label_starts, blocks_for(U, 256), 256, 0, m->d_uniq_vkeys, U, V_LABEL_SHIFT, d_vert_off);
+  IGN_LAUNCH(ctx, k_label_starts<uint32_t>, blocks_for(T, 256), 256, 0, tlab_s, (uint64_t)T, 0, d_tri_off);
+  IGN_LAUNCH(ctx, k_label_starts<uint64_t>, blocks_for(U, 256), 256, 0, m->d_uniq_vkeys, U, V_LABEL_SHIFT,
+             d_vert_off);
   IGN_TRY(small_d2h(ctx, m->tri_off.data(), d_tri_off, (K + 2) * 4));
   IGN_TRY(small_d2h(ctx, m->vert_off.data(), d_vert_off, (K + 2) * 4));
   IGN_TRY(small_sync(ctx));
@@ -408,7 +479,9 @@
     if (m->vert_off[l] > m->vert_off[l + 1]) m->vert_off[l] = m->vert_off[l + 1];
   }
   IGN_TRY(small_h2d(ctx, d_vert_off, m->vert_off.data(), (K + 2) * 4));
-  IGN_LAUNCH(ctx, k_faces_local, blocks_for(3 * T, 256), 256, 0, keys_s, d_vert_off, (uint64_t)T, m->d_faces);
+  IGN_LAUNCH(ctx, k_faces_local, blocks_for(3 * T, 256), 256, 0, tlab_s, final_id, d_vert_off, (uint64_t)T, m->d_faces);
+  prof.end();
+  trace.mark("offsets");
   IGN_CUDA(cudaStreamSynchronize(ctx->stream));
   for (uint64_t l = 1; l <= K; l++)
     if (m->tri_off[l + 1] > m->tri_off[l]) m->present.push_back(m->ids[l - 1]);
diff --git a/igneous_b200/csrc/simplify.cu b/igneous_b200/csrc/simplify.cu
--- a/igneous_b200/csrc/simplify.cu
+++ b/igneous_b200/csrc/simplify.cu
@@ -155,8 +155,7 @@
     k_simp_init_faces(const uint32_t* __restrict__ faces_local, const uint32_t* __restrict__ tri_off,
                       const uint32_t* __restrict__ vert_off, uint32_t K, uint64_t T,
                       uint32_t* __restrict__ face, uint32_t* __restrict__ flabel,
-                      uint8_t* __restrict__ falive, uint32_t* __restrict__ node_vertex,
-                      uint32_t* __restrict__ node_id) {
+                      uint8_t* __restrict__ falive) {
   const uint64_t f = blockIdx.x * (uint64_t)blockDim.x + threadIdx.x;
   if (f >= T) return;
   uint32_t lo = 1, hi = K;
@@ -168,30 +167,37 @@
   flabel[f] = lo;
   falive[f] = 1;
   for (int k = 0; k < 3; k++) {
-    const uint32_t g = faces_local[3 * f + k] + vert_off[lo];
-    face[3 * f + k] = g;
-    node_vertex[3 * f + k] = g;
-    node_id[3 * f + k] = (uint32_t)(3 * f + k);
+    face[3 * f + k] = faces_local[3 * f + k] + vert_off[lo];
   }
 }
 
 __global__ void __launch_bounds__(256)
-    k_simp_link(const uint32_t* __restrict__ sv, const uint32_t* __restrict__ sh, uint64_t n,
-                uint32_t* __restrict__ vf, uint32_t* __restrict__ vn, uint32_t* overflow) {
-  const uint64_t i = blockIdx.x * (uint64_t)blockDim.x + threadIdx.x;
-  if (i >= n) return;
-  const uint32_t v = sv[i];
-  if (i > 0 && sv[i - 1] == v) return;
-  uint32_t c = 0;
-  for (uint64_t j = i; j < n && sv[j] == v; j++) {
-    if (c < S_VCAP) vf[(uint64_t)v * S_VCAP + c] = sh[j];
-    c++;
-  }
+    k_simp_link_claim(const uint32_t* __restrict__ face, uint64_t n, uint32_t* __restrict__ vf,
+                      uint32_t* __restrict__ vn) {
+  const uint64_t h = blockIdx.x * (uint64_t)blockDim.x + threadIdx.x;
+  if (h >= n) return;
+  const uint32_t v = face[h];
+  const uint32_t c = atomicAdd(&vn[v], 1u);
+  if (c < S_VCAP) vf[(uint64_t)v * S_VCAP + c] = (uint32_t)h;
+}
+
+__global__ void __launch_bounds__(256)
+    k_simp_link_order(uint64_t U, uint32_t* __restrict__ vf, uint32_t* __restrict__ vn, uint32_t* overflow) {
+  const uint64_t v = blockIdx.x * (uint64_t)blockDim.x + threadIdx.x;
+  if (v >= U) return;
+  uint32_t c = vn[v];
   if (c > S_VCAP) {
     *overflow = 1;
     c = S_VCAP;
-  }
-  vn[v] = c;
+    vn[v] = c;
+  }
+  uint32_t* l = vf + v * S_VCAP;
+  for (uint32_t i = 1; i < c; i++) {
+    const uint32_t x = l[i];
+    uint32_t j = i;
+    for (; j > 0 && l[j - 1] > x; j--) l[j] = l[j - 1];
+    l[j] = x;
+  }
 }
 
 __global__ void __launch_bounds__(128) k_simp_quadrics(Simp s) {
@@ -1409,18 +1415,18 @@
     m->d_pos_f = nullptr;
     return IGN_OK;
   }
-  size_t sortb = 0, scanb = 0;
-  cub::DeviceRadixSort::SortPairs(nullptr, sortb, (const uint32_t*)nullptr, (uint32_t*)nullptr,
-                                  (const uint32_t*)nullptr, (uint32_t*)nullptr, (int)(3 * T));
+  ProfSpan prof_init(ctx, IGN_PROF_MC);
+  PhaseTrace trace(ctx, "simplify");
+  size_t scanb = 0;
   cub::DeviceScan::ExclusiveSum(nullptr, scanb, (const uint32_t*)nullptr, (uint32_t*)nullptr,
-                                (int)(3 * T));
-  const size_t tmpb = (sortb > scanb ? sortb : scanb) + 256;
+                                (int)(U > T ? U : T));
+  const size_t tmpb = scanb + 256;
   ScratchFrame f(ctx);
   Simp s;
   s.U = U;
   s.T = T;
-  uint32_t *node_v, *node_h, *vscan, *vflag32, *d_target, *d_tri_off, *d_vert_off, *d_new_tri_off, *d_new_vert_off;
-  uint32_t *d_order, *flags, *gl_f[2], *gl_v[2], *sorted_v, *sorted_h, *d_mq;
+  uint32_t *fscan, *fflag, *vscan, *vflag32, *d_target, *d_tri_off, *d_vert_off, *d_new_tri_off, *d_new_vert_off;
+  uint32_t *d_order, *flags, *gl_f[2], *gl_v[2], *d_mq;
   uint16_t* finv;
   uint8_t *fstate, *vflag, *vlose;
   unsigned long long* key1;
@@ -1430,8 +1436,8 @@
   IGN_TRY(f.take(&s.Q, U * 10));
   IGN_TRY(f.take(&s.face, 3 * T));
   IGN_TRY(f.take(&s.vf, U * S_VCAP));
-  IGN_TRY(f.take(&node_v, 3 * T));
-  IGN_TRY(f.take(&node_h, 3 * T));
+  IGN_TRY(f.take(&fscan, T));
+  IGN_TRY(f.take(&fflag, T));
   IGN_TRY(f.take(&s.flabel, T));
   IGN_TRY(f.take(&s.falive, T));
   IGN_TRY(f.take(&fstate, T));
@@ -1458,8 +1464,6 @@
   IGN_TRY(f.take(&d_mq, (size_t)SL_MREC * K * (SL_NCLASS - 1)));
   IGN_TRY(f.take(&finv, T));
   IGN_TRY(f.take(&tmp, tmpb));
-  IGN_TRY(f.take(&sorted_v, 3 * T));
-  IGN_TRY(f.take(&sorted_h, 3 * T));
   s.tri_off = d_tri_off;
 
   std::vector<uint32_t> target(K + 2, 0);
@@ -1491,23 +1495,21 @@
   IGN_LAUNCH(ctx, k_simp_init_verts, blocks_for(U, 256), 256, 0, m->d_uniq_vkeys, U, (double)resolution[0],
              (double)resolution[1], (double)resolution[2], s.pos, s.valive, s.vbound, s.vn);
   IGN_LAUNCH(ctx, k_simp_init_faces, blocks_for(T, 256), 256, 0, m->d_faces, d_tri_off, d_vert_off, (uint32_t)K, T,
-             s.face, s.flabel, s.falive, node_v, node_h);
-  {
-    int bits = 1;
-    while (bits < 32 && (1ull << bits) < U) bits++;
-    size_t tb = tmpb;
-    IGN_CUDA(cub::DeviceRadixSort::SortPairs(tmp, tb, node_v, sorted_v, node_h, sorted_h, (int)(3 * T), 0, bits,
-                                             ctx->stream));
-    ctx->launches += 3;
-  }
+             s.face, s.flabel, s.falive);
+  trace.mark("init_setup");
   IGN_CUDA(cudaMemsetAsync(flags, 0, 32 * 4, ctx->stream));
-  IGN_LAUNCH(ctx, k_simp_link, blocks_for(3 * T, 256), 256, 0, sorted_v, sorted_h, (uint64_t)(3 * T), s.vf, s.vn,
-             flags + 12);
+  IGN_LAUNCH(ctx, k_simp_link_claim, blocks_for(3 * T, 256), 256, 0, s.face, (uint64_t)(3 * T), s.vf, s.vn);
+  IGN_LAUNCH(ctx, k_simp_link_order, blocks_for(U, 256), 256, 0, U, s.vf, s.vn, flags + 12);
+  trace.mark("init_link");
   IGN_LAUNCH(ctx, k_simp_quadrics, blocks_for(U, 128), 128, 0, s);
+  trace.mark("init_quadrics");
   IGN_LAUNCH(ctx, k_simp_boundary, blocks_for(3 * T, 256), 256, 0, s);
+  trace.mark("init_boundary");
   const double max_err2 = (double)max_error * (double)max_error;
   IGN_LAUNCH(ctx, k_simp_ecost, blocks_for(T, 256), 256, 0, s, max_err2, ecost, fstate, flags + 26);
-
+  trace.mark("init_ecost");
+
+  prof_init.end();
   IGN_CUDA(cudaFuncSetAttribute(k_simp_labels, cudaFuncAttributeMaxDynamicSharedMemorySize, (int)sl_dyn[0]));
   IGN_CUDA(cudaFuncSetAttribute(k_simp_resume, cudaFuncAttributeMaxDynamicSharedMemorySize, (int)sl_dyn[1]));
   SlArgs A;
@@ -1601,9 +1603,9 @@
     prof_end(ctx, slot);
     IGN_CUDA(err);
   }
-
-  uint32_t* fscan = node_v;
-  uint32_t* fflag = node_h;
+  trace.mark("labels");
+
+  ProfSpan prof_compact(ctx, IGN_PROF_MC);
   size_t tb = tmpb;
   IGN_LAUNCH(ctx, k_simp_flags_u32, blocks_for(U, 256), 256, 0, s.valive, U, vflag32);
   IGN_CUDA(cub::DeviceScan::ExclusiveSum(tmp, tb, vflag32, vscan, (int)U, ctx->stream));
@@ -1709,6 +1711,8 @@
   IGN_LAUNCH(ctx, k_simp_compact_faces, blocks_for(T, 256), 256, 0, s, vscan, fscan, d_new_vert_off, m->d_faces);
   IGN_TRY(small_d2h(ctx, m->tri_off.data(), d_new_tri_off, (K + 2) * 4));
   IGN_TRY(small_d2h(ctx, m->vert_off.data(), d_new_vert_off, (K + 2) * 4));
+  prof_compact.end();
+  trace.mark("compact");
   IGN_TRY(small_sync(ctx));
   m->U = U2;
   m->T = T2;
```

Measured after the change: 6513 (median of 6 runs). +3.6%, better.
